# arclab-hku/ESVIO

Measured on AMD Instinct MI355X. Metric: Mevents/s through time-surface+detect+track @640x480, higher is better.
Workload: dtype f64 timestamps / u8 images / f32 LK sums in the reference build's order

## Files before the change

### esvio_amd/csrc/fe_api.cpp

```cpp
#include "fe_internal.h"

namespace {
typedef int (*nccl_allgather_fn)(const void*, void*, size_t, int , void* ,
                                 hipStream_t);
struct NcclId {
  char internal[128];
};
typedef int (*nccl_get_id_fn)(NcclId*);
typedef int (*nccl_init_rank_fn)(void** , int, NcclId, int);
typedef int (*nccl_destroy_fn)(void*);
void* rccl_lib() {
  static void* lib = []() -> void* {
    const char* names[] = {"librccl.so.1", "librccl.so"};
    for (const char* n : names)
      if (void* l = dlopen(n, RTLD_NOW | RTLD_NOLOAD | RTLD_GLOBAL)) return l;
    for (const char* n : names)
      if (void* l = dlopen(n, RTLD_NOW | RTLD_GLOBAL)) return l;
    return dlopen("/opt/rocm/lib/librccl.so.1", RTLD_NOW | RTLD_GLOBAL);
  }();
  return lib;
}
template <class F>
F rccl_sym(const char* name) {
  void* l = rccl_lib();
// ... 143 lines not shown
    c->n_cu = n_cu;
    c->waits_fit_spec = lk_blocks + 2 <= n_cu;
    c->waits_fit_chain = 2 * lk_blocks + 2 <= n_cu;
  }
  int prio_least = 0, prio_greatest = 0;
  (void)hipDeviceGetStreamPriorityRange(&prio_least, &prio_greatest);
  if (c->stream.create(hipStreamNonBlocking, prio_greatest) != hipSuccess ||
      c->stream2.create(hipStreamNonBlocking, prio_least) != hipSuccess ||
      c->stream3.create(hipStreamNonBlocking, prio_greatest) != hipSuccess ||
      c->stream4.create(hipStreamNonBlocking, prio_least) != hipSuccess)
    return bail(ESVIO_FE_EHIP);
  {
    const unsigned timed = c->trace ? 0 : hipEventDisableTiming;
    const std::pair<Event*, unsigned> evs[] = {
        {&c->ev_pts_ready, hipEventDisableTiming},  {&c->ev_spec_done, timed},
        {&c->ev_chain_done, timed},                 {&c->ev_dbg_sel_start, 0},
        {&c->ev_sel_host, timed},                   {&c->ev_lks_done[0], hipEventDisableTiming},
        {&c->ev_lks_done[1], hipEventDisableTiming}, {&c->ev_lknew_done, hipEventDisableTiming},
        {&c->ev_planes_free, hipEventDisableTiming}, {&c->ev_imgs_ready, hipEventDisableTiming},
        {&c->ev_arc_side, hipEventDisableTiming},   {&c->ev_sae_left, hipEventDisableTiming},
        {&c->ev_right_ready, hipEventDisableTiming}};
    for (const auto& ef : evs)
      if (ef.first->create(ef.second) != hipSuccess) return bail(ESVIO_FE_EHIP);
    for (int i = 0; i < kPrefetchDepth; i++)
      if (c->ev_lane_done[i].create(timed) != hipSuccess || c->ev_lane_arc[i].create() != hipSuccess)
        return bail(ESVIO_FE_EHIP);
  }
  const size_t M = cfg->max_cnt;
  const int Mc = cfg->max_cnt;
  int rc = 0;
  if ((rc = c->L2.alloc(c, (size_t)2 * c->P))) return bail(rc);
  if ((rc = c->S2.alloc(c, (size_t)2 * c->P))) return bail(rc);
  if ((rc = c->d_rejected.alloc(c, 1))) return bail(rc);
  if ((rc = c->d_res.alloc(c, res_layout(Mc).total))) return bail(rc);
  c->dres = res_view(c->d_res, Mc, 0);
  c->dres.mask = nullptr;
  {
    uint8_t* z_spec = nullptr;
    const size_t bytes = kSpecBlocks * spec_layout(Mc).bytes;
    if ((rc = c->h_spec.alloc(c, bytes))) return bail(rc);
    if (hipHostGetDevicePointer((void**)&z_spec, c->h_spec, 0) != hipSuccess) return bail(ESVIO_FE_EHIP);
    std::memset(c->h_spec, 0, bytes);
    for (int b = 0; b < kSpecBlocks; b++) {
      c->hspec[b] = spec_view(c->h_spec, Mc, b);
      c->zspec[b] = spec_view(z_spec, Mc, b);
    }
  }
  if ((rc = c->d_chain.alloc(c, 2 * std::max<size_t>(M, 1)))) return bail(rc);
  if ((rc = c->d_lane_gate.alloc(c, 16))) return bail(rc);
  c->stage_threads = stager_threads_from_env();
  if (const char* v = getenv("ESVIO_FE_FAULT")) esvio_fe_debug_inject(c, atoi(v));
  if (const char* e = getenv("ESVIO_FE_STEREO_SPLIT")) c->stereo_split_env = atoi(e) != 0;
  c->chain_enabled = getenv("ESVIO_FE_NO_CHAIN") == nullptr;
  c->cam_split_enabled = getenv("ESVIO_FE_NO_CAMSPLIT") == nullptr;
  c->dedup_enabled = getenv("ESVIO_FE_NO_DEDUP") == nullptr && (cfg->max_cnt > 500 || getenv("ESVIO_FE_DEDUP") != nullptr);
  c->fuse_ts_pyr = getenv("ESVIO_FE_NO_FUSE") == nullptr;
  if (const char* v = getenv("ESVIO_FE_CONVERT_PINNED_COPY")) c->cvt_pinned_copy = atoi(v) != 0 ? 1 : 0;
  if (const char* v = getenv("ESVIO_FE_RAW_PINNED_COPY")) c->rawdec.pinned_copy = atoi(v) != 0 ? 1 : 0;
  c->select_one_wave = getenv("ESVIO_FE_SELECT_SERIAL") != nullptr;
  if (const char* v = getenv("ESVIO_FE_SAE_EV_MIN")) c->sae_ev_min = (size_t)strtoull(v, nullptr, 10);
  c->tiled = make_tile_geom(c->W, c->H, &c->tgeom) && getenv("ESVIO_FE_SAE_SORT") == nullptr;
  for (int i = 0; i < kRightSlots; i++)
    if ((rc = c->d_first[i].alloc(c, (size_t)c->P))) return bail(rc);
  for (int i = 0; i < kRightSlots; i++) {
    const size_t words = arc_bitmap_words(c->W, c->H);
    if ((rc = c->d_cmap[i].alloc(c, words))) return bail(rc);
    if ((rc = c->d_touched[i].alloc(c, arc_flag_bytes(c->W, c->H)))) return bail(rc);
    if (hipMemsetAsync(c->d_cmap[i], 0, words * 4, cur_stream(c)) != hipSuccess ||
        hipMemsetAsync(c->d_touched[i], 0, arc_flag_bytes(c->W, c->H), cur_stream(c)) != hipSuccess)
      return bail(ESVIO_FE_EHIP);
  }
  if ((rc = c->d_pub_slots.alloc(c, std::max<size_t>(M, 1)))) return bail(rc);
  if ((rc = c->d_pub_done.alloc(c, 1))) return bail(rc);
  if (hipMemsetAsync(c->d_lane_gate, 0, 64, cur_stream(c)) != hipSuccess ||
      hipMemsetAsync(c->d_chain, 0, std::max<size_t>(M, 1) * 16, cur_stream(c)) != hipSuccess ||
      hipMemsetAsync(c->d_pub_slots, 0, std::max<size_t>(M, 1) * 8, cur_stream(c)) != hipSuccess ||
      hipMemsetAsync(c->d_pub_done, 0, 8, cur_stream(c)) != hipSuccess)
    return bail(ESVIO_FE_EHIP);
  if ((rc = c->d_ptsD.alloc(c, M))) return bail(rc);
  if ((rc = c->d_sel_idx.alloc(c, M))) return bail(rc);
  if ((rc = c->d_mask_bits.alloc(c, (size_t)c->H * ((c->W + 31) / 32)))) return bail(rc);
  for (PyrStore& ps : c->pyr)
    if ((rc = pyr_alloc(c, ps, c->W, c->H, 3))) return bail(rc);
  if (cfg->median_blur_kernel_size > 0)
    for (PyrStore& ps : c->med_tmp)
      if ((rc = pyr_alloc(c, ps, c->W, c->H, 0))) return bail(rc);
  if (cfg->equalize) {
    for (auto& rb : c->raw)
      for (PyrStore& ps : rb)
        if ((rc = pyr_alloc(c, ps, c->W, c->H, 0))) return bail(rc);
    if ((rc = c->d_lut.alloc(c, (size_t)2 * 64 * 256))) return bail(rc);
    if ((rc = c->d_eq_tmp.alloc(c, (size_t)2 * c->P))) return bail(rc);
    if ((rc = c->d_minmax.alloc(c, 4))) return bail(rc);
  }
  {
    uint8_t* z_res = nullptr;
    if ((rc = c->h_pin.alloc(c, pin_bytes(Mc, cfg->width, cfg->height)))) return bail(rc);
    if (hipHostGetDevicePointer((void**)&z_res, c->h_pin, 0) != hipSuccess) return bail(ESVIO_FE_EHIP);
    std::memset(c->h_pin, 0, c->h_pin.cap);
    for (int s = 0; s < 2; s++) {
      c->pin[s] = res_view(c->h_pin, Mc, s);
      c->zpin[s] = res_view(z_res, Mc, s);
    }
  }
  if (hipMemsetAsync(c->L2, 0, (size_t)2 * c->P * 16, cur_stream(c)) != hipSuccess ||
      hipMemsetAsync(c->S2, 0, (size_t)2 * c->P * 16, cur_stream(c)) != hipSuccess ||
// ... 23 lines not shown
    const hipStream_t st[5] = {c->stream, c->stream2, c->stream3, c->stream4, c->stream6};
    const char* nm[5] = {"main", "prefetch", "speculative", "stereo", "stereo-unpublished"};
    const int ns = c->stream6 ? 5 : 4;
    for (int a = 0; a < ns; a++)
      for (int b = 0; b < ns; b++) {
        if (a == b || st[a] == st[b]) continue;
        launch_spin(st[a], 10000);
        const auto t0 = std::chrono::steady_clock::now();
        launch_fill_f64(st[b], (double*)c->d_rejected, 1, 0.0);
        (void)hipStreamSynchronize(st[b]);
        const double us = std::chrono::duration<double, std::micro>(std::chrono::steady_clock::now() - t0).count();
        (void)hipStreamSynchronize(st[a]);
        if (us > 60.0) {
          c->n_queue_conflicts++;
          fprintf(stderr, "[esvio_fe] streams '%s' and '%s' share a hardware queue (%.0f us behind a 100 us kernel)\n", nm[b], nm[a], us);
        }
      }
    if (!c->n_queue_conflicts) fprintf(stderr, "[esvio_fe] the handle's %d streams have a hardware queue each\n", ns);
  }
  c->select_ok = select_lds_bytes(c) <= 160 * 1024;
  if (!c->select_ok && (rc = c->d_sel_bitmap.alloc(c, (size_t)c->H * ((c->W + 31) / 32) + 4))) return bail(rc);
  *out = c;
  return 0;
}

namespace {
int baf_clear(esvio_fe_ctx* c);
int hot_clear(esvio_fe_ctx* c);
int baf_ensure(esvio_fe_ctx* c, size_t n, bool host_src, bool host_dst, bool fields_form);
void decode_state_reset(esvio_fe_ctx* c);
void feed_empty(esvio_fe_ctx* c, bool streams_idle);
}

int esvio_fe_reset(esvio_fe_handle c) {
  if (!c) return ESVIO_FE_EINVAL;
  HIPCHK(c, hipSetDevice(c->dev));
  (void)launcher_drain(c);
  launcher_clear_error(c);
  HIPCHK(c, hipStreamSynchronize(c->stream3));
  HIPCHK(c, hipStreamSynchronize(c->stream4));
  if (c->stream6) HIPCHK(c, hipStreamSynchronize(c->stream6));
  HIPCHK(c, hipStreamSynchronize(c->stream2));
  HIPCHK(c, hipStreamSynchronize(c->stream));
  c->announced.clear();
  c->inflight.clear();
  stager_drain(c);
  c->cur_stage = -1;
  c->pin[0].counts[3] = 0;
  if (c->hist) HIPCHK(c, hipMemsetAsync(c->hist, 0, c->hist.cap * 4, cur_stream(c)));
  std::memset(c->h_spec, 0, kSpecBlocks * spec_layout(c->cfg.max_cnt).bytes);
  c->spec_valid = false;
  c->chain_valid = false;
  c->chain_map_ok = false;
  c->pend.active = false;
  c->pend_right.active = false;
  HIPCHK(c, hipMemsetAsync(c->L2, 0, (size_t)2 * c->P * 16, cur_stream(c)));
  HIPCHK(c, hipMemsetAsync(c->S2, 0, (size_t)2 * c->P * 16, cur_stream(c)));
  if (c->evimg.on)
    if (int rc = evimg_zero(c, true)) return rc;
  if (int rc = baf_clear(c)) return rc;
  if (int rc = hot_clear(c)) return rc;
  decode_state_reset(c);
  c->slice.st[0] = c->slice.st[1] = esvio_fe_ctx::Slice::State();
  HIPCHK(c, hipStreamSynchronize(cur_stream(c)));
  feed_empty(c, true);
  clear_tracker_state(c);
  return 0;
}

static int create_sae_stereo(esvio_fe_ctx* c, const esvio_fe_event* left, size_t nL, const esvio_fe_event* right,
                             size_t nR, int space, const McParams* mc, uint64_t* n_rejected) {
  if (nL + nR >= (1ull << 31)) return fail(c, ESVIO_FE_EINVAL, "batch too large");
  if (!c->inflight.empty()) return fail(c, ESVIO_FE_EINVAL, "a prefetched batch is pending");
  HIPCHK(c, hipSetDevice(c->dev));
  c->ext_sae_pending = false;
  const EventRec *dL, *dR;
  if (int rc = stage_events(c, left, nL, right, nR, space, &dL, &dR)) return rc;
  HIPCHK(c, hipMemsetAsync(c->d_rejected, 0, 8, cur_stream(c)));
  c->evimg.fresh_cams = 0;
  if (int rc = sae_update(c, dL, (uint32_t)nL, dR, (uint32_t)nR, mc)) return rc;
  unsigned long long rej = 0;
  HIPCHK(c, hipMemcpyAsync(&rej, c->d_rejected, 8, hipMemcpyDeviceToHost, cur_stream(c)));
  HIPCHK(c, hipStreamSynchronize(cur_stream(c)));
  if (int rc = lookback_expired(c)) return rc;
  if (n_rejected) *n_rejected = rej;
  if (c->prof_on) resolve_profile(c);
  return 0;
}

int esvio_fe_create_sae_stereo(esvio_fe_handle c, const esvio_fe_event* left, size_t nL,
                               const esvio_fe_event* right, size_t nR, int space,
                               uint64_t* n_rejected) {
  if (!c || (nL && !left) || (nR && !right)) return ESVIO_FE_EINVAL;
  return create_sae_stereo(c, left, nL, right, nR, space, nullptr, n_rejected);
}

int esvio_fe_create_sae_stereo_mc(esvio_fe_handle c, const esvio_fe_event* left, size_t nL,
                                  const esvio_fe_event* right, size_t nR, int space,
                                  const esvio_fe_motion* motion, uint64_t* n_rejected) {
  if (!c || !motion || !nL || !left || (nR && !right)) return ESVIO_FE_EINVAL;
  const McParams mc = make_mc_params(motion);
  return create_sae_stereo(c, left, nL, right, nR, space, &mc, n_rejected);
}

namespace {
int slice_scratch(esvio_fe_ctx* c) {
// ... 238 lines not shown
    for (uint32_t i = 0; i < c->P; i++) {
      L0[i] = l[2 * i];
      L1[i] = l[2 * i + 1];
      S0[i] = s[2 * i];
      S1[i] = s[2 * i + 1];
    }
  }
  return 0;
}

int esvio_fe_get_sae(esvio_fe_handle c, int cam, double* L0, double* L1, double* S0, double* S1) {
  if (!L0 || !L1 || !S0 || !S1) return ESVIO_FE_EINVAL;
  return planes_io(c, cam, L0, L1, S0, S1, nullptr, nullptr, nullptr, nullptr, false);
}
int esvio_fe_set_sae(esvio_fe_handle c, int cam, const double* L0, const double* L1,
                     const double* S0, const double* S1) {
  if (!L0 || !L1 || !S0 || !S1) return ESVIO_FE_EINVAL;
  return planes_io(c, cam, nullptr, nullptr, nullptr, nullptr, L0, L1, S0, S1, true);
}

static int prep_tmp_pyr(esvio_fe_handle c, int slot, const uint8_t* img, int w, int hgt,
                        int max_level) {
  if (int rc = pyr_alloc(c, c->tmp_pyr[slot], w, hgt, max_level)) return rc;
  return copy_level0_in(c, c->tmp_pyr[slot].d, img);
}

int esvio_fe_calc_optical_flow_pyr_lk(esvio_fe_handle c, const uint8_t* prev_img,
                                      const uint8_t* next_img, int w, int hgt,
                                      const float* prev_pts, float* next_pts, uint8_t* status,
                                      int n, int max_level, int max_count, double eps, int flags) {
  if (!c || !prev_img || !next_img || n < 0 || (n && (!prev_pts || !next_pts || !status)))
    return ESVIO_FE_EINVAL;
  if (w < 2 * kLkWin || hgt < 2 * kLkWin || max_level < 0 || max_level >= kMaxLevels)
    return ESVIO_FE_EINVAL;
  if (n > c->cfg.max_cnt) return fail(c, ESVIO_FE_EINVAL, "n > max_cnt");
  if (!n) return 0;
  HIPCHK(c, hipSetDevice(c->dev));
  if (int rc = prep_tmp_pyr(c, 0, prev_img, w, hgt, max_level)) return rc;
  if (int rc = prep_tmp_pyr(c, 1, next_img, w, hgt, max_level)) return rc;
  PyrDesc two[2] = {c->tmp_pyr[0].d, c->tmp_pyr[1].d};
  pyr_build(c, two, 2);
  float2 *d_prev = (float2*)c->dres.A, *d_next = (float2*)c->dres.s1.fwd;
  uint8_t* d_st = c->dres.s1.st_fwd;
  HIPCHK(c, hipMemcpyAsync(d_prev, prev_pts, (size_t)n * 8, hipMemcpyHostToDevice, cur_stream(c)));
  if (flags & ESVIO_FE_LK_USE_INITIAL_FLOW)
    HIPCHK(c, hipMemcpyAsync(d_next, next_pts, (size_t)n * 8, hipMemcpyHostToDevice, cur_stream(c)));
  LkArgs f = make_lk(two[0], two[1], d_prev, d_next, d_next, d_st, nullptr, n, max_level, max_count, eps, flags);
  run_lk(c, f, nullptr, nullptr, nullptr);
  HIPCHK(c, hipMemcpyAsync(next_pts, d_next, (size_t)n * 8, hipMemcpyDeviceToHost, cur_stream(c)));
  HIPCHK(c, hipMemcpyAsync(status, d_st, (size_t)n, hipMemcpyDeviceToHost, cur_stream(c)));
  HIPCHK(c, hipStreamSynchronize(cur_stream(c)));
  if (c->prof_on) resolve_profile(c);
  return 0;
}

int esvio_fe_build_pyramid(esvio_fe_handle c, const uint8_t* img, int w, int hgt, int max_level,
                           int level, uint8_t* out_img, int16_t* out_deriv, int32_t* lw,
                           int32_t* lh, int32_t* n_levels) {
  if (!c || !img || max_level < 0 || max_level >= kMaxLevels || w < 2 * kLkWin || hgt < 2 * kLkWin)
    return ESVIO_FE_EINVAL;
  HIPCHK(c, hipSetDevice(c->dev));
  if (int rc = prep_tmp_pyr(c, 0, img, w, hgt, max_level)) return rc;
  const PyrDesc& d = c->tmp_pyr[0].d;
  pyr_build(c, &d, 1);
  if (n_levels) *n_levels = d.levels + 1;
  if (level < 0 || level > d.levels) {
    HIPCHK(c, hipStreamSynchronize(cur_stream(c)));
    return level < 0 ? 0 : ESVIO_FE_EINVAL;
  }
  if (lw) *lw = d.w[level];
  if (lh) *lh = d.h[level];
  const int stride = d.stride[level];
  if (out_img)
    HIPCHK(c, hipMemcpy2DAsync(out_img, d.w[level], d.img[level] + (size_t)kPad * stride + kPad,
                               stride, d.w[level], d.h[level], hipMemcpyDeviceToHost, cur_stream(c)));
  if (out_deriv)
    HIPCHK(c, hipMemcpy2DAsync(out_deriv, (size_t)d.w[level] * 4,
                               d.deriv[level] + ((size_t)kPad * stride + kPad) * 2, (size_t)stride * 4,
                               (size_t)d.w[level] * 4, d.h[level], hipMemcpyDeviceToHost, cur_stream(c)));
  HIPCHK(c, hipStreamSynchronize(cur_stream(c)));
  if (c->prof_on) resolve_profile(c);
  return 0;
}

int esvio_fe_find_fundamental_mat(const float* p1, const float* p2, int n, double thr, double conf,
                                  uint8_t* status, int32_t* n_inliers) {
  if (n < 0 || (n && (!p1 || !p2 || !status))) return ESVIO_FE_EINVAL;
  const int k = host::find_fundamental_mat(p1, p2, n, thr, conf, status);
  if (n_inliers) *n_inliers = k;
  return 0;
}

int esvio_fe_host_hypot(const double* x, const double* y, int n, double* out) {
  if (n < 0 || (n && (!x || !y || !out))) return ESVIO_FE_EINVAL;
  host::host_hypot(x, y, n, out);
  return ESVIO_FE_OK;
}

int esvio_fe_host_stage_copy(void* dst, const void* src, size_t len) {
  if (len && (!dst || !src)) return ESVIO_FE_EINVAL;
  stager_copy_bytes((uint8_t*)dst, (const uint8_t*)src, len);
  return ESVIO_FE_OK;
}

int esvio_fe_host_stage_pack(void* dst, const void* src, size_t len, uint32_t* base_sec) {
  uint32_t b = 0;
// ... 3415 lines not shown
  return 0;
}

int esvio_fe_mem_free(int space, void* p) {
  if (space != ESVIO_FE_HOST && space != ESVIO_FE_DEVICE) return ESVIO_FE_EINVAL;
  if (!p) return 0;
  return (space == ESVIO_FE_HOST ? hipHostFree(p) : hipFree(p)) == hipSuccess ? 0 : ESVIO_FE_EHIP;
}

int esvio_fe_mem_upload(void* dst_device, const void* src_host, size_t bytes) {
  if (bytes && (!dst_device || !src_host)) return ESVIO_FE_EINVAL;
  if (!bytes) return 0;
  return hipMemcpy(dst_device, src_host, bytes, hipMemcpyHostToDevice) == hipSuccess ? 0 : ESVIO_FE_EHIP;
}

int esvio_fe_register_host_buffer(void* p, size_t bytes) {
  if (!p || !bytes) return ESVIO_FE_EINVAL;
  if (hipHostRegister(p, bytes, hipHostRegisterDefault) != hipSuccess) {
    (void)hipGetLastError();
    return ESVIO_FE_EHIP;
  }
  return 0;
}

int esvio_fe_unregister_host_buffer(void* p) {
  if (!p) return ESVIO_FE_EINVAL;
  if (hipHostUnregister(p) != hipSuccess) {
    (void)hipGetLastError();
    return ESVIO_FE_EHIP;
  }
  return 0;
}

int esvio_fe_debug_inject(esvio_fe_handle c, int mask) {
  if (!c || mask < 0 || mask > 31) return ESVIO_FE_EINVAL;
  c->lim = esvio_fe_ctx::WaitLimits();
  c->lazy_late = (mask & ESVIO_FE_FAULT_LAZY_LATE) != 0;
  if (mask & ESVIO_FE_FAULT_TICKET) c->lim.ticket = 0;
  if (mask & ESVIO_FE_FAULT_LOOKBACK) c->lim.lookback = 0;
  if (mask & ESVIO_FE_FAULT_SPECULATIVE) c->lim.poll = 0;
  if (mask & ESVIO_FE_FAULT_CHAINED) c->lim.chain = 0;
  return 0;
}

int esvio_fe_debug_counters(esvio_fe_handle c, uint64_t out4[4]) {
  if (!c || !out4) return ESVIO_FE_EINVAL;
  out4[0] = c->n_spec_expired;
  out4[1] = c->n_chain_expired;
  out4[2] = c->tr_chain_launch;
  out4[3] = c->tr_chain_used;
  return 0;
}

int esvio_fe_plain_call_counters(esvio_fe_handle c, uint64_t out4[4]) {
  if (!c || !out4) return ESVIO_FE_EINVAL;
  out4[0] = c->n_plain_calls;
  out4[1] = c->n_cam_split;
  out4[2] = c->n_stereo_chained;
  out4[3] = c->n_chain_expired;
  return 0;
}

int esvio_fe_reserve(esvio_fe_handle c, size_t max_left, size_t max_right, int host_batches) {
  if (!c) return ESVIO_FE_EINVAL;
  const size_t n = max_left + max_right;
  if (n >= (1ull << 31)) return fail(c, ESVIO_FE_EINVAL, "batch too large");
  if (!c->inflight.empty() || !c->announced.empty())
    return fail(c, ESVIO_FE_EINVAL, "esvio_fe_reserve while batches are announced");
  HIPCHK(c, hipSetDevice(c->dev));
  HIPCHK(c, hipStreamSynchronize(c->stream2));
  HIPCHK(c, hipStreamSynchronize(c->stream3));
  HIPCHK(c, hipStreamSynchronize(c->stream4));
  if (c->stream6) HIPCHK(c, hipStreamSynchronize(c->stream6));
  HIPCHK(c, hipStreamSynchronize(c->stream));
  if (c->tiled) {
    if (int rc = ensure_part_capacity(c, n, false)) return rc;
  } else if (int rc = ensure_sort_capacity(c, n)) {
    return rc;
  }
  for (int k = 0; k < kRightSlots; k++)
    if (int rc = ensure_arc_capacity(c, max_left, k)) return rc;
  if (c->baf.B)
    if (int rc = baf_ensure(c, std::max(max_left, max_right), host_batches != 0, false, false)) return rc;
  const size_t events[2] = {max_left, max_right};
  if (int rc = raw_reserve(c, events, host_batches != 0)) return rc;
  if (int rc = text_reserve(c, events, host_batches != 0)) return rc;
  if (int rc = aedat_reserve(c, events)) return rc;
  if (int rc = bag_reserve(c, events)) return rc;
  if (int rc = bag_image_reserve(c)) return rc;
  if (int rc = aedat_frame_reserve(c)) return rc;
  if (c->feed.open) {
    const size_t ev[2] = {max_left, max_right};
    for (int cam = 0; cam < 2; cam++) {
      esvio_fe_ctx::Feed::Cam& fc = c->feed.cam[cam];
      for (int b = 0; b < 2; b++)
        if ((b != fc.cur || fc.len == 0) && fc.buf[b].cap < 2 * ev[cam]) {
          if (int rc = fc.buf[b].alloc(c, 2 * ev[cam])) return rc;
          fc.read_rec[b] = false;
        }
    }
  }
  if (host_batches) {
    if (int rc = ensure_event_capacity(c, n)) return rc;
    if (stager_enabled(c)) {
      if (int rc = stager_reserve(c, n)) return rc;
    } else {
// ... 447 lines not shown
```

### esvio_amd/csrc/fe_ctx.h

```cpp
#pragma once
#include <hip/hip_runtime.h>

#include <algorithm>
#include <atomic>
#include <chrono>
#include <cmath>
#include <cstdarg>
#include <cstdio>
#include <cstdlib>
#include <cstring>
#include <dlfcn.h>
#include <map>
#include <string>
#include <utility>
#include <deque>
#include <vector>

#include "../../include/esvio_fe.h"
#include "../../include/esvio_fe_test.h"
#include "fe_aedat.h"
#include "fe_bag.h"
#include "fe_host.h"
#include "fe_kernels.h"
#include "fe_layout.h"
// ... 180 lines not shown
  DevBuf<double> slice_stage;
  bool ext_sae_pending = false;
  DevBuf<float> x_send, x_recv;
  PinBuf<float> x_pin, x_pin_recv;
  void* x_comm = nullptr;
  int x_world = 0;
  Stream x_stream;
  Event x_done;
  bool x_pending = false;
  bool x_auto = false;
  bool x_deferred = false;
  std::deque<Batch> announced;
  std::deque<Inflight> inflight;
  bool cur_prefetched = false;
  EventStager* stager = nullptr;
  std::atomic<int> stage_pending{0};
  int cur_stage = -1;
  int stage_threads = 0;
  Launcher* launcher = nullptr;
  uint64_t lane_job[kPrefetchDepth] = {};
  int launch_err = 0;
  uint64_t lks_wait_job[2] = {};
  struct WaitLimits {
    uint32_t lookback = kSpinLookback, ticket = kSpinTicket;
    unsigned long long poll = kTicksPoll, chain = kTicksChain;
  } lim;
  bool lazy_late = false;
  uint64_t n_spec_expired = 0, n_chain_expired = 0;
  DevBuf<EventRec> d_evp[kPrefetchDepth];
  Event ev_lane_done[kPrefetchDepth], ev_lane_arc[kPrefetchDepth];
  PyrStore tmp_pyr[2];
  PyrStore med_tmp[2];
  PyrStore raw[kRightSlots][2];
  int raw_cur = 0;
  DevBuf<uint8_t> d_lut;
  DevBuf<int> d_minmax;
  DevBuf<uint8_t> d_res;
  ResView dres{};
  DevBuf<float2> d_ptsD;
  ResView pin[2] = {}, zpin[2] = {};
  SpecView hspec[kSpecBlocks] = {}, zspec[kSpecBlocks] = {};
  int res_set = 0;
  int lks_last = -1;
  PinBuf<uint8_t> h_spec;
  bool spec_valid = false;
  int spec_n = 0;
  DevBuf<unsigned long long> d_chain;
  DevBuf<uint32_t> d_lane_gate;
  uint32_t gate_seq = 0;
  int n_cu = 0;
  bool waits_fit_spec = true, waits_fit_chain = true;
  uint32_t chain_seq = 0;
  bool chain_enabled = true;
  bool cam_split_enabled = true;
  uint64_t n_plain_calls = 0, n_cam_split = 0, n_stereo_chained = 0;
  bool chain_valid = false;
  uint64_t chain_for = 0;
  bool chain_map_ok = false;
  std::vector<int> chain_map;
  uint64_t frame_no = 0;
  Event ev_chain_done;
  DevBuf<unsigned long long> d_pub_slots, d_pub_done;
  uint32_t pub_seq = 0;
  bool lazy_new = false;
  struct PendingNew {
    bool active = false;
    bool prev_map_was_empty = false;
    std::vector<int> ids;
    std::vector<P2f> left;
  } pend;
  struct PendingRight {
    bool active = false;
    int set = 0;
    double dt = 0;
    std::vector<int> ids;
    std::vector<P2f> left;
  } pend_right;
  Event ev_lks_done[2], ev_lknew_done;
  host::RansacPool* pool = nullptr;
  DevBuf<uint8_t> d_flags;
  struct CandSet {
    DevBuf<uint32_t> xy, idx, cnt;
    DevBuf<uint32_t> comp_xy, comp_idx, total, grp;
    size_t cap = 0;
  } cand[kRightSlots];
  DevBuf<uint32_t> d_first[kRightSlots];
  DevBuf<uint32_t> d_cmap[kRightSlots];
  DevBuf<uint8_t> d_touched[kRightSlots];
  uint32_t first_epoch[kRightSlots] = {};
  bool dedup_enabled = true;
  bool fuse_ts_pyr = true;
  int cand_cur = 0;
  DevBuf<uint32_t> d_mask_bits;
  DevBuf<float4> d_gftt_cov, d_gftt_rowsum;
  DevBuf<float> d_gftt_eig;
  DevBuf<uint32_t> d_gftt_max;
  DevBuf<int32_t> d_sel_idx;
  DevBuf<uint8_t> d_fast_img;
  PinBuf<uint8_t> h_img;
  DevBuf<uint8_t> d_img;
  unsigned img_stage_next = 0;
  PinBuf<uint8_t> h_pin;

  int n_id = 0;
  double cur_time = 0, prev_time = 0;
  std::vector<P2f> prev_pts, cur_pts, cur_right_pts, n_pts;
// ... 359 lines not shown
```

### esvio_amd/csrc/fe_host.cpp

```cpp
#include "fe_host.h"

#include <algorithm>
#include <cfloat>
#include <climits>
#include <cmath>
#include <cstdio>
#include <cstdlib>
#include <cstring>

#include <atomic>
#include <chrono>
#include <condition_variable>
#include <sys/resource.h>
#include <memory>
#include <mutex>
#include <thread>

#if defined(__linux__)
#include <pthread.h>
#include <sched.h>
#endif

#if defined(__HIP_DEVICE_COMPILE__) || defined(ESVIO_NO_SIMD_CLONES)
#define ESVIO_SIMD_CLONES
// ... 678 lines not shown
  const double F0 = F[0], F1 = F[1], F2 = F[2], F3 = F[3], F4 = F[4], F5 = F[5], F6 = F[6], F7 = F[7],
               F8 = F[8];
  int good = 0;
  for (int i = i0; i < i1; i++) {
    double a = F0 * x1[i] + F1 * y1[i] + F2;
    double b = F3 * x1[i] + F4 * y1[i] + F5;
    double c = F6 * x1[i] + F7 * y1[i] + F8;
    const double s2 = 1. / (a * a + b * b);
    const double d2 = x2[i] * a + y2[i] * b + c;
    a = F0 * x2[i] + F3 * y2[i] + F6;
    b = F1 * x2[i] + F4 * y2[i] + F7;
    c = F2 * x2[i] + F5 * y2[i] + F8;
    const double s1 = 1. / (a * a + b * b);
    const double d1 = x1[i] * a + y1[i] * b + c;
    const double e1 = d1 * d1 * s1, e2 = d2 * d2 * s2;
    const float err = (float)(e1 < e2 ? e2 : e1);
    const int f = err <= t;
    mask[i] = (uint8_t)f;
    good += f;
  }
  return good;
}

int mark_inliers_bounded(const double* x1, const double* y1, const double* x2, const double* y2, int n,
                         const double* F, uint8_t* mask, double thresh, int need) {
  const float t = (float)(thresh * thresh);
  constexpr int kBlock = 32;
  int good = 0;
  for (int i0 = 0; i0 < n; i0 += kBlock) {
    const int i1 = std::min(n, i0 + kBlock);
    good += score_block(x1, y1, x2, y2, i0, i1, F, t, mask);
    if (good + (n - i1) <= need) return good;
  }
  return good;
}

}

namespace {
constexpr int kRansacMaxIters = 1000;
constexpr int kRansacWindow = 128;
constexpr int kIdleSpinUs = 2000;

struct alignas(64) IterResult {
  int nm;
  int good[3];
  double models[27];
};
constexpr uint32_t kCollinear = 0xffffffffu;
}

namespace {
std::atomic<uint64_t> g_rs_calls{0}, g_rs_iters{0}, g_rs_points{0}, g_rs_ns{0}, g_rs_lm_calls{0}, g_rs_lm_ns{0};
std::atomic<uint64_t> g_rs_max_ns{0}, g_rs_lm_max_ns{0}, g_rs_redone{0}, g_rs_solo{0}, g_rs_skipped{0}, g_rs_helper_sw{0};
void atomic_max(std::atomic<uint64_t>& a, uint64_t v) {
  uint64_t cur = a.load(std::memory_order_relaxed);
  while (v > cur && !a.compare_exchange_weak(cur, v, std::memory_order_relaxed)) {
  }
}
}

struct RansacJob {
  alignas(64) std::atomic<int> next{0};
  alignas(64) std::atomic<int> avail{0};
  alignas(64) std::atomic<int> bound{0};
  alignas(64) std::atomic<int> active{0};
  std::vector<double> xy;
  std::vector<float> pts;
  int count = 0;
  double thr = 0;
  bool lmeds = false;
  std::vector<int32_t> picks;
  std::unique_ptr<IterResult[]> res;
  std::unique_ptr<std::atomic<uint64_t>[]> summary;

  uint32_t evaluate(int idx, IterResult& r, std::vector<uint8_t>& scratch) const {
    float s1[14], s2[14];
    if (!gather(idx, s1, s2)) {
      r.nm = -1;
      return kCollinear;
    }
    r.nm = seven_point(s1, s2, r.models);
    return score(r, scratch);
  }

  void evaluate_lanes(int idx0, int cnt, uint32_t e, std::vector<uint8_t>& scratch) {
    float s1[kLanes][14], s2[kLanes][14];
    int lane_of[kLanes], nm[kLanes], live = 0;
    double models[kLanes][27];
    for (int i = 0; i < cnt; i++) {
      if (gather(idx0 + i, s1[live], s2[live])) {
        lane_of[i] = live++;
      } else {
        lane_of[i] = -1;
        res[idx0 + i].nm = -1;
        summary[idx0 + i].store(((uint64_t)e << 32) | kCollinear, std::memory_order_release);
      }
    }
    if (!live) return;
    seven_point_lanes(live, s1, s2, nm, models);
    for (int i = 0; i < cnt; i++) {
      if (lane_of[i] < 0) continue;
      IterResult& r = res[idx0 + i];
      r.nm = nm[lane_of[i]];
      if (r.nm > 0) std::memcpy(r.models, models[lane_of[i]], sizeof(double) * 9 * r.nm);
      summary[idx0 + i].store(((uint64_t)e << 32) | score(r, scratch), std::memory_order_release);
    }
// ... 289 lines not shown
  if (reset) {
    g_rs_skipped = 0;
    g_rs_helper_sw = 0;
    g_rs_max_ns = 0;
    g_rs_lm_max_ns = 0;
    g_rs_redone = 0;
    g_rs_solo = 0;
  }
}

void host_hypot(const double* x, const double* y, int n, double* out) {
  for (int i = 0; i < n; i++) out[i] = cv_hypot(x[i], y[i]);
}

int host_nullspace(const double* A, int n, int lanes, double* f) {
  if (!lanes) {
    for (int i = 0; i < n; i++)
      epipolar_nullspace((const double(*)[9])(A + (size_t)i * 63), f + (size_t)i * 18, f + (size_t)i * 18 + 9);
    return 0;
  }
  int redone = 0;
  for (int i0 = 0; i0 < n; i0 += kLanes) {
    const int cnt = std::min(kLanes, n - i0);
    double Al[kLanes][7][9], f1[kLanes][9], f2[kLanes][9];
    for (int l = 0; l < kLanes; l++) std::memcpy(Al[l], A + (size_t)(i0 + (l < cnt ? l : 0)) * 63, sizeof(Al[l]));
    if (!epipolar_nullspace_lanes(Al, f1, f2)) {
      for (int l = 0; l < cnt; l++) epipolar_nullspace(Al[l], f1[l], f2[l]);
      redone += cnt;
    }
    for (int l = 0; l < cnt; l++) {
      std::memcpy(f + (size_t)(i0 + l) * 18, f1[l], sizeof(f1[l]));
      std::memcpy(f + (size_t)(i0 + l) * 18 + 9, f2[l], sizeof(f2[l]));
    }
  }
  return redone;
}

RansacStats ransac_stats(bool reset) {
  RansacStats r{g_rs_calls.load(), g_rs_iters.load(), g_rs_points.load(), g_rs_ns.load(),
                g_rs_lm_calls.load(), g_rs_lm_ns.load()};
  if (reset) {
    g_rs_lm_calls = 0;
    g_rs_lm_ns = 0;
    g_rs_calls = 0;
    g_rs_iters = 0;
    g_rs_points = 0;
    g_rs_ns = 0;
    g_rs_max_ns = 0;
    g_rs_lm_max_ns = 0;
    g_rs_redone = 0;
    g_rs_solo = 0;
    g_rs_skipped = 0;
    g_rs_helper_sw = 0;
  }
  return r;
}

namespace {
int ransac_pooled(RansacPool* P, const float* m1, const float* m2, int count, double thr, double conf,
                  const double* xy, uint8_t* status, int* iterations) {
  const int kModelPoints = 7;
  const uint32_t e = P->epoch.load(std::memory_order_relaxed) + 1;
  RansacJob& J = P->job[(e >> 1) & 1];
  while (J.active.load(std::memory_order_acquire) != 0) cpu_relax();
  J.xy.assign(xy, xy + 4 * (size_t)count);
  J.pts.resize(4 * (size_t)count);
  std::memcpy(J.pts.data(), m1, 2 * (size_t)count * sizeof(float));
  std::memcpy(J.pts.data() + 2 * (size_t)count, m2, 2 * (size_t)count * sizeof(float));
  J.count = count;
  J.thr = thr;
  J.lmeds = false;
  J.next.store(0, std::memory_order_relaxed);
  J.avail.store(0, std::memory_order_relaxed);
  J.bound.store(kModelPoints - 1, std::memory_order_relaxed);
  P->epoch.store(e, std::memory_order_release);
  if (!P->th.empty()) ransac_pool_wake(P);

  OcvRng rng;
  std::vector<uint8_t> scratch(count);
  std::vector<uint64_t> rng_before;
  rng_before.reserve(256);
  IterResult local;
  double best_F[9];
  const double *x1 = J.xy.data(), *y1 = x1 + count, *x2 = y1 + count, *y2 = x2 + count;
  int drawn = 0, rp = 0, niters = kRansacMaxIters, best_good = 0;
  bool have_best = false;
  int collinear_at = -1;
  unsigned stalled = 0;
  while (collinear_at < 0) {
    while (rp < niters && rp < drawn) {
      const IterResult* r = &J.res[rp];
      const uint64_t sm = J.summary[rp].load(std::memory_order_acquire);
      uint32_t code;
      if ((uint32_t)(sm >> 32) == e) {
        code = (uint32_t)sm;
      } else if (stalled > 64) {
        code = J.evaluate(rp, local, scratch);
        r = &local;
        g_rs_redone.fetch_add(1, std::memory_order_relaxed);
      } else {
        break;
      }
      stalled = 0;
      if (code == kCollinear) {
        collinear_at = rp;
        break;
      }
      if ((int)code > std::max(best_good, kModelPoints - 1))
        for (int k = 0; k < r->nm; k++)
          if (r->good[k] > std::max(best_good, kModelPoints - 1)) {
            best_good = r->good[k];
            std::memcpy(best_F, r->models + 9 * k, sizeof(best_F));
            have_best = true;
            niters = update_num_iters(conf, (double)(count - best_good) / count, kModelPoints, niters);
          }
      rp++;
      J.bound.store(std::max(best_good, kModelPoints - 1), std::memory_order_relaxed);
    }
    if (rp >= niters || collinear_at >= 0) break;
    if (drawn < niters && drawn - rp < kRansacWindow) {
      for (int j = 0; j < kLanes && drawn < niters; j++) {
        rng_before.push_back(rng.s);
        int32_t* pk = &J.picks[(size_t)drawn * 8];
        for (int i = 0; i < 7; i++) {
          int pick, q;
          for (;;) {
            pick = pk[i] = rng.uniform(0, count);
            for (q = 0; q < i; q++)
              if (pick == pk[q]) break;
            if (q == i) break;
          }
        }
        drawn++;
      }
      J.avail.store(drawn, std::memory_order_release);
      continue;
    }
    int idx = J.next.load(std::memory_order_relaxed);
    if (idx < drawn && J.next.compare_exchange_strong(idx, idx + kLanes, std::memory_order_relaxed)) {
      J.evaluate_lanes(idx, std::min(kLanes, drawn - idx), e, scratch);
    } else {
      cpu_relax();
      stalled++;
    }
  }
  P->epoch.store(e + 1, std::memory_order_release);
  if (collinear_at >= 0) {
    rng.s = rng_before[collinear_at];
    float s1[14], s2[14];
    for (int iter = collinear_at; iter < niters; iter++) {
      if (!draw_subset(m1, m2, count, s1, s2, rng, 10000)) {
        if (iter == 0) return 0;
        break;
      }
      const int nm = seven_point(s1, s2, local.models);
      for (int k = 0; k < nm; k++) {
        const int good = mark_inliers_bounded(x1, y1, x2, y2, count, local.models + 9 * k, scratch.data(), thr,
                                              std::max(best_good, kModelPoints - 1));
        if (good > std::max(best_good, kModelPoints - 1)) {
          best_good = good;
          std::memcpy(best_F, local.models + 9 * k, sizeof(best_F));
          have_best = true;
          niters = update_num_iters(conf, (double)(count - good) / count, kModelPoints, niters);
        }
      }
    }
  }
  *iterations = niters;
  if (have_best) score_block(x1, y1, x2, y2, 0, count, best_F, (float)(thr * thr), status);
  return best_good;
}

int lmeds_pooled(RansacPool* P, const float* m1, const float* m2, int count, double conf, uint8_t* status) {
  const int kModelPoints = 7;
  const int niters = std::max(update_num_iters(conf, 0.45, kModelPoints, kRansacMaxIters), 3);
  const uint32_t e = P->epoch.load(std::memory_order_relaxed) + 1;
  RansacJob& J = P->job[(e >> 1) & 1];
  while (J.active.load(std::memory_order_acquire) != 0) cpu_relax();
  OcvRng rng;
  float s1[14], s2[14];
  int nsub = 0;
  for (; nsub < niters; nsub++)
    if (!draw_subset(m1, m2, count, s1, s2, rng, 1000, &J.picks[(size_t)nsub * 8])) break;
  if (nsub == 0) return 0;
  J.pts.resize(4 * (size_t)count);
  std::memcpy(J.pts.data(), m1, 2 * (size_t)count * sizeof(float));
  std::memcpy(J.pts.data() + 2 * (size_t)count, m2, 2 * (size_t)count * sizeof(float));
  J.count = count;
  J.lmeds = true;
  J.next.store(0, std::memory_order_relaxed);
  J.avail.store(nsub, std::memory_order_relaxed);
  P->epoch.store(e, std::memory_order_release);
  if (!P->th.empty()) ransac_pool_wake(P);
  std::vector<uint8_t> scratch;
  IterResult local;
  double best[9], min_median = DBL_MAX;
  unsigned stalled = 0;
  for (int rp = 0; rp < nsub;) {
    const IterResult* r = &J.res[rp];
    const uint64_t sm = J.summary[rp].load(std::memory_order_acquire);
    if ((uint32_t)(sm >> 32) != e) {
      int idx = J.next.load(std::memory_order_relaxed);
      if (idx < nsub && J.next.compare_exchange_strong(idx, idx + kLanes, std::memory_order_relaxed)) {
        J.evaluate_lanes(idx, std::min(kLanes, nsub - idx), e, scratch);
        continue;
      }
      if (++stalled <= 64) {
        cpu_relax();
        continue;
      }
      J.evaluate(rp, local, scratch);
      r = &local;
      g_rs_redone.fetch_add(1, std::memory_order_relaxed);
    }
    stalled = 0;
    for (int k = 0; k < r->nm; k++) {
      float med;
      std::memcpy(&med, &r->good[k], sizeof(float));
      if ((double)med < min_median) {
        min_median = med;
        std::memcpy(best, r->models + 9 * k, sizeof(best));
      }
    }
    rp++;
  }
  P->epoch.store(e + 1, std::memory_order_release);
  if (min_median < DBL_MAX) {
    double sigma = 2.5 * 1.4826 * (1 + 5. / (count - kModelPoints)) * std::sqrt(min_median);
    sigma = std::max(sigma, 0.001);
    std::vector<float> err(count);
    return mark_inliers(m1, m2, count, best, err, status, sigma);
  }
  return 0;
}
}

int find_fundamental_mat(const float* m1, const float* m2, int count, double thr, double conf,
                         uint8_t* status, RansacPool* pool) {
  std::fill(status, status + count, (uint8_t)0);
  if (count < 7) return 0;
  if (thr <= 0) thr = 3;
  if (conf < DBL_EPSILON || conf > 1 - DBL_EPSILON) conf = 0.99;
  if (count == 7) {
    double models[27];
    const int n = seven_point(m1, m2, models);
    std::fill(status, status + count, (uint8_t)1);
    return n > 0 ? count : 0;
  }
  static thread_local std::unique_ptr<RansacPool> solo;
  if (pool) {
    auto held = [&](uint32_t e) { return pool->job[(e >> 1) & 1].active.load(std::memory_order_acquire) != 0; };
    const uint32_t e = pool->epoch.load(std::memory_order_relaxed) + 1;
    int spins = 0;
    while (held(e) && ++spins < 256) cpu_relax();
    if (held(e)) {
      if (!held(e + 2)) {
        pool->epoch.store(e + 1, std::memory_order_release);
        g_rs_skipped.fetch_add(1, std::memory_order_relaxed);
      } else {
        g_rs_solo.fetch_add(1, std::memory_order_relaxed);
        pool = nullptr;
      }
    }
  }
  if (!pool) {
    if (!solo) solo.reset(ransac_pool_alloc());
    pool = solo.get();
  }
  if (count >= 15) {
    std::vector<double> xy((size_t)4 * count);
    double *x1 = xy.data(), *y1 = x1 + count, *x2 = y1 + count, *y2 = x2 + count;
    for (int i = 0; i < count; i++) {
      x1[i] = m1[2 * i];
      y1[i] = m1[2 * i + 1];
      x2[i] = m2[2 * i];
      y2[i] = m2[2 * i + 1];
    }
    const auto t0 = std::chrono::steady_clock::now();
    int iters = 0;
    const int good = ransac_pooled(pool, m1, m2, count, thr, conf, xy.data(), status, &iters);
    g_rs_calls.fetch_add(1, std::memory_order_relaxed);
    g_rs_iters.fetch_add((uint64_t)iters, std::memory_order_relaxed);
    g_rs_points.fetch_add((uint64_t)count, std::memory_order_relaxed);
    const uint64_t ns = (uint64_t)std::chrono::duration_cast<std::chrono::nanoseconds>(
                            std::chrono::steady_clock::now() - t0).count();
    g_rs_ns.fetch_add(ns, std::memory_order_relaxed);
    atomic_max(g_rs_max_ns, ns);
    return good;
  }
  const auto t0 = std::chrono::steady_clock::now();
  const int good = lmeds_pooled(pool, m1, m2, count, conf, status);
  g_rs_lm_calls.fetch_add(1, std::memory_order_relaxed);
  const uint64_t ns = (uint64_t)std::chrono::duration_cast<std::chrono::nanoseconds>(
                          std::chrono::steady_clock::now() - t0).count();
  g_rs_lm_ns.fetch_add(ns, std::memory_order_relaxed);
  atomic_max(g_rs_lm_max_ns, ns);
  return good;
}

}
}
```

### esvio_amd/csrc/fe_host.h

```cpp
#pragma once
#include <atomic>
#include <stdint.h>

#include <vector>

#include "../../include/esvio_fe.h"
#include "../../include/esvio_fe_test.h"

namespace esvio {
inline void cpu_relax() {
#if !defined(__HIP_DEVICE_COMPILE__) && (defined(__x86_64__) || defined(__i386__))
  __builtin_ia32_pause();
#endif
}
namespace host {

int cv_round(double v);
int cv_floor(float v);

void lift_projective(const esvio_fe_camera& cam, double u, double v, double out[3]);
void lift_projective_batch(const esvio_fe_camera& cam, const float* uv, int n, double* xu, double* yu);

std::vector<int> disc_halfwidths(int r);

struct BitMask {
  int W = 0, H = 0, wpr = 0;
  std::vector<uint32_t> bits;
  void reset(int w, int h);
  bool test(int x, int y) const { return (bits[(size_t)y * wpr + (x >> 5)] >> (x & 31)) & 1u; }
  void stamp_disc(int cx, int cy, int r, const std::vector<int>& hw);
  void from_bytes(const uint8_t* mask);
};

struct RansacPool;
RansacPool* ransac_pool_create(int helpers);
void ransac_pool_destroy(RansacPool* p);
void ransac_pool_wake(RansacPool* p);
void host_hypot(const double* x, const double* y, int n, double* out);
int host_nullspace(const double* A, int n, int lanes, double* f);
struct RansacStats {
  uint64_t calls, iterations, points, ns, lmeds_calls, lmeds_ns;
};
RansacStats ransac_stats(bool reset);
void ransac_tail(uint64_t out6[6], bool reset);
void ransac_pool_hold(RansacPool* p, int mask, bool on);
void ransac_pool_set_idle_work(RansacPool* p, const std::atomic<int>* pending, bool (*fn)(void*), void* arg);
int find_fundamental_mat(const float* p1, const float* p2, int n, double thr, double conf,
                         uint8_t* status, RansacPool* pool = nullptr);

}
}
```

### esvio_amd/csrc/fe_internal.h

```cpp
#pragma once
#include "fe_ctx.h"

namespace esvio {
namespace fe {

template <class T>
void reduce_vector(std::vector<T>& v, const std::vector<uint8_t>& status) {
  int j = 0;
  for (int i = 0; i < int(v.size()); i++)
    if (status[i]) v[j++] = v[i];
  v.resize(j);
}

inline uint8_t* px00(const PyrDesc& d) { return d.img[0] + (size_t)kPad * d.stride[0] + kPad; }

inline int lookback_expired(esvio_fe_ctx* c) {
  return c->pin[0].counts[3] ? fail(c, ESVIO_FE_EINTERNAL, "radix sort look-back spin expired") : 0;
}

int ensure_event_capacity(esvio_fe_ctx* c, size_t n);
int ensure_sort_capacity(esvio_fe_ctx* c, size_t n);
int ensure_part_capacity(esvio_fe_ctx* c, size_t n, bool mc);
int ensure_cand_capacity(esvio_fe_ctx* c, int set, size_t n);
int ensure_arc_capacity(esvio_fe_ctx* c, size_t n, int set);
int pyr_alloc(esvio_fe_ctx* c, PyrStore& ps, int w, int h, int max_level);
uint64_t pyr_pixels(const PyrDesc& d);
void pyr_build(esvio_fe_ctx* c, const PyrDesc* p, int nimg);
McParams make_mc_params(const esvio_fe_motion* m);
int sae_update(esvio_fe_ctx* c, const EventRec* evL, uint32_t nL, const EventRec* evR, uint32_t nR,
               const McParams* mc = nullptr, double2* L2 = nullptr, double2* S2 = nullptr, int arc_set = -1,
               bool* arc_marked = nullptr);
int evimg_update(esvio_fe_ctx* c, const EventRec* evL, uint32_t nL, const EventRec* evR, uint32_t nR, const McParams* mc);
int evimg_zero(esvio_fe_ctx* c, bool every_set = false);
int radix_sort_pairs(esvio_fe_ctx* c, uint32_t n, int passes, int bits, bool booked = true);
struct SortBufs {
  uint32_t *keys[2], *vals[2];
  uint32_t* scratch;
  const uint32_t* n_dev;
};
int radix_sort_pairs(esvio_fe_ctx* c, const SortBufs& b, uint32_t n, int passes, int bits, bool booked);
int cand_set_alloc(esvio_fe_ctx* c, esvio_fe_ctx::CandSet& s, size_t cap, size_t total_words = 1);
int stage_events(esvio_fe_ctx* c, const esvio_fe_event* left, size_t nL, const esvio_fe_event* right,
                 size_t nR, int space, const EventRec** dL, const EventRec** dR, int lane = -1);
void render_ts(esvio_fe_ctx* c, double t_sync, uint8_t* dst0, uint8_t* dst1, int ncam, const double2* S2);
void run_clahe(esvio_fe_ctx* c, const uint8_t* src0, const uint8_t* src1, int src_stride, uint8_t* dst0, uint8_t* dst1,
               int dst_stride, int nimg, int stages, uint64_t booked_px);
void render_lk_images(esvio_fe_ctx* c, double t_sync, int cams, int slotL, int slotR, int rawbuf);
bool render_cam_ok(const esvio_fe_ctx* c);
void build_lk_images(esvio_fe_ctx* c, double t_sync, int cams , int slotL, int slotR,
                     int rawbuf, bool right_imported = false);
inline int other_right_slot(const esvio_fe_ctx* c) { return c->slot_curR == kLeftSlots ? kLeftSlots + 1 : kLeftSlots; }
void rotate_slots(esvio_fe_ctx* c, bool right_advanced);
const PyrDesc& raw_ts_desc(const esvio_fe_ctx* c, int cam);
LkArgs make_lk(const PyrDesc& P, const PyrDesc& N, const float2* prev, const float2* init, float2* next,
               uint8_t* status, const int* n_ptr, int n_max, int max_level, int max_count, double eps,
               int flags);
void run_lk(esvio_fe_ctx* c, const LkArgs& f, const LkArgs* b, float2* back_pts, uint8_t* back_status);
enum LkPairKind { kLkTemporal, kLkStereo };
struct LkPair {
  LkArgs f, b;
  LkOut out;
};
LkPair lk_pair(const PyrDesc& P, const PyrDesc& N, const P2f* src, const int* n_ptr, int n_max, LkPairKind kind,
               const LkOut& out);
void run_lk_pair(esvio_fe_ctx* c, const LkPair& p);
int copy_level0_out(esvio_fe_ctx* c, const PyrDesc& d, uint8_t* out);
int copy_level0_in(esvio_fe_ctx* c, const PyrDesc& d, const uint8_t* in, int space = ESVIO_FE_HOST);
bool in_border_event(const esvio_fe_ctx* c, const P2f& pt);
double pt_distance(const P2f& a, const P2f& b);
void event_set_mask(esvio_fe_ctx* c);
std::vector<P2f> undistorted_pts(const std::vector<P2f>& pts, const esvio_fe_camera& cam);
std::vector<P2f> pts_velocity_fn(std::vector<int>& ids, std::vector<P2f>& pts, IdMap& cur_id_pts,
                                 IdMap& prev_id_pts, double dt, size_t n_left);
void reject_with_f_event(esvio_fe_ctx* c);
void clear_tracker_state(esvio_fe_ctx* c);
SelectArgs make_select_args(esvio_fe_ctx* c, int set, int max_corners, float2* out_pts, int out_base,
                            int32_t* out_idx);
size_t select_lds_bytes(const esvio_fe_ctx* c);
KernelId launch_select_args(esvio_fe_ctx* c, SelectArgs s);
void compact_set(esvio_fe_ctx* c, const esvio_fe_ctx::CandSet& cs, uint32_t nblk, bool booked);
void run_select(esvio_fe_ctx* c, int set, int max_corners, float2* out_pts, int out_base, int32_t* out_idx,
                const uint32_t* mask_bits = nullptr, int* host_counts = nullptr, bool publish = false,
                const float2* stamp_pts = nullptr, int n_stamp = 0);
void run_arc(esvio_fe_ctx* c, const EventRec* ev, uint32_t n, const PyrDesc* ts, bool use_mask,
             bool want_flags, bool want_cand, int set, bool marked = false);
int run_detect(esvio_fe_ctx* c, const EventRec* ev, uint32_t n, const PyrDesc& ts, int set, bool marked);
inline size_t detect_cand_need(const esvio_fe_ctx* c, size_t n) { return c->detector == ESVIO_FE_DETECT_FAST ? (size_t)c->P : n; }
hipError_t sync_main(esvio_fe_ctx* c);
hipError_t sync_event(hipEvent_t ev);

int stager_threads_from_env();
inline bool stager_enabled(const esvio_fe_ctx* c) { return c->stage_threads > 0; }
int stager_begin(esvio_fe_ctx* c, const esvio_fe_event* left, size_t nL, const esvio_fe_event* right, size_t nR,
                 int dma_groups, int* slot_out, bool by_camera = false);
int stager_attach_left(esvio_fe_ctx* c, int slot, hipStream_t s, const EventRec** dL);
int stager_mark_read_aux(esvio_fe_ctx* c, int slot, hipStream_t s);
bool stager_ready(esvio_fe_ctx* c, int slot);
int stager_attach(esvio_fe_ctx* c, int slot, size_t nL, hipStream_t s, const EventRec** dL, const EventRec** dR);
int stager_mark_read(esvio_fe_ctx* c, int slot, hipStream_t s, bool main_stream);
int stager_release(esvio_fe_ctx* c, int slot);
void stager_abandon(esvio_fe_ctx* c, int slot);
void stager_share_pool(esvio_fe_ctx* c);
int stager_reserve(esvio_fe_ctx* c, size_t n_events);
void stager_ptrs(esvio_fe_ctx* c, int slot, size_t nL, const EventRec** dL, const EventRec** dR);
void stager_drain(esvio_fe_ctx* c);
void stager_destroy(esvio_fe_ctx* c);
void stager_copy_bytes(uint8_t* dst, const uint8_t* src, size_t len);
bool stager_pack_bytes(uint8_t* dst, const uint8_t* src, size_t len, uint32_t* base_sec);
void stager_counters(esvio_fe_ctx* c, uint64_t out4[4]);

int prefetch_next(esvio_fe_ctx* c, bool wait_planes, bool must_take_first = false);
int launcher_set(esvio_fe_ctx* c, bool on);
int stereo_split_prepare(esvio_fe_ctx* c);
int launcher_drain(esvio_fe_ctx* c);
int launcher_wait_lane(esvio_fe_ctx* c, int lane);
void launcher_clear_error(esvio_fe_ctx* c);
int cancel_chain(esvio_fe_ctx* c);
int finalize_lazy(esvio_fe_ctx* c);
int track_event_impl(esvio_fe_ctx* c, double cur_time, const esvio_fe_event* left, size_t nL,
                     const esvio_fe_event* right, size_t nR, int space, bool PUB_THIS_FRAME,
                     const esvio_fe_motion* motion = nullptr);

int exchange_pack(esvio_fe_ctx* c);
int exchange_flush(esvio_fe_ctx* c);

void euclid_halfwidths(double md, int8_t* hw , int* radius);
int gftt_run(esvio_fe_ctx* c, const PyrDesc& d, int max_corners, double quality, double min_distance,
// ... 16 lines not shown
```

### esvio_amd/csrc/fe_kernels.h

```cpp
#pragma once
#include <hip/hip_runtime.h>
#include <stdint.h>
#include <stdlib.h>

#include <vector>

namespace esvio {


struct __attribute__((aligned(16))) EventRec {
  uint16_t x, y;
  uint32_t sec, nsec;
  uint8_t pol;
  uint8_t pad[3];
};
static_assert(sizeof(EventRec) == 16, "event record must be 16 B");

constexpr int kPad = 24;
constexpr int kMaxLevels = 4;
constexpr int kLkWin = 21;
constexpr int kArcBlock = 256;
constexpr int kMaxDiscR = 63;

struct PyrDesc {
// ... 205 lines not shown
                      unsigned long long* n_rejected);
void launch_tile_scatter(hipStream_t s, const EventRec* evL, uint32_t nL, const EventRec* evR, uint32_t nR,
                         const TileGeom& g, const TileScratch& sc, EventRec* part, const uint32_t* warp_xy = nullptr);
void launch_tile_apply(hipStream_t s, const EventRec* part, uint32_t n, const TileGeom& g, const TileScratch& sc,
                       double2* L2, double2* S2, double filter_threshold, uint8_t* arc_touched, int* err,
                       uint32_t spin_limit = kSpinTicket);

constexpr double kSliceNone = -1.0;
void launch_fill_f64(hipStream_t s, double* p, size_t n, double v);
void launch_spin(hipStream_t s, unsigned long long ticks);
void launch_set_u32(hipStream_t s, uint32_t* p, uint32_t v);
void launch_overlay_f64(hipStream_t s, double* dst, const double* src, size_t n, double none);

KernelId launch_time_surface(hipStream_t s, const double2* S2, int W, int H, double t_sync,
                         double decay_sec, int ignore_polarity, uint8_t* dst0, uint8_t* dst1,
                         int dst_stride, int ncam);

constexpr int kMaxMedianK = 7;
void launch_median(hipStream_t s, const uint8_t* src0, const uint8_t* src1, int src_stride,
                   uint8_t* dst0, uint8_t* dst1, int dst_stride, int W, int H, int k, int nimg);

void launch_norm_pyr(hipStream_t s, const uint8_t* src0, const uint8_t* src1, int src_stride, const int* minmax,
                     const PyrDesc* p);
void launch_clahe(hipStream_t s, const uint8_t* raw0, const uint8_t* raw1, int raw_stride,
                  uint8_t* dst0, uint8_t* dst1, int dst_stride, int W, int H, uint8_t* lut,
                  int* minmax, int nimg, int stage);

void launch_pyr_down(hipStream_t s, const PyrDesc* p, int nimg, int src_level);
void launch_pyr3(hipStream_t s, const PyrDesc* p, int nimg);
void launch_pyr_pad(hipStream_t s, const PyrDesc* p, int nimg);
void launch_pad_scharr(hipStream_t s, const PyrDesc* p, int nimg);
void launch_scharr(hipStream_t s, const PyrDesc* p, int nimg);

struct LkArgs {
  PyrDesc P;
  PyrDesc N;
  const float2* prev_pts;
  const float2* init_pts;
  float2* next_pts;
  uint8_t* status;
  const int* n_ptr;
  int n_max;
  const unsigned long long* poll_slots = nullptr;
  const unsigned long long* poll_done = nullptr;
  uint32_t poll_seq = 0;
  int poll_from = 0;
  int* poll_err = nullptr;
  unsigned long long* chain_out = nullptr;
  const unsigned long long* chain_in = nullptr;
  uint32_t chain_seq = 0;
  unsigned long long poll_ticks = kTicksPoll, chain_ticks = kTicksChain;
  const uint32_t* gate_ptr = nullptr;
  uint32_t gate_val = 0;
  int max_level;
  int max_count;
  double eps2;
  int flags;
  int accum = 1;
};
void launch_lk(hipStream_t s, const LkArgs& f, const LkArgs* b, float2* back_pts,
               uint8_t* back_status);

struct ArcArgs {
  const EventRec* ev;
  uint32_t n;
  const double2* L2;
  const double2* S2;
  int W, H;
  double filter_threshold;
  int border;
  const uint8_t* ts;
  int ts_stride;
  double ts_lk_threshold;
  const uint32_t* mask_bits;
  int wpr;
  uint8_t* flags;
  uint32_t* cand_xy;
  uint32_t* cand_idx;
  uint32_t* cand_cnt;
  uint32_t* first_map;
  uint32_t first_key;
  uint8_t* touched;
  uint32_t* cmap;
};
inline size_t arc_bitmap_words(int W, int H) { return ((size_t)2 * W * H + 31) / 32 + 64; }
inline size_t arc_flag_bytes(int W, int H) { return (size_t)2 * W * H + 1024; }
void launch_stage_pull(hipStream_t s, const void* pinned_src, void* dst, size_t bytes);
void launch_stage_pull_packed(hipStream_t s, const void* pinned_src, void* dst, size_t bytes, const void* desc, uint32_t epc);
void launch_arc_mark(hipStream_t s, const ArcArgs& a);
void launch_arc_map(hipStream_t s, const ArcArgs& a);
void launch_arc(hipStream_t s, const ArcArgs& a);

void launch_dedup(hipStream_t s, uint32_t* cand_xy, uint32_t* cand_idx, uint32_t* cand_cnt,
                  uint32_t nblk, const uint32_t* first_map, uint32_t first_key, int W);

void launch_compact(hipStream_t s, const uint32_t* cand_xy, const uint32_t* cand_idx,
                    const uint32_t* cand_cnt, uint32_t nblk, uint32_t* comp_xy, uint32_t* comp_idx,
                    uint32_t* total, uint32_t* grp_scratch = nullptr);

struct GfttArgs {
  const uint8_t* img;
  int stride;
  int W, H;
  float4* cov;
  float4* rowsum;
  float* eig;
// ... 446 lines not shown
```

### esvio_amd/csrc/fe_kernels.hip

```cpp
#include "fe_kernels.h"
#include "fe_mc.h"
#include "fe_text.h"

#include <algorithm>
#include <cstdio>
#include <cstdlib>
#include <cstring>
#include <tuple>
#include <type_traits>

namespace esvio {

namespace {
template <typename... P, typename... A>
void launch_k(void (*kernel)(P...), dim3 grid, dim3 block, unsigned shmem, hipStream_t s, A... args) {
  static_assert(sizeof...(P) == sizeof...(A), "argument count");
  hipLaunchKernelGGL(kernel, grid, block, shmem, s, args...);
}
}

__device__ __forceinline__ int lane_id() { return threadIdx.x & 63; }

__device__ __forceinline__ double ev_time(uint32_t sec, uint32_t nsec) {
  return __dadd_rn((double)sec, __dmul_rn(1e-9, (double)nsec));
// ... 2270 lines not shown
          np.y -= d.y * 0.5f;
          level_done = true;
          break;
        }
        if (j >= c.max_count) {
          level_done = true;
          break;
        }
        if (wave_any(inx < -WIN || inx >= cols || iny < -WIN || iny >= rows)) {
          if (L == 0) st = 0;
          level_done = true;
          break;
        }
        if (wave_any(ox > rngx || oy > rngy)) {
          restage = true;
          break;
        }
      }
      (void)restage;
    }
    if (st && L == 0) {
      const float fx = np.x - halfWin, fy = np.y - halfWin;
      const int ix = (int)floorf(fx), iy = (int)floorf(fy);
      if (ix < -WIN || ix >= cols || iy < -WIN || iy >= rows) st = 0;
    }
  }
  np_out = np;
  st_out = st;
}

struct LkKernelArgs {
  LkCall fwd;
  LkCall back;
  int have_back;
  const float2* prev_pts;
  const float2* init_pts;
  float2* next_pts;
  uint8_t* status;
  float2* back_pts;
  uint8_t* back_status;
  const int* n_ptr;
  int n_max;
  const unsigned long long* poll_slots;
  const unsigned long long* poll_done;
  uint32_t poll_seq;
  int poll_from;
  int* poll_err;
  unsigned long long* chain_out;
  const unsigned long long* chain_in;
  uint32_t chain_seq;
  unsigned long long poll_ticks, chain_ticks;
  const uint32_t* gate_ptr;
  uint32_t gate_val;
};

__device__ __forceinline__ void chain_publish(const LkKernelArgs& a, int pt, int lane, float2 p, int alive) {
  if (!a.chain_out || lane != 0) return;
  const unsigned long long hi = (unsigned long long)((a.chain_seq << 2) | (uint32_t)(alive ? 1 : 0)) << 32;
  __hip_atomic_store(&a.chain_out[2 * pt], hi | __float_as_uint(p.x), __ATOMIC_RELAXED, __HIP_MEMORY_SCOPE_AGENT);
  __hip_atomic_store(&a.chain_out[2 * pt + 1], hi | __float_as_uint(p.y), __ATOMIC_RELAXED,
                     __HIP_MEMORY_SCOPE_AGENT);
}

template <int ACCUM>
__device__ __forceinline__ void lk_kernel_body(const LkKernelArgs& a, uint32_t (*regJ_s)[kLkRegStore], uint32_t acc_t,
                                               float* acc_ta, const LkLaneF32* lnf) {
  const int wave = threadIdx.x >> 6, lane = lane_id();
  const int pt = blockIdx.x * kLkWaves + wave;
  const int n = a.n_ptr ? *a.n_ptr : a.n_max;
  if (pt >= a.n_max) return;
  if (pt >= n) {
    chain_publish(a, pt, lane, make_float2(0.f, 0.f), 0);
    return;
  }
  float2 prev0;
  if (a.chain_in) {
    const unsigned long long t0 = wall_clock64();
    unsigned long long vx, vy;
    if (!a.chain_ticks) {
      if (lane == 0) *a.poll_err = 1;
      return;
    }
    for (;;) {
      vx = __hip_atomic_load(&a.chain_in[2 * pt], __ATOMIC_RELAXED, __HIP_MEMORY_SCOPE_AGENT);
      vy = __hip_atomic_load(&a.chain_in[2 * pt + 1], __ATOMIC_RELAXED, __HIP_MEMORY_SCOPE_AGENT);
      if ((uint32_t)(vx >> 34) == a.chain_seq && (uint32_t)(vy >> 34) == a.chain_seq) break;
      if (wall_clock64() - t0 > a.chain_ticks) {
        if (lane == 0) *a.poll_err = 1;
        return;
      }
      __builtin_amdgcn_s_sleep(8);
    }
    if (!((uint32_t)(vx >> 32) & 1u)) {
      if (lane == 0) {
        a.status[pt] = 0;
        if (a.have_back) a.back_status[pt] = 0;
      }
      return;
    }
    prev0 = make_float2(__uint_as_float((uint32_t)vx), __uint_as_float((uint32_t)vy));
    if (a.gate_ptr) {
      for (;;) {
        const uint32_t gv = __hip_atomic_load(a.gate_ptr, __ATOMIC_RELAXED, __HIP_MEMORY_SCOPE_AGENT);
        if ((int)(gv - a.gate_val) >= 0) break;
        if (wall_clock64() - t0 > a.chain_ticks) {
          if (lane == 0) *a.poll_err = 1;
          return;
        }
        __builtin_amdgcn_s_sleep(8);
      }
      __builtin_amdgcn_fence(__ATOMIC_ACQUIRE, "agent");
    }
  } else if (a.poll_slots && pt >= a.poll_from) {
    const unsigned long long t0 = wall_clock64();
    unsigned long long v;
    for (;;) {
      v = __hip_atomic_load(&a.poll_slots[pt], __ATOMIC_RELAXED, __HIP_MEMORY_SCOPE_AGENT);
      if ((uint32_t)(v >> 32) == a.poll_seq) break;
      const unsigned long long d = __hip_atomic_load(a.poll_done, __ATOMIC_RELAXED, __HIP_MEMORY_SCOPE_AGENT);
      if ((uint32_t)(d >> 32) == a.poll_seq && pt >= (int)(uint32_t)d) {
        chain_publish(a, pt, lane, make_float2(0.f, 0.f), 0);
        return;
      }
      if (wall_clock64() - t0 > a.poll_ticks) {
        if (lane == 0) *a.poll_err = 1;
        chain_publish(a, pt, lane, make_float2(0.f, 0.f), 0);
        return;
      }
      __builtin_amdgcn_s_sleep(16);
    }
    prev0 = make_float2((float)(uint32_t)(v & 0xffffu), (float)(uint32_t)((v >> 16) & 0xffffu));
  } else {
    prev0 = a.prev_pts[pt];
  }
  const float2 init = (a.fwd.flags & 4) ? a.init_pts[pt] : make_float2(0.f, 0.f);
  float2 np;
  int st;
  lk_point<ACCUM>(a.fwd, prev0, init, regJ_s[wave], acc_t, acc_ta, lnf, lane, np, st);
  chain_publish(a, pt, lane, np, st);
  if (lane == 0) {
    a.next_pts[pt] = np;
    a.status[pt] = (uint8_t)st;
  }
  if (a.have_back) {
    float2 bp;
    int bs;
    lk_point<ACCUM>(a.back, np, prev0, regJ_s[wave], acc_t, acc_ta, lnf, lane, bp, bs);
    if (lane == 0) {
      a.back_pts[pt] = bp;
      a.back_status[pt] = (uint8_t)bs;
    }
  }
}

__global__ __launch_bounds__(64 * kLkWaves) void k_lk(LkKernelArgs a) {
  __shared__ __attribute__((aligned(16))) uint32_t regJ_s[kLkWaves][kLkRegStore];
  lk_kernel_body<1>(a, regJ_s, 0u, nullptr, nullptr);
}
__global__ __launch_bounds__(64 * kLkWaves) void k_lk_f32(LkKernelArgs a) {
  __shared__ __attribute__((aligned(16))) uint32_t regJ_s[kLkWaves][kLkRegStore];
  __shared__ __attribute__((aligned(16))) int term_all[kLkWaves][kF32TermWords];
  __shared__ __attribute__((aligned(16))) float term_a[kLkWaves][kLkTermWordsA];
  const int wave = threadIdx.x >> 6, lane = threadIdx.x & 63;
  for (int i = lane; i < kF32TermWords; i += 64) term_all[wave][i] = 0;
  {
    const int l = lane < 63 ? lane : 62, t = l / kLkWin, rw = l - t * kLkWin;
    float* z = term_a[wave] + 5 * t * kLkChainWordsA + rw * 5 + 4;
#pragma unroll
    for (int L = 0; L < kMaxLevels; L++)
#pragma unroll
      for (int k = 0; k < 4; k++) z[L * kLkTermLevelA + k * kLkChainWordsA] = 0.f;
  }
  __builtin_amdgcn_fence(__ATOMIC_SEQ_CST, "wavefront", "local");
  const LkLaneF32 lnf =
      lk_lane_f32(lane, (uint32_t)(uintptr_t)(__attribute__((address_space(3))) float*)term_a[wave]);
  const uint32_t tb = (uint32_t)(uintptr_t)(__attribute__((address_space(3))) int*)term_all[wave];
  lk_kernel_body<2>(a, regJ_s, tb, term_a[wave], &lnf);
}

void launch_lk(hipStream_t s, const LkArgs& f, const LkArgs* b, float2* back_pts,
               uint8_t* back_status) {
  if (f.n_max <= 0) return;
  LkKernelArgs a;
  a.fwd.P = f.P;
  a.fwd.N = f.N;
  a.fwd.max_level = f.max_level;
  a.fwd.max_count = f.max_count;
  a.fwd.eps2 = f.eps2;
  a.fwd.flags = f.flags;
  a.have_back = b ? 1 : 0;
  a.back = a.fwd;
  if (b) {
    a.back.P = b->P;
    a.back.N = b->N;
    a.back.max_level = b->max_level;
    a.back.max_count = b->max_count;
    a.back.eps2 = b->eps2;
    a.back.flags = b->flags;
  }
  a.prev_pts = f.prev_pts;
  a.init_pts = f.init_pts;
  a.next_pts = f.next_pts;
  a.status = f.status;
  a.back_pts = back_pts;
  a.back_status = back_status;
  a.n_ptr = f.n_ptr;
  a.n_max = f.n_max;
  a.poll_slots = f.poll_slots;
  a.poll_done = f.poll_done;
  a.poll_seq = f.poll_seq;
  a.poll_from = f.poll_from;
  a.poll_err = f.poll_err;
  a.chain_out = f.chain_out;
  a.chain_in = f.chain_in;
  a.chain_seq = f.chain_seq;
  a.poll_ticks = f.poll_ticks;
  a.chain_ticks = f.chain_ticks;
  a.gate_ptr = f.gate_ptr;
  a.gate_val = f.gate_val;
  if (f.accum == 2)
    launch_k(k_lk_f32, dim3((a.n_max + kLkWaves - 1) / kLkWaves), dim3(64 * kLkWaves), 0, s, a);
  else
    launch_k(k_lk, dim3((a.n_max + kLkWaves - 1) / kLkWaves), dim3(64 * kLkWaves), 0, s, a);
}

__constant__ int8_t c_small[16][2] = {{0, 3},  {1, 3},   {2, 2},   {3, 1},  {3, 0},  {3, -1},
                                      {2, -2}, {1, -3},  {0, -3},  {-1, -3}, {-2, -2}, {-3, -1},
                                      {-3, 0}, {-3, 1},  {-2, 2},  {-1, 3}};
__constant__ int8_t c_large[20][2] = {{0, 4},   {1, 4},   {2, 3},   {3, 2},  {4, 1},  {4, 0},  {4, -1},
                                      {3, -2},  {2, -3},  {1, -4},  {0, -4}, {-1, -4}, {-2, -3}, {-3, -2},
                                      {-4, -1}, {-4, 0},  {-4, 1},  {-3, 2}, {-2, 3},  {-1, 4}};

template <int N>
struct RingRanks {
  unsigned long long lo, hi;
  __device__ __forceinline__ int get(int i) const {
    if (N <= 16) return (int)((lo >> (4 * i)) & 15ull);
    return i < 10 ? (int)((lo >> (5 * i)) & 31ull) : (int)((hi >> (5 * (i - 10))) & 31ull);
  }
};

template <int N, int KMIN, int KMAX>
__device__ __forceinline__ bool arc_ring_ranks(const double (&v)[N]) {
  int r[N];
#pragma unroll
  for (int i = 0; i < N; i++) r[i] = 0;
#pragma unroll
  for (int i = 1; i < N; i++)
#pragma unroll
    for (int j = 0; j < i; j++) {
      r[i] += v[j] < v[i] ? 1 : 0;
      r[j] += v[i] < v[j] ? 1 : 0;
    }
  RingRanks<N> rk;
  rk.lo = 0;
  rk.hi = 0;
#pragma unroll
  for (int i = 0; i < N; i++) {
    if (N <= 16) rk.lo |= (unsigned long long)r[i] << (4 * i);
    else if (i < 10) rk.lo |= (unsigned long long)r[i] << (5 * i);
    else rk.hi |= (unsigned long long)r[i] << (5 * (i - 10));
  }
  int segment_new_min_t = r[0];
  int arc_right_idx = 0;
#pragma unroll
  for (int i = 1; i < N; i++)
    if (r[i] > segment_new_min_t) {
      segment_new_min_t = r[i];
      arc_right_idx = i;
    }
  int arc_left_idx = arc_right_idx == 0 ? N - 1 : arc_right_idx - 1;
  arc_right_idx = arc_right_idx == N - 1 ? 0 : arc_right_idx + 1;
// ... 3655 lines not shown
```

### esvio_amd/csrc/fe_layout.h

```cpp
#pragma once
#include <cstddef>
#include <cstdint>

namespace esvio {
namespace fe {

struct P2f {
  float x, y;
};

struct LkOut {
  P2f *fwd, *back;
  uint8_t *st_fwd, *st_back;
};

inline size_t layout_points(int max_cnt) { return max_cnt > 1 ? (size_t)max_cnt : 1; }
inline size_t round_up(size_t v, size_t to) { return (v + to - 1) / to * to; }

struct ResLayout {
  size_t B1[2], C1[2], SA1[2], SB1[2], A[2], CNT, NEW, B2, C2, SA2, SB2, total;
  size_t mask;
};
inline ResLayout res_layout(int max_cnt) {
  const size_t M = layout_points(max_cnt), stM = round_up(M, 64);
  ResLayout L;
  size_t o = 0;
  for (int s = 0; s < 2; s++) {
    L.B1[s] = o;  o += M * 8;
    L.C1[s] = o;  o += M * 8;
    L.SA1[s] = o; o += stM;
    L.SB1[s] = o; o += stM;
    L.A[s] = o;   o += M * 8;
  }
  L.CNT = o; o += 64;
  L.NEW = o; o += M * 8;
  L.B2 = o;  o += M * 8;
  L.C2 = o;  o += M * 8;
  L.SA2 = o; o += stM;
  L.SB2 = o; o += stM;
  L.total = o;
  L.mask = round_up(o, 256);
  return L;
}
inline size_t pin_bytes(int max_cnt, int width, int height) {
  return res_layout(max_cnt).mask + (size_t)height * ((width + 31) / 32) * 4 + 256;
}

struct SpecLayout {
  size_t B, C, SA, SB, expired, bytes;
};
inline SpecLayout spec_layout(int max_cnt) {
  const size_t M = layout_points(max_cnt), stM = round_up(M, 64);
  SpecLayout L;
  L.B = 0;
  L.C = M * 8;
  L.SA = M * 16;
  L.SB = L.SA + stM;
  L.expired = L.SB + stM;
  L.bytes = round_up(L.expired + 64, 256);
  return L;
}
constexpr int kSpecBlocks = 2;

struct ResView {
  LkOut s1;
  P2f* A;
  LkOut s2;
  P2f* news;
  int* counts;
  uint32_t* mask;
};
inline ResView res_view(uint8_t* b, int max_cnt, int set) {
  const ResLayout L = res_layout(max_cnt);
  ResView v;
  v.s1 = LkOut{(P2f*)(b + L.B1[set]), (P2f*)(b + L.C1[set]), b + L.SA1[set], b + L.SB1[set]};
  v.A = (P2f*)(b + L.A[set]);
  v.s2 = LkOut{(P2f*)(b + L.B2), (P2f*)(b + L.C2), b + L.SA2, b + L.SB2};
  v.news = (P2f*)(b + L.NEW);
  v.counts = (int*)(b + L.CNT);
  v.mask = (uint32_t*)(b + L.mask);
  return v;
}

struct SpecView {
  LkOut out;
  int* expired;
};
inline SpecView spec_view(uint8_t* b, int max_cnt, int block) {
  const SpecLayout L = spec_layout(max_cnt);
  b += (size_t)block * L.bytes;
  return SpecView{LkOut{(P2f*)(b + L.B), (P2f*)(b + L.C), b + L.SA, b + L.SB}, (int*)(b + L.expired)};
}

}
}
```

### esvio_amd/csrc/fe_stages.cpp

```cpp
#include "fe_internal.h"

#include <optional>

namespace esvio {
namespace fe {


int ensure_event_capacity(esvio_fe_ctx* c, size_t n) { return c->d_ev.grow(c, n); }

static int grow_sort_buffers(esvio_fe_ctx* c, size_t cap) {
  c->sort_cap = 0;
  for (int i = 0; i < 2; i++) {
    c->keys[i].release();
    c->vals[i].release();
  }
  for (int i = 0; i < 2; i++) {
    if (int rc = c->keys[i].alloc(c, cap)) return rc;
    if (int rc = c->vals[i].alloc(c, cap)) return rc;
  }
  if (int rc = c->sae_marks.alloc(c, cap)) return rc;
  c->sort_cap = cap;
  return 0;
}

// ... 431 lines not shown
  return LkPair{make_lk(P, N, (const float2*)src, nullptr, (float2*)out.fwd, out.st_fwd, n_ptr, n_max, 3, 30, 0.01, 0),
                make_lk(N, P, nullptr, nullptr, nullptr, nullptr, n_ptr, n_max, t ? 1 : 3, 30, 0.01,
                        t ? ESVIO_FE_LK_USE_INITIAL_FLOW : 0),
                out};
}

void run_lk_pair(esvio_fe_ctx* c, const LkPair& p) {
  run_lk(c, p.f, c->cfg.flow_back ? &p.b : nullptr, (float2*)p.out.back, p.out.st_back);
}

static int image_stage_slot(esvio_fe_ctx* c, size_t bytes, size_t* off) {
  constexpr int kSlots = 4;
  if (!c->d_img || c->d_img.cap < kSlots * bytes) {
    HIPCHK(c, hipStreamSynchronize(cur_stream(c)));
    c->d_img.release();
    if (int rc = c->h_img.alloc(c, kSlots * bytes)) return rc;
    if (int rc = c->d_img.alloc(c, kSlots * bytes)) return rc;
  }
  *off = (size_t)(c->img_stage_next++ % kSlots) * (c->d_img.cap / kSlots);
  return 0;
}

int copy_level0_in(esvio_fe_ctx* c, const PyrDesc& d, const uint8_t* in, int space) {
  const int stride = d.stride[0];
  const size_t bytes = (size_t)d.w[0] * d.h[0];
  if (space == ESVIO_FE_DEVICE) {
    HIPCHK(c, hipMemcpy2DAsync(d.img[0] + (size_t)kPad * stride + kPad, stride, in, d.w[0], d.w[0], d.h[0], hipMemcpyDeviceToDevice,
                               cur_stream(c)));
    return 0;
  }
  size_t off = 0;
  if (int rc = image_stage_slot(c, bytes, &off)) return rc;
  std::memcpy(c->h_img + off, in, bytes);
  HIPCHK(c, hipMemcpyAsync(c->d_img + off, c->h_img + off, bytes, hipMemcpyHostToDevice, cur_stream(c)));
  HIPCHK(c, hipMemcpy2DAsync(d.img[0] + (size_t)kPad * stride + kPad, stride, c->d_img + off, d.w[0], d.w[0],
                             d.h[0], hipMemcpyDeviceToDevice, cur_stream(c)));
  return 0;
}

int copy_level0_out(esvio_fe_ctx* c, const PyrDesc& d, uint8_t* out) {
  const int stride = d.stride[0];
  const size_t bytes = (size_t)d.w[0] * d.h[0];
  size_t off = 0;
  if (int rc = image_stage_slot(c, bytes, &off)) return rc;
  HIPCHK(c, hipMemcpy2DAsync(c->d_img + off, d.w[0], d.img[0] + (size_t)kPad * stride + kPad, stride, d.w[0],
                             d.h[0], hipMemcpyDeviceToDevice, cur_stream(c)));
  HIPCHK(c, hipMemcpyAsync(c->h_img + off, c->d_img + off, bytes, hipMemcpyDeviceToHost, cur_stream(c)));
  HIPCHK(c, hipStreamSynchronize(cur_stream(c)));
  std::memcpy(out, c->h_img + off, bytes);
  return 0;
}


bool in_border_event(const esvio_fe_ctx* c, const P2f& pt) {
  const int BORDER_SIZE = 1;
  const int img_x = host::cv_round(pt.x), img_y = host::cv_round(pt.y);
  return BORDER_SIZE <= img_x && img_x < c->W - BORDER_SIZE && BORDER_SIZE <= img_y &&
         img_y < c->H - BORDER_SIZE;
}

double pt_distance(const P2f& a, const P2f& b) {
  const double dx = a.x - b.x, dy = a.y - b.y;
  return std::sqrt(dx * dx + dy * dy);
}

void event_set_mask(esvio_fe_ctx* c) {
  c->mask_event.reset(c->W, c->H);
  struct Item {
    int first;
    std::pair<P2f, int> second;
    int src;
  };
  std::vector<Item> cnt_pts_id;
  cnt_pts_id.reserve(c->cur_pts.size());
  for (unsigned int i = 0; i < c->cur_pts.size(); i++)
    cnt_pts_id.push_back(Item{c->track_cnt[i], std::make_pair(c->cur_pts[i], c->ids[i]), c->src_idx[i]});
  std::sort(cnt_pts_id.begin(), cnt_pts_id.end(),
            [](const Item& a, const Item& b) { return a.first > b.first; });
  c->cur_pts.clear();
  c->ids.clear();
  c->track_cnt.clear();
  c->src_idx.clear();
  for (auto& it : cnt_pts_id) {
    const int px = host::cv_round(it.second.first.x), py = host::cv_round(it.second.first.y);
    if (px < 0 || px >= c->W || py < 0 || py >= c->H) continue;
    if (!c->mask_event.test(px, py)) {
      c->cur_pts.push_back(it.second.first);
      c->ids.push_back(it.second.second);
      c->track_cnt.push_back(it.first);
      c->src_idx.push_back(it.src);
      c->mask_event.stamp_disc(px, py, c->cfg.min_dist, c->hw);
    }
  }
}

std::vector<P2f> undistorted_pts(const std::vector<P2f>& pts, const esvio_fe_camera& cam) {
  const size_t n = pts.size();
  std::vector<P2f> un(n);
  if (!n) return un;
  std::vector<double> lx(n), ly(n);
  host::lift_projective_batch(cam, &pts[0].x, (int)n, lx.data(), ly.data());
  for (size_t i = 0; i < n; i++) un[i] = P2f{(float)lx[i], (float)ly[i]};
  return un;
}

std::vector<P2f> pts_velocity_fn(std::vector<int>& ids, std::vector<P2f>& pts, IdMap& cur_id_pts,
                                 IdMap& prev_id_pts, double dt, size_t n_left) {
  std::vector<P2f> vel;
  cur_id_pts.build(ids, pts);
  if (!prev_id_pts.empty()) {
    vel.reserve(pts.size());
    for (unsigned int i = 0; i < pts.size(); i++) {
      const P2f* prev = ids[i] != -1 ? prev_id_pts.find(ids[i]) : nullptr;
      if (prev) {
        const double v_x = (pts[i].x - prev->x) / dt;
        const double v_y = (pts[i].y - prev->y) / dt;
        vel.push_back(P2f{(float)v_x, (float)v_y});
      } else {
        vel.push_back(P2f{0, 0});
      }
    }
  } else {
    vel.assign(n_left, P2f{0, 0});
  }
  return vel;
}

void reject_with_f_event(esvio_fe_ctx* c) {
  if (c->trace) c->tr_fm_class[c->cur_pts.size() < 8 ? 0 : c->cur_pts.size() < 15 ? 1 : 2]++;
  if (c->cur_pts.size() >= 8) {
    const esvio_fe_camera& cam = c->cfg.cam[0];
    const double FOCAL = c->cfg.focal_length;
    const size_t n = c->prev_pts.size();
    std::vector<float> un_cur(n * 2), un_prev(n * 2);
    std::vector<double> lx(n), ly(n);
    const double cx = c->W / 2.0, cy = c->H / 2.0;
    const auto tl = std::chrono::steady_clock::now();
    const bool pre = c->pre_lift_valid && c->pre_lx.size() == n;
    if (!pre) host::lift_projective_batch(cam, &c->prev_pts[0].x, (int)n, lx.data(), ly.data());
    const double* plx = pre ? c->pre_lx.data() : lx.data();
    const double* ply = pre ? c->pre_ly.data() : ly.data();
    c->pre_lift_valid = false;
    for (size_t i = 0; i < n; i++) {
      un_prev[2 * i] = (float)(FOCAL * plx[i] / 1.0 + cx);
      un_prev[2 * i + 1] = (float)(FOCAL * ply[i] / 1.0 + cy);
    }
    host::lift_projective_batch(cam, &c->cur_pts[0].x, (int)n, lx.data(), ly.data());
    for (size_t i = 0; i < n; i++) {
      un_cur[2 * i] = (float)(FOCAL * lx[i] / 1.0 + cx);
      un_cur[2 * i + 1] = (float)(FOCAL * ly[i] / 1.0 + cy);
    }
    std::vector<uint8_t> status(c->cur_pts.size());
    const auto t0 = std::chrono::steady_clock::now();
    host::find_fundamental_mat(un_prev.data(), un_cur.data(), (int)c->cur_pts.size(),
                               c->cfg.f_threshold, 0.99, status.data(), c->pool);
    if (c->trace) {
      const double ms = std::chrono::duration<double, std::milli>(std::chrono::steady_clock::now() - t0).count();
      c->tr_fm_ms += ms;
      c->tr_fm_max_ms = std::max(c->tr_fm_max_ms, ms);
      c->tr_lift_ms += std::chrono::duration<double, std::milli>(t0 - tl).count();
    }
    reduce_vector(c->prev_pts, status);
    reduce_vector(c->cur_pts, status);
    reduce_vector(c->ids, status);
    reduce_vector(c->track_cnt, status);
    reduce_vector(c->src_idx, status);
  }
}

void clear_tracker_state(esvio_fe_ctx* c) {
  c->prev_pts.clear();
  c->cur_pts.clear();
  c->cur_right_pts.clear();
  c->n_pts.clear();
  c->cur_un_pts.clear();
  c->cur_un_right_pts.clear();
  c->pts_velocity.clear();
  c->right_pts_velocity.clear();
  c->ids.clear();
  c->ids_right.clear();
  c->track_cnt.clear();
  c->track_cnt_right.clear();
  c->cur_un_pts_map.clear();
  c->prev_un_pts_map.clear();
  c->cur_un_right_pts_map.clear();
  c->prev_un_right_pts_map.clear();
  c->have_img = false;
  c->slot_prevL = c->slot_curL = 0;
  c->slot_curR = kLeftSlots;
  c->ext_right_pending = false;
  c->ext_sae_pending = false;
  c->cur_time = c->prev_time = 0;
}

SelectArgs make_select_args(esvio_fe_ctx* c, int set, int max_corners, float2* out_pts, int out_base,
                            int32_t* out_idx) {
  SelectArgs s{};
  s.comp_xy = c->cand[set].comp_xy;
  s.comp_idx = c->cand[set].comp_idx;
  s.total = c->cand[set].total;
  s.W = c->W;
  s.H = c->H;
  s.wpr = (c->W + 31) / 32;
  s.max_corners = max_corners;
  s.radius = c->cfg.min_dist;
  for (int i = 0; i <= kMaxDiscR; i++) s.hw[i] = i < (int)c->hw.size() ? (int8_t)c->hw[i] : -1;
  s.disc_c = disc_threshold(s.hw, s.radius);
  s.out_pts = out_pts;
  s.out_idx = out_idx;
  s.out_base = out_base;
  s.n_out = c->dres.counts;
  s.n_total = c->dres.counts + 1;
  s.host_counts = nullptr;
  s.init_bits = nullptr;
  s.gbitmap = nullptr;
  s.pub_slots = nullptr;
  s.pub_done = nullptr;
  s.pub_seq = 0;
  s.one_wave = c->select_one_wave ? 1 : 0;
  return s;
// ... 113 lines not shown
```

### esvio_amd/csrc/fe_track.cpp

```cpp
#include "fe_internal.h"

#include <sched.h>
#include <sys/resource.h>

#include <atomic>
#include <condition_variable>
#include <mutex>
#include <thread>

namespace esvio {
namespace fe {

struct PrefetchJob {
  Inflight b;
  bool wait_planes = false;
  int lks_wait = -1;
};

static int prefetch_issue(esvio_fe_ctx* c, const PrefetchJob& j) {
  const Inflight& b = j.b;
  StreamScope on_prefetch_stream(c->stream2);
  PrefetchBatchScope its_event_images(&b);
  if (j.wait_planes) HIPCHK(c, hipStreamWaitEvent(c->stream2, c->ev_planes_free, 0));
  if (j.lks_wait >= 0) HIPCHK(c, hipStreamWaitEvent(c->stream2, c->ev_lks_done[j.lks_wait], 0));
// ... 237 lines not shown
      }
    }
    if (rc) break;
    c->inflight.push_back(b);
    c->announced.pop_front();
    if (only_first) break;
  }
  return rc;
}

static uint32_t next_chain_seq(esvio_fe_ctx* c) {
  c->chain_seq = (c->chain_seq + 1) & 0x3fffffffu;
  if (!c->chain_seq) c->chain_seq = 1;
  return c->chain_seq;
}

int enqueue_spec_temporal(esvio_fe_ctx* c, const Inflight& nxt ,
                          int n_kept, bool with_new) {
  if (int rc = launcher_wait_lane(c, nxt.lane)) return rc;
  HIPCHK(c, hipStreamWaitEvent(c->stream3, c->ev_lane_done[nxt.lane], 0));
  const PyrDesc& P = c->pyr[c->slot_curL].d;
  const PyrDesc& N = c->pyr[nxt.slotL].d;
  const int n_max = with_new ? (int)layout_points(c->cfg.max_cnt) : n_kept;
  LkPair sp = lk_pair(P, N, c->zpin[0].news, nullptr, n_max, kLkTemporal, c->zspec[0].out);
  if (with_new) {
    sp.f.poll_slots = c->d_pub_slots;
    sp.f.poll_done = c->d_pub_done;
    sp.f.poll_seq = c->pub_seq;
    sp.f.poll_from = n_kept;
    sp.f.poll_err = c->zspec[0].expired;
    sp.f.poll_ticks = c->lim.poll;
  }
  const Inflight* nxt2 = nullptr;
  if (c->chain_enabled && c->waits_fit_chain && !nxt.pub && c->inflight.size() >= 2 && c->inflight[0].lane == nxt.lane &&
      !c->chain_valid)
    nxt2 = &c->inflight[1];
  if (nxt2) {
    sp.f.chain_out = c->d_chain;
    sp.f.chain_seq = next_chain_seq(c);
  }
  {
    StreamScope on_spec_stream(c->stream3);
    run_lk_pair(c, sp);
  }
  HIPCHK(c, hipEventRecord(c->ev_spec_done, c->stream3));
  c->spec_valid = true;
  if (nxt2) {
    const bool gated = c->launcher && nxt2->gate != 0;
    if (!gated)
      if (int rc = launcher_wait_lane(c, nxt2->lane)) return rc;
    HIPCHK(c, hipStreamWaitEvent(c->stream4, c->ev_lane_done[nxt.lane], 0));
    if (!gated) HIPCHK(c, hipStreamWaitEvent(c->stream4, c->ev_lane_done[nxt2->lane], 0));
    const PyrDesc& N2 = c->pyr[nxt2->slotL].d;
    LkPair ch = lk_pair(N, N2, nullptr, nullptr, n_max, kLkTemporal, c->zspec[1].out);
    ch.f.chain_in = c->d_chain;
    ch.f.chain_seq = c->chain_seq;
    ch.f.chain_ticks = c->lim.chain;
    ch.f.poll_err = c->zspec[1].expired;
    if (gated) {
      ch.f.gate_ptr = c->d_lane_gate + nxt2->lane;
      ch.f.gate_val = nxt2->gate;
    }
    {
      StreamScope on_chain_stream(c->stream4);
      run_lk_pair(c, ch);
    }
    HIPCHK(c, hipEventRecord(c->ev_chain_done, c->stream4));
    c->chain_valid = true;
    c->tr_chain_launch++;
    c->chain_for = c->frame_no + 2;
    c->chain_map_ok = false;
  }
  return 0;
}

int cancel_chain(esvio_fe_ctx* c) {
  if (!c->chain_valid) return 0;
  c->chain_valid = false;
  c->chain_map_ok = false;
  c->tr_chain_cancel++;
  HIPCHK(c, hipStreamSynchronize(c->stream4));
  return 0;
}

void right_tail(esvio_fe_ctx* c, const LkOut& kept, const P2f* left, const int* ids, const int* src,
                int n, int n_kept, double dt, size_t n_left) {
  const esvio_fe_config& cfg = c->cfg;
  c->ids_right.clear();
  c->cur_right_pts.clear();
  c->cur_un_right_pts.clear();
  c->right_pts_velocity.clear();
  c->cur_un_right_pts_map.clear();
  c->track_cnt_right.clear();
  if (n_left) {
    std::vector<uint8_t> status(n), statusRightLeft(n);
    std::vector<P2f> reverseLeftPts(n);
    c->cur_right_pts.resize(n);
    for (int i = 0; i < n; i++) {
      const LkOut& r = i < n_kept ? kept : c->pin[0].s2;
      const int j = i < n_kept ? (src ? src[i] : i) : i - n_kept;
      c->cur_right_pts[i] = r.fwd[j];
      status[i] = r.st_fwd[j];
      reverseLeftPts[i] = r.back[j];
      statusRightLeft[i] = r.st_back[j];
    }
    if (cfg.flow_back && !c->cur_right_pts.empty()) {
      for (int i = 0; i < n; i++) {
        if (status[i] && statusRightLeft[i] && in_border_event(c, c->cur_right_pts[i]) &&
            pt_distance(left[i], reverseLeftPts[i]) <= 0.5)
          status[i] = 1;
        else
          status[i] = 0;
      }
    }
    c->ids_right.assign(ids, ids + n);
    reduce_vector(c->cur_right_pts, status);
    reduce_vector(c->ids_right, status);
    c->track_cnt_right.assign(c->cur_right_pts.size(), 1);
    c->cur_un_right_pts = undistorted_pts(c->cur_right_pts, cfg.cam[1]);
    c->right_pts_velocity =
        pts_velocity_fn(c->ids_right, c->cur_un_right_pts, c->cur_un_right_pts_map,
                        c->prev_un_right_pts_map, dt, n_left);
  }
  c->prev_un_right_pts_map.swap(c->cur_un_right_pts_map);
}

static int finalize_right(esvio_fe_ctx* c) {
  if (!c->pend_right.active) return 0;
  esvio_fe_ctx::PendingRight& pr = c->pend_right;
  pr.active = false;
  const int n = (int)pr.left.size();
  if (n) HIPCHK(c, sync_event(c->ev_lks_done[pr.set]));
  if (int rc = lookback_expired(c)) return rc;
  right_tail(c, c->pin[pr.set].s1, pr.left.data(), pr.ids.data(), nullptr, n, n, pr.dt, (size_t)n);
  return 0;
}
// ... 15 lines not shown
      add_ids.push_back(c->pend.ids[j]);
    }
  }
  if (add.empty()) return 0;
  const std::vector<P2f> un = undistorted_pts(add, cfg.cam[1]);
  for (size_t j = 0; j < add.size(); j++) {
    c->ids_right.push_back(add_ids[j]);
    c->cur_right_pts.push_back(add[j]);
    c->cur_un_right_pts.push_back(un[j]);
    c->track_cnt_right.push_back(1);
    if (!c->pend.prev_map_was_empty) c->right_pts_velocity.push_back(P2f{0, 0});
    c->prev_un_right_pts_map.v.emplace_back(add_ids[j], un[j]);
  }
  return 0;
}

int finalize_lazy(esvio_fe_ctx* c) {
  if (int rc = finalize_pending(c)) return rc;
  return finalize_right(c);
}

static bool event_over(hipEvent_t ev) {
  const bool over = hipEventQuery(ev) != hipErrorNotReady;
  (void)hipGetLastError();
  return over;
}

namespace {
using clk = std::chrono::steady_clock;

struct TrackCall {
  esvio_fe_ctx* c;
  const double time;
  const esvio_fe_event *left, *right;
  const size_t nL, nR;
  const int space;
  const bool PUB_THIS_FRAME;
  const esvio_fe_motion* motion;
  const int M;
  ResView pin{}, zpin{};
  const EventRec *dL = nullptr, *dR = nullptr;
  bool first = false;
  bool arc_done = false, arc_prefetched = false, arc_marked_main = false;
  int arc_lane = 0;
  bool main_reads_events = false;
  bool main_reads_planes = false;
  bool have_next = false, had_announced = false;
  Inflight next_b;
  bool early_done = false, defer_late = false;
  bool use_spec = false, use_chain = false, chain_covers_next = false;
  bool will_spec = false, detect = false;
  bool plain = false, arc_side = false, stereo_chained = false;
  bool split_right = false;
  int set_st = 0;
  std::vector<int> surv_src;
  int n_surv = 0, n_kept = 0;
  PhaseClock clock;

  TrackCall(esvio_fe_ctx* ctx, double t, const esvio_fe_event* l, size_t nl, const esvio_fe_event* r, size_t nr,
            int sp, bool pub, const esvio_fe_motion* mo)
      : c(ctx), time(t), left(l), right(r), nL(nl), nR(nr), space(sp), PUB_THIS_FRAME(pub), motion(mo),
        M(ctx->cfg.max_cnt) {}

  void lap(Phase p) { c->lat.cur_phase[p] += clock.lap(); }

  bool same_motion(const Batch& a) const {
    if ((motion != nullptr) != a.has_motion) return false;
    if (!motion) return true;
    const esvio_fe_motion &x = *motion, &y = a.motion;
    bool eq = x.t1 == y.t1 && x.fx == y.fx && x.fy == y.fy && x.cx == y.cx && x.cy == y.cy;
    for (int i = 0; i < 3; i++)
      eq = eq && x.v[i] == y.v[i] && x.v_pre[i] == y.v_pre[i] && x.accel[i] == y.accel[i] && x.omega[i] == y.omega[i];
    return eq;
  }

  int check() {
    if (c->launch_err)
      return fail(c, c->launch_err, "a prefetch job of the launch thread failed earlier: esvio_fe_reset the handle");
    if (c->inflight.empty() && !c->announced.empty()) {
      const Batch& a = c->announced.front();
      if (left == a.left && nL == a.nL && right == a.right && nR == a.nR && space == a.space) {
        if (time != a.time || !same_motion(a))
          return fail(c, ESVIO_FE_EINVAL, "batch differs from the one given to esvio_fe_set_next_batch");
        HIPCHK(c, hipEventRecord(c->ev_planes_free, c->stream));
        if (int rc = prefetch_next(c, true, true)) return rc;
      }
    }
    if (!c->inflight.empty()) {
      const Inflight& b = c->inflight.front();
      if (left != b.left || nL != b.nL || right != b.right || nR != b.nR || space != b.space ||
          time != b.time || !same_motion(b))
        return fail(c, ESVIO_FE_EINVAL, "batch differs from the one given to esvio_fe_set_next_batch");
      if (PUB_THIS_FRAME && !b.arc_done && c->inflight.size() > 1)
        return fail(c, ESVIO_FE_EINVAL,
                    "PUB hint was 0 for a published frame and a later batch is already applied to "
                    "the SAE: with more than one batch announced the hint must be exact");
    }
    return 0;
  }

  int take_batch() {
    first = !c->have_img;
    c->cur_stage = -1;
    if (!c->inflight.empty()) {
      const Inflight b = c->inflight.front();
      c->inflight.pop_front();
// ... 113 lines not shown
      const PyrDesc ts = raw_ts_desc(c, 0);
      if (plain) {
        StreamScope on_side_stream(c->stream2);
        HIPCHK(c, hipStreamWaitEvent(c->stream2, c->ev_imgs_ready, 0));
        if (int rc = run_detect(c, dL, (uint32_t)nL, ts, c->cand_cur, arc_marked_main)) return rc;
        HIPCHK(c, hipEventRecord(c->ev_arc_side, c->stream2));
        arc_side = true;
      } else {
        if (int rc = run_detect(c, dL, (uint32_t)nL, ts, c->cand_cur, arc_marked_main)) return rc;
      }
      arc_done = true;
      main_reads_planes = true;
      main_reads_events = true;
    }
    if (!had_announced) return 0;
    if (main_reads_planes) HIPCHK(c, hipEventRecord(c->ev_planes_free, c->stream));
    return prefetch_next(c, main_reads_planes);
  }

  int plan_temporal() {
    if (c->spec_valid) {
      c->spec_valid = false;
      use_spec = c->cur_prefetched && (int)c->prev_pts.size() == c->spec_n;
      if (!use_spec) HIPCHK(c, hipStreamSynchronize(c->stream3));
    }
    if (c->chain_valid && c->chain_for == c->frame_no) {
      use_chain = !use_spec && c->cur_prefetched && c->chain_map_ok &&
                  c->chain_map.size() == c->prev_pts.size();
      if (!use_chain)
        if (int rc = cancel_chain(c)) return rc;
      c->chain_valid = false;
    } else if (c->chain_valid && (c->chain_for != c->frame_no + 1 || PUB_THIS_FRAME || !use_spec)) {
      if (int rc = cancel_chain(c)) return rc;
    }
    chain_covers_next = c->chain_valid;
    const bool early_results = use_spec || use_chain;
    const bool before_sync = early_results && !PUB_THIS_FRAME;
    defer_late = !(PUB_THIS_FRAME && !arc_done) && have_next && !before_sync;
    return 0;
  }

  void pre_lift() {
    const esvio_fe_config& cfg = c->cfg;
    const size_t n = c->prev_pts.size();
    if (!PUB_THIS_FRAME || !cfg.f_ransac || n < 8 || c->pre_lift_valid) return;
    c->pre_lx.resize(n);
    c->pre_ly.resize(n);
    host::lift_projective_batch(cfg.cam[0], &c->prev_pts[0].x, (int)n, c->pre_lx.data(), c->pre_ly.data());
    c->pre_lift_valid = true;
  }

  bool take_expired(int block) { return std::exchange(*c->hspec[block].expired, 0) != 0; }

  int await_early(hipEvent_t done, int block, bool* ok) {
    if (!defer_late)
      if (int rc = early_work()) return rc;
    pre_lift();
    lap(PH_ENQ_TEMPORAL);
    if (int rc = exchange_flush(c)) return rc;
    HIPCHK(c, sync_event(done));
    lap(PH_WAIT_TEMPORAL);
    *ok = !take_expired(block);
    return 0;
  }

  int temporal() {
    if (int rc = plan_temporal()) return rc;
    const esvio_fe_config& cfg = c->cfg;
    c->pre_lift_valid = false;
    const PyrDesc& prevL = c->pyr[c->slot_prevL].d;
    const PyrDesc& curL = c->pyr[c->slot_curL].d;
    if (c->prev_pts.size() > 0) {
      const int n = (int)c->prev_pts.size();
      LkOut t{};
      bool spec_ok = false;
      if (use_spec) {
        if (int rc = await_early(c->ev_spec_done, 0, &spec_ok)) return rc;
        t = c->hspec[0].out;
        if (!spec_ok) {
          c->n_spec_expired++;
          HIPCHK(c, hipStreamSynchronize(c->stream3));
        }
      }
      std::vector<P2f> g_ptsB, g_ptsC;
      std::vector<uint8_t> g_stA, g_stB;
      if (use_chain) {
        if (int rc = await_early(c->ev_chain_done, 1, &spec_ok)) return rc;
        c->tr_chain_used += spec_ok;
        if (!spec_ok) c->n_chain_expired++;
        if (c->trace && spec_ok) trace_chain_intervals();
        if (spec_ok) {
          const LkOut& r = c->hspec[1].out;
          g_ptsB.resize(n);
          g_ptsC.resize(n);
          g_stA.resize(n);
          g_stB.resize(n);
          for (int j = 0; j < n; j++) {
            const int k = c->chain_map[j];
            g_ptsB[j] = r.fwd[k];
            g_ptsC[j] = r.back[k];
            g_stA[j] = r.st_fwd[k];
            g_stB[j] = r.st_back[k];
          }
          t = LkOut{g_ptsB.data(), g_ptsC.data(), g_stA.data(), g_stB.data()};
        }
      }
      if (!spec_ok) {
        std::memcpy(pin.A, c->prev_pts.data(), (size_t)n * 8);
        LkPair lk = lk_pair(prevL, curL, zpin.A, nullptr, n, kLkTemporal, zpin.s1);
        stereo_chained = plain && c->chain_enabled && c->waits_fit_chain;
        if (stereo_chained) {
          c->n_stereo_chained++;
          lk.f.chain_out = c->d_chain;
          lk.f.chain_seq = next_chain_seq(c);
        }
        run_lk_pair(c, lk);
        if (stereo_chained) {
          const PyrDesc& curR = c->pyr[c->slot_curR].d;
          set_st = c->res_set ^ 1;
          LkPair st = lk_pair(curL, curR, nullptr, nullptr, n, kLkStereo, c->zpin[set_st].s1);
          st.f.chain_in = c->d_chain;
          st.f.chain_seq = c->chain_seq;
          st.f.chain_ticks = c->lim.chain;
          st.f.poll_err = c->zspec[1].expired;
          StreamScope on_stereo_stream(stereo_stream(c));
          HIPCHK(c, hipStreamWaitEvent(stereo_stream(c), c->ev_imgs_ready, 0));
          run_lk_pair(c, st);
          if (int rc = record_lks_done(c, c->res_set)) return rc;
        }
        if (int rc = early_work()) return rc;
        if (int rc = exchange_flush(c)) return rc;
        pre_lift();
        lap(PH_ENQ_TEMPORAL);
        HIPCHK(c, sync_main(c));
        lap(PH_WAIT_TEMPORAL);
        t = pin.s1;
      }
      std::vector<uint8_t> status(t.st_fwd, t.st_fwd + n);
      c->cur_pts.resize(n);
      std::memcpy(c->cur_pts.data(), t.fwd, (size_t)n * 8);
      if (cfg.flow_back) {
        const P2f* reverse_pts = t.back;
        for (int i = 0; i < n; i++) {
          if (status[i] && t.st_back[i] && pt_distance(c->prev_pts[i], reverse_pts[i]) <= 0.5)
            status[i] = 1;
          else
            status[i] = 0;
        }
      }
      for (int i = 0; i < n; i++)
        if (status[i] && !in_border_event(c, c->cur_pts[i])) status[i] = 0;
      if (chain_covers_next) {
        if (use_spec && spec_ok) {
          c->chain_map.clear();
          for (int i = 0; i < n; i++)
            if (status[i]) c->chain_map.push_back(i);
          c->chain_map_ok = true;
        } else if (int rc = cancel_chain(c)) {
          return rc;
        }
      }
      if (stereo_chained) {
        surv_src.clear();
        for (int i = 0; i < n; i++)
          if (status[i]) surv_src.push_back(i);
// ... 23 lines not shown
      c->tr_gpu_sel += a;
      c->tr_gpu_spec += b;
      c->tr_gpu_chain += d;
      float e2 = 0;
      if (c->tr_lane >= 0 && hipEventElapsedTime(&e2, c->ev_sel_host, c->ev_lane_done[c->tr_lane]) == hipSuccess)
        c->tr_gpu_pyr += e2;
      else
        (void)hipGetLastError();
      c->tr_host_chain += std::chrono::duration<double, std::milli>(clk::now() - c->tr_sel_launch).count();
      c->tr_gpu_n++;
    } else {
      (void)hipGetLastError();
    }
  }

  int upload_kept() {
    if (!will_spec || !n_kept) return 0;
    if (c->pend.active && M > 1024) HIPCHK(c, sync_event(c->ev_lknew_done));
    std::memcpy(pin.news, c->cur_pts.data(), (size_t)n_kept * 8);
    return 0;
  }

  int survivors_stereo() {
    const PyrDesc& curL = c->pyr[c->slot_curL].d;
    const PyrDesc& curR = c->pyr[c->slot_curR].d;
    n_surv = (int)c->cur_pts.size();
    c->src_idx.resize(n_surv);
    for (int i = 0; i < n_surv; i++) c->src_idx[i] = stereo_chained ? surv_src[i] : i;
    lap(PH_FILTER);
    n_kept = n_surv;
    will_spec = (have_next || had_announced) && c->waits_fit_spec;
    if (!PUB_THIS_FRAME) {
      if (int rc = upload_kept()) return rc;
      if (will_spec && n_kept && !c->chain_valid)
        if (const Inflight* nb = next_batch())
          if (int rc = enqueue_spec_temporal(c, *nb, n_kept, false)) return rc;
    }
    if (n_surv && !stereo_chained) {
      std::memcpy(pin.A, c->cur_pts.data(), (size_t)n_surv * 8);
      {
        StreamScope on_stereo_stream(stereo_stream(c));
        run_lk_pair(c, lk_pair(curL, curR, zpin.A, nullptr, n_surv, kLkStereo, zpin.s1));
        if (int rc = record_lks_done(c, c->res_set)) return rc;
      }
    }
    return 0;
  }

  int publish() {
    const esvio_fe_config& cfg = c->cfg;
    const PyrDesc& curL = c->pyr[c->slot_curL].d;
    const PyrDesc& curR = c->pyr[c->slot_curR].d;
    if (PUB_THIS_FRAME) {
      if (cfg.f_ransac) reject_with_f_event(c);
      lap(PH_RANSAC);
      PhaseClock parts;
      auto sub = [&](Phase p) { c->lat.cur_phase[p] += parts.lap(); };
      event_set_mask(c);
      sub(PH_PUB_SETMASK);
      if (arc_side) HIPCHK(c, hipStreamWaitEvent(c->stream, c->ev_arc_side, 0));
      n_kept = (int)c->cur_pts.size();
      const int n_max_cnt = M - n_kept;
      if (int rc = upload_kept()) return rc;
      if (n_max_cnt <= 0 && will_spec && n_kept)
        if (const Inflight* nb = next_batch())
          if (int rc = enqueue_spec_temporal(c, *nb, n_kept, false)) return rc;
      if (n_max_cnt > 0) {
        detect = true;
        if (!will_spec && n_kept) std::memcpy(pin.news, c->cur_pts.data(), (size_t)n_kept * 8);
        if (arc_prefetched) HIPCHK(c, hipStreamWaitEvent(c->stream, c->ev_lane_arc[arc_lane], 0));
        c->pub_seq++;
        if (c->trace) {
          HIPCHK(c, hipEventRecord(c->ev_dbg_sel_start, cur_stream(c)));
          c->tr_sel_launch = clk::now();
        }
        run_select(c, c->cand_cur, n_max_cnt, (float2*)zpin.news, n_kept, nullptr, nullptr, zpin.counts, will_spec,
                   (const float2*)zpin.news, n_kept);
        sub(PH_PUB_SELECT);
        if (will_spec)
          if (const Inflight* nb = next_batch())
            if (int rc = enqueue_spec_temporal(c, *nb, n_kept, true)) return rc;
        sub(PH_PUB_SPEC);
        HIPCHK(c, hipEventRecord(c->ev_sel_host, cur_stream(c)));
        if (int rc = finalize_pending(c)) return rc;
        if (!c->pend_right.active || c->pend_right.left.empty() ||
            (!c->lazy_late && event_over(c->ev_lks_done[c->pend_right.set])))
          if (int rc = finalize_right(c)) return rc;
        sub(PH_PUB_PREV_RIGHT);
        if (split_right) HIPCHK(c, hipStreamWaitEvent(c->stream, c->ev_right_ready, 0));
        run_lk_pair(c, lk_pair(curL, curR, zpin.news + n_kept, c->dres.counts, n_max_cnt, kLkStereo, zpin.s2));
        if (c->lazy_new) HIPCHK(c, hipEventRecord(c->ev_lknew_done, cur_stream(c)));
        sub(PH_PUB_STEREO_NEW);
      }
      if (defer_late)
        if (int rc = early_work()) return rc;
      sub(PH_PUB_PREFETCH);
    } else if (defer_late) {
      if (int rc = early_work()) return rc;
    }
    lap(PH_MASK_DETECT);
    if (detect) HIPCHK(c, sync_event(c->ev_sel_host));
    return 0;
  }

  int tails() {
    const esvio_fe_config& cfg = c->cfg;
    int n_new = 0;
    if (PUB_THIS_FRAME) {
      c->n_pts.clear();
      if (detect) {
        n_new = pin.counts[0];
// ... 200 lines not shown
```

### esvio_amd/frontend.py

```python
import ctypes as C
import os

import numpy as np

from . import build as _build

_HERE = os.path.dirname(os.path.abspath(__file__))
HOST, DEVICE = 0, 1
EVENT_IMAGES_AHEAD = 2
LK_USE_INITIAL_FLOW = 4


class FrontendError(RuntimeError):
    pass


class Camera(C.Structure):
    _fields_ = [(n, C.c_double) for n in ("fx", "fy", "cx", "cy", "k1", "k2", "p1", "p2")]


class Config(C.Structure):
    _fields_ = [
        ("width", C.c_int32), ("height", C.c_int32),
        ("decay_ms", C.c_double),
# ... 260 lines not shown
        if origin is not None:
            self.origin.sec, self.origin.nsec, self.has_origin = int(origin[0]), int(origin[1]), 1


class SliceInfo(C.Structure):
    _fields_ = [("closed", C.c_uint64), ("first_window", C.c_uint64), ("count", C.c_uint64), ("open_events", C.c_uint64),
                ("first_sec", C.c_uint32), ("first_nsec", C.c_uint32), ("last_sec", C.c_uint32), ("last_nsec", C.c_uint32)]


SLICE_MAX_WINDOWS = 4096


class FeedInfo(C.Structure):
    _fields_ = [("appended", C.c_uint64), ("rejected", C.c_uint64), ("bad", C.c_uint64), ("closed", C.c_uint64),
                ("queued", C.c_uint64)]


class FeedWindow(C.Structure):
    _fields_ = [("ready", C.c_int32), ("reserved", C.c_int32), ("index", C.c_uint64), ("end_sec", C.c_uint32),
                ("end_nsec", C.c_uint32), ("count", C.c_uint64 * 2)]


class Tracks(C.Structure):
    _fields_ = [
        ("n_left", C.c_int32), ("n_right", C.c_int32),
        ("ids", C.c_void_p), ("track_cnt", C.c_void_p),
        ("cur_pts", C.c_void_p), ("cur_un_pts", C.c_void_p), ("pts_velocity", C.c_void_p),
        ("ids_right", C.c_void_p), ("cur_right_pts", C.c_void_p),
        ("cur_un_right_pts", C.c_void_p), ("right_pts_velocity", C.c_void_p),
    ]


ABI_SYMBOLS = [
    "esvio_fe_calc_optical_flow_pyr_lk", "esvio_fe_comm_init", "esvio_fe_comm_unique_id",
    "esvio_fe_convert_events", "esvio_fe_create", "esvio_fe_decode_raw", "esvio_fe_decode_reset",
    "esvio_fe_decode_triggers", "esvio_fe_raw_header", "esvio_fe_slice_events_at",
    "esvio_fe_aedat_header", "esvio_fe_decode_aedat", "esvio_fe_aedat_side", "esvio_fe_track_aedat", "esvio_fe_feed_push_aedat",
    "esvio_fe_decode_aedat_frames", "esvio_fe_convert_frame16",
    "esvio_fe_bag_header", "esvio_fe_bag_set_topics", "esvio_fe_decode_bag", "esvio_fe_bag_side", "esvio_fe_feed_push_bag",
    "esvio_fe_bag_set_image_topics", "esvio_fe_decode_bag_images", "esvio_fe_convert_image", "esvio_fe_track_image_space",
    "esvio_fe_create_sae", "esvio_fe_create_sae_stereo", "esvio_fe_create_sae_stereo_mc", "esvio_fe_destroy",
    "esvio_fe_exchange_begin", "esvio_fe_exchange_end", "esvio_fe_exchange_tracks", "esvio_fe_export_image",
    "esvio_fe_feed_close", "esvio_fe_feed_open", "esvio_fe_feed_peek", "esvio_fe_feed_push_events", "esvio_fe_feed_push_fields",
    "esvio_fe_feed_push_raw", "esvio_fe_feed_track",
    "esvio_fe_fast_corners", "esvio_fe_filter_batch", "esvio_fe_filter_events", "esvio_fe_filter_reset", "esvio_fe_features_to_track", "esvio_fe_features_to_track_fast", "esvio_fe_find_fundamental_mat", "esvio_fe_finish", "esvio_fe_get_sae",
    "esvio_fe_get_pixel_mask", "esvio_fe_get_time_surface", "esvio_fe_good_features_to_track", "esvio_fe_hot_learn",
    "esvio_fe_hot_reset", "esvio_fe_hot_select", "esvio_fe_import_image", "esvio_fe_is_corner",
    "esvio_fe_last_error", "esvio_fe_mem_alloc", "esvio_fe_mem_free", "esvio_fe_mem_upload",
    "esvio_fe_pack_track_records", "esvio_fe_register_host_buffer", "esvio_fe_reserve", "esvio_fe_reset",
    "esvio_fe_sae_plane_doubles", "esvio_fe_sae_slice_apply", "esvio_fe_sae_slice_commit",
    "esvio_fe_sae_slice_last", "esvio_fe_sae_to_time_surface", "esvio_fe_set_address_filter", "esvio_fe_set_auto_exchange",
    "esvio_fe_set_detector", "esvio_fe_set_pixel_mask",
    "esvio_fe_set_event_images", "esvio_fe_clear_event_images", "esvio_fe_get_event_image", "esvio_fe_get_event_canvas",
    "esvio_fe_set_host_threads", "esvio_fe_set_launch_thread", "esvio_fe_set_lazy_new_stereo",
    "esvio_fe_set_next_batch", "esvio_fe_set_next_batch_mc", "esvio_fe_slice_events", "esvio_fe_slice_flush",
    "esvio_fe_slice_reset", "esvio_fe_track_batch", "esvio_fe_track_event", "esvio_fe_track_event_fields",
    "esvio_fe_track_event_filtered", "esvio_fe_track_event_mc", "esvio_fe_track_raw",
    "esvio_fe_track_image", "esvio_fe_unregister_host_buffer", "esvio_fe_version",
    "esvio_fe_kf_set_pattern", "esvio_fe_kf_blur", "esvio_fe_kf_fast", "esvio_fe_kf_brief", "esvio_fe_kf_match",
    "esvio_fe_kf_describe",
    "esvio_fe_bow_vocabulary_header", "esvio_fe_bow_set_vocabulary", "esvio_fe_bow_transform", "esvio_fe_bow_add",
    "esvio_fe_bow_query", "esvio_fe_bow_detect_loop", "esvio_fe_bow_clear", "esvio_fe_bow_entries", "esvio_fe_bow_reserve",
    "esvio_fe_bow_create_vocabulary", "esvio_fe_bow_get_created",
    "esvio_fe_decode_text", "esvio_fe_track_text", "esvio_fe_feed_push_text", "esvio_fe_text_imu", "esvio_fe_text_images",
]
TEST_SYMBOLS = [
    "esvio_fe_build_pyramid", "esvio_fe_debug_counters", "esvio_fe_debug_inject", "esvio_fe_device_memory",
    "esvio_fe_export_level",
    "esvio_fe_find_fundamental_mat_held", "esvio_fe_find_fundamental_mat_idle", "esvio_fe_find_fundamental_mat_mt",
    "esvio_fe_get_kernel_stats", "esvio_fe_host_hypot", "esvio_fe_host_nullspace", "esvio_fe_host_stage_copy",
    "esvio_fe_host_stage_pack", "esvio_fe_staging_counters",
    "esvio_fe_kernel_count", "esvio_fe_kernel_name", "esvio_fe_latency_phase_name", "esvio_fe_latency_recent",
    "esvio_fe_latency_stats", "esvio_fe_lift_projective", "esvio_fe_plain_call_counters", "esvio_fe_ransac_stats",
    "esvio_fe_ransac_tail", "esvio_fe_raw_tile_bytes", "esvio_fe_reset_kernel_stats", "esvio_fe_select_candidates",
    "esvio_fe_set_profiling", "esvio_fe_set_sae",
    "esvio_fe_slice_tile_events", "esvio_fe_stage_kernel_count", "esvio_fe_stream",
    "esvio_fe_aedat_tile_events", "esvio_fe_ingest_kernel_count", "esvio_fe_aedat_walk_tap", "esvio_fe_aedat_walk_state_bytes",
    "esvio_fe_bag_tile_events", "esvio_fe_bag_walk_tap", "esvio_fe_bag_walk_state_bytes",
    "esvio_fe_bag_image_walk_tap", "esvio_fe_image_tile_pixels", "esvio_fe_event_image_kernel_stats",
    "esvio_fe_aedat_frame_walk_tap", "esvio_fe_aedat_frame_kernel_stats", "esvio_fe_frame16_tile_pixels",
    "esvio_fe_kf_kernel_count", "esvio_fe_kf_kernel_name", "esvio_fe_kf_kernel_stats", "esvio_fe_kf_blur_tile",
    "esvio_fe_bow_kernel_count", "esvio_fe_bow_kernel_name", "esvio_fe_bow_kernel_stats", "esvio_fe_bow_limits", "esvio_fe_bow_scores",
    "esvio_fe_bow_create_kernel_count", "esvio_fe_bow_create_kernel_name", "esvio_fe_bow_create_kernel_stats", "esvio_fe_bow_create_pick",
    "esvio_fe_text_limits", "esvio_fe_text_kernel_count", "esvio_fe_text_kernel_name", "esvio_fe_text_kernel_stats",
    "esvio_fe_scan_lanes",
]

LATENCY_PHASES = 16
SELECT_EUCLID, SELECT_TABLE = 1, 2


class LatencyCall(C.Structure):
    _fields_ = [("call", C.c_uint64), ("published", C.c_int32), ("reserved", C.c_int32), ("begin_ms", C.c_double),
                ("ms", C.c_double), ("phase_ms", C.c_double * LATENCY_PHASES)]


class KfOut(C.Structure):
    _fields_ = [("window_desc", C.c_void_p), ("kp_xy", C.c_void_p), ("kp_score", C.c_void_p), ("kp_norm", C.c_void_p),
                ("kp_desc", C.c_void_p), ("kp_capacity", C.c_int32), ("n_kp", C.c_int32), ("n_detected", C.c_int32),
                ("desc_space", C.c_int32)]


KF_BEST_INIT, KF_MATCH_DIST = 128, 80


class BowVocabularyInfo(C.Structure):
    _fields_ = [("k", C.c_int32), ("L", C.c_int32), ("scoring", C.c_int32), ("weighting", C.c_int32), ("nodes", C.c_int32),
                ("words", C.c_int32), ("leaves", C.c_int32), ("max_children", C.c_int32), ("depth", C.c_int32),
                ("message", C.c_char * 188)]


class BowResult(C.Structure):
    _fields_ = [("id", C.c_int32), ("score", C.c_double)]


class BowCreateParams(C.Structure):
    _fields_ = [("k", C.c_int32), ("L", C.c_int32), ("weighting", C.c_int32), ("scoring", C.c_int32), ("max_passes", C.c_int32),
                ("reserved", C.c_int32), ("seed", C.c_uint64)]


class BowCreateInfo(C.Structure):
    _fields_ = [("nodes", C.c_int32), ("words", C.c_int32), ("depth", C.c_int32), ("max_children", C.c_int32),
# ... 68 lines not shown


_lib = None


def lib_path():
    return os.environ.get("ESVIO_FE_LIB") or os.path.join(_HERE, "libesvio_fe.so")


def load_library(build_if_missing=True):
    global _lib
    if _lib is not None:
        return _lib
    path = lib_path()
    if build_if_missing and not os.environ.get("ESVIO_FE_LIB") and _build.needs_build():
        _build.build()
    if not os.path.exists(path):
        raise FrontendError("libesvio_fe.so is missing: run `python -m esvio_amd.build`")
    L = C.CDLL(path)
    vp, i, d, sz = C.c_void_p, C.c_int, C.c_double, C.c_size_t
    L.esvio_fe_create.argtypes = [C.POINTER(Config), C.POINTER(vp)]
    L.esvio_fe_destroy.argtypes = [vp]
    L.esvio_fe_reset.argtypes = [vp]
    L.esvio_fe_last_error.restype = C.c_char_p
    L.esvio_fe_last_error.argtypes = [vp]
    L.esvio_fe_version.restype = C.c_char_p
    L.esvio_fe_create_sae.argtypes = [vp, i, vp, sz, i, C.POINTER(C.c_uint64)]
    L.esvio_fe_create_sae_stereo.argtypes = [vp, vp, sz, vp, sz, i, C.POINTER(C.c_uint64)]
    L.esvio_fe_sae_to_time_surface.argtypes = [vp, i, d, vp]
    L.esvio_fe_is_corner.argtypes = [vp, vp, sz, i, vp]
    L.esvio_fe_features_to_track.argtypes = [vp, vp, sz, i, i, vp, vp, vp, C.POINTER(C.c_int32)]
    L.esvio_fe_get_sae.argtypes = [vp, i, vp, vp, vp, vp]
    L.esvio_fe_set_sae.argtypes = [vp, i, vp, vp, vp, vp]
    L.esvio_fe_calc_optical_flow_pyr_lk.argtypes = [vp, vp, vp, i, i, vp, vp, vp, i, i, i, d, i]
    L.esvio_fe_build_pyramid.argtypes = [vp, vp, i, i, i, i, vp, vp, C.POINTER(C.c_int32),
                                         C.POINTER(C.c_int32), C.POINTER(C.c_int32)]
    L.esvio_fe_find_fundamental_mat.argtypes = [vp, vp, i, d, d, vp, C.POINTER(C.c_int32)]
    L.esvio_fe_lift_projective.argtypes = [C.POINTER(Camera), d, d, vp]
    L.esvio_fe_track_event.argtypes = [vp, d, vp, sz, vp, sz, i, i, C.POINTER(Tracks)]
    L.esvio_fe_track_event_mc.argtypes = [vp, d, vp, sz, vp, sz, i, i, C.POINTER(Motion),
                                          C.POINTER(Tracks)]
    L.esvio_fe_create_sae_stereo_mc.argtypes = [vp, vp, sz, vp, sz, i, C.POINTER(Motion),
                                                C.POINTER(C.c_uint64)]
    L.esvio_fe_set_next_batch.argtypes = [vp, d, vp, sz, vp, sz, i, i]
    L.esvio_fe_set_next_batch_mc.argtypes = [vp, d, vp, sz, vp, sz, i, i, C.POINTER(Motion)]
    L.esvio_fe_mem_alloc.argtypes = [i, sz, vp]
    L.esvio_fe_mem_free.argtypes = [i, vp]
    L.esvio_fe_mem_upload.argtypes = [vp, vp, sz]
    L.esvio_fe_register_host_buffer.argtypes = [vp, sz]
    L.esvio_fe_unregister_host_buffer.argtypes = [vp]
    L.esvio_fe_debug_inject.argtypes = [vp, i]
    L.esvio_fe_debug_counters.argtypes = [vp, vp]
    L.esvio_fe_plain_call_counters.argtypes = [vp, vp]
    L.esvio_fe_good_features_to_track.argtypes = [vp, vp, i, d, d, vp, vp, vp, vp]
    L.esvio_fe_track_image.argtypes = [vp, d, vp, vp, i, vp]
    L.esvio_fe_pack_track_records.argtypes = [vp, vp, vp]
    L.esvio_fe_set_lazy_new_stereo.argtypes = [vp, i]
    L.esvio_fe_set_host_threads.argtypes = [vp, i]
    L.esvio_fe_ransac_stats.argtypes = [vp, i]
    L.esvio_fe_host_hypot.argtypes = [vp, vp, i, vp]
    L.esvio_fe_host_stage_copy.argtypes = [vp, vp, C.c_size_t]
    L.esvio_fe_host_nullspace.argtypes = [vp, i, i, vp, C.POINTER(C.c_int32)]
    L.esvio_fe_find_fundamental_mat_mt.argtypes = [vp, vp, i, d, d, i, vp, C.POINTER(C.c_int32)]
    L.esvio_fe_finish.argtypes = [vp, vp]
    L.esvio_fe_get_time_surface.argtypes = [vp, i, vp]
    L.esvio_fe_export_image.argtypes = [vp, i, vp, i]
    L.esvio_fe_import_image.argtypes = [vp, i, vp, i]
    L.esvio_fe_export_level.argtypes = [vp, i, i, vp, vp, C.POINTER(C.c_int32), C.POINTER(C.c_int32), C.POINTER(C.c_int32)]
    L.esvio_fe_fast_corners.argtypes = [vp, i, vp, i, i, i, i, vp, vp, C.c_int32, C.POINTER(C.c_int32),
                                        C.POINTER(C.c_int32)]
    L.esvio_fe_set_detector.argtypes = [vp, i, i]
    L.esvio_fe_set_event_images.argtypes = [vp, i]
    L.esvio_fe_clear_event_images.argtypes = [vp]
    L.esvio_fe_get_event_image.argtypes = [vp, i, vp, i]
    L.esvio_fe_get_event_canvas.argtypes = [vp, vp, i]
    L.esvio_fe_event_image_kernel_stats.argtypes = [vp, i, C.POINTER(d), C.POINTER(C.c_uint64), C.POINTER(C.c_uint64)]
    L.esvio_fe_features_to_track_fast.argtypes = [vp, vp, i, i, i, vp, vp, vp, C.POINTER(C.c_int32), C.POINTER(C.c_int32)]
    L.esvio_fe_select_candidates.argtypes = [vp, vp, vp, i, d, i, vp, vp, i, i, i, i, vp, vp, vp, C.POINTER(C.c_int32)]
    L.esvio_fe_convert_events.argtypes = [vp, C.POINTER(EventFieldsDesc), sz, i, vp, i, C.POINTER(C.c_uint64)]
    L.esvio_fe_track_event_fields.argtypes = [vp, d, C.POINTER(EventFieldsDesc), sz, C.POINTER(EventFieldsDesc), sz, i, i,
                                              C.POINTER(Tracks)]
    L.esvio_fe_filter_events.argtypes = [vp, i, vp, sz, i, C.c_int64, i, vp, i, C.POINTER(C.c_uint64), vp, vp,
                                         C.POINTER(C.c_uint64)]
    L.esvio_fe_filter_reset.argtypes = [vp]
    L.esvio_fe_filter_batch.argtypes = [vp, i, vp, C.POINTER(EventFieldsDesc), sz, i, C.POINTER(FilterParams), vp, i,
                                        C.POINTER(C.c_uint64), vp, vp, C.POINTER(C.c_uint64), C.POINTER(C.c_uint64)]
    L.esvio_fe_set_address_filter.argtypes = [vp, i, C.POINTER(AddressFilter)]
    L.esvio_fe_set_pixel_mask.argtypes = [vp, i, vp, sz]
    L.esvio_fe_get_pixel_mask.argtypes = [vp, i, vp, sz, C.POINTER(sz)]
    L.esvio_fe_hot_learn.argtypes = [vp, i, vp, C.POINTER(EventFieldsDesc), sz, i, C.POINTER(C.c_uint64)]
    L.esvio_fe_hot_select.argtypes = [vp, i, C.POINTER(HotParams), vp, vp, sz, C.POINTER(HotInfo)]
    L.esvio_fe_hot_reset.argtypes = [vp]
    L.esvio_fe_track_batch.argtypes = [vp, C.POINTER(Batch), C.POINTER(Tracks), C.POINTER(BatchInfo)]
    L.esvio_fe_track_event_filtered.argtypes = [vp, vp, sz, vp, sz, i, C.c_int64, i, i, C.POINTER(Tracks),
                                                C.POINTER(C.c_uint64 * 2), C.POINTER(d)]
    L.esvio_fe_decode_raw.argtypes = [vp, i, i, vp, sz, i, C.c_int64, vp, sz, i, C.POINTER(RawInfo)]
    L.esvio_fe_decode_reset.argtypes = [vp]
    L.esvio_fe_track_raw.argtypes = [vp, i, vp, sz, vp, sz, i, C.c_int64, i, C.POINTER(FilterParams), C.POINTER(Motion),
                                     C.POINTER(Tracks), C.POINTER(BatchInfo), C.POINTER(RawInfo * 2)]
    L.esvio_fe_slice_events.argtypes = [vp, i, vp, sz, i, C.POINTER(SliceParams), vp, sz, C.POINTER(SliceInfo)]
    L.esvio_fe_decode_triggers.argtypes = [vp, i, i, vp, sz, i, C.c_int64, vp, sz, C.POINTER(TriggerInfo)]
    L.esvio_fe_raw_header.argtypes = [vp, sz, C.POINTER(RawHeaderInfo)]
    L.esvio_fe_slice_events_at.argtypes = [vp, i, vp, sz, i, vp, sz, vp, sz, C.POINTER(SliceInfo)]
    L.esvio_fe_slice_flush.argtypes = [vp, i, C.POINTER(SliceInfo)]
    L.esvio_fe_slice_reset.argtypes = [vp]
    L.esvio_fe_feed_open.argtypes = [vp, C.POINTER(SliceParams), C.POINTER(FilterParams)]
# ... 992 lines not shown
        pr, nr, sr, k2 = _events_arg(event_right)
        assert sl == sr
        self._next_keep = (getattr(self, "_next_keep", []) + [(k1, k2)])[-8:]
        if measurements is None:
            self._hd.check(self._hd.L.esvio_fe_set_next_batch(self._hd.h, float(next_cur_time), pl, nl,
                                                              pr, nr, sl, int(bool(PUB_NEXT_FRAME))))
        else:
            self._hd.check(self._hd.L.esvio_fe_set_next_batch_mc(self._hd.h, float(next_cur_time), pl, nl, pr, nr, sl,
                                                                 int(bool(PUB_NEXT_FRAME)), C.byref(measurements)))

    def reset(self):
        self._hd.check(self._hd.L.esvio_fe_reset(self._hd.h))

    def reserve(self, max_left, max_right, host_batches=False):
        self._hd.check(self._hd.L.esvio_fe_reserve(self._hd.h, int(max_left), int(max_right), int(bool(host_batches))))

    def latency_stats(self, reset=False):
        o = Latency()
        L = self._hd.L
        self._hd.check(L.esvio_fe_latency_stats(self._hd.h, C.byref(o), int(bool(reset))))
        phases = {L.esvio_fe_latency_phase_name(k).decode(): round(o.max_phase_ms[k], 4)
                  for k in range(LATENCY_PHASES) if o.max_phase_ms[k] > 0.0005}
        return dict(calls=int(o.calls), mean_ms=o.mean_ms, p50_ms=o.p50_ms, p99_ms=o.p99_ms, max_ms=o.max_ms,
                    max_call=int(o.max_call), max_published=bool(o.max_published),
                    max_cpu=(int(o.max_cpu_begin), int(o.max_cpu_end)), max_invol_switches=int(o.max_invol_switches),
                    max_allocs=int(o.max_allocs), max_phase_ms=phases, allocs=int(o.allocs),
                    invol_switches=int(o.invol_switches))

    def latency_recent(self, n):
        L = self._hd.L
        names = [L.esvio_fe_latency_phase_name(k).decode() for k in range(LATENCY_PHASES)]
        out = []
        for back in range(n - 1, -1, -1):
            o = LatencyCall()
            if L.esvio_fe_latency_recent(self._hd.h, back, C.byref(o)) != 0:
                continue
            out.append((int(o.call), bool(o.published), o.begin_ms, o.ms,
                        {names[k]: o.phase_ms[k] for k in range(LATENCY_PHASES) if o.phase_ms[k] > 0.0005}))
        return out

    def debug_inject(self, mask):
        self._hd.check(self._hd.L.esvio_fe_debug_inject(self._hd.h, int(mask)))

    def staging_counters(self):
        out = (C.c_uint64 * 4)()
        self._hd.check(self._hd.L.esvio_fe_staging_counters(self._hd.h, out))
        return dict(batches=out[0], bytes=out[1], chunks_packed=out[2], chunks_raw=out[3])

    def debug_counters(self):
        out = (C.c_uint64 * 4)()
        self._hd.check(self._hd.L.esvio_fe_debug_counters(self._hd.h, out))
        return dict(spec_redone=out[0], chain_redone=out[1], chain_launched=out[2], chain_used=out[3])

    def plain_call_counters(self):
        out = (C.c_uint64 * 4)()
        self._hd.check(self._hd.L.esvio_fe_plain_call_counters(self._hd.h, out))
        return dict(plain_calls=out[0], split_by_camera=out[1], stereo_chained=out[2], chained_redone=out[3])

    def comm_init(self, unique_id, rank, world):
        buf = (C.c_uint8 * 128).from_buffer_copy(bytes(unique_id))
        self._hd.check(self._hd.L.esvio_fe_comm_init(self._hd.h, buf, int(rank), int(world)))
        self._x_world = int(world)

    def set_auto_exchange(self, on=True):
        self._hd.check(self._hd.L.esvio_fe_set_auto_exchange(self._hd.h, int(bool(on))))

    def exchange_begin(self):
        self._hd.check(self._hd.L.esvio_fe_exchange_begin(self._hd.h))

    def exchange_end(self, want=True):
        out = np.empty((self._x_world, 2 * self.cfg.max_cnt, 8), np.float32) if want else None
        self._hd.check(self._hd.L.esvio_fe_exchange_end(self._hd.h, _p(out)))
        return out

    def device_memory(self):
        f, t = C.c_size_t(0), C.c_size_t(0)
        self._hd.check(self._hd.L.esvio_fe_device_memory(self._hd.h, C.byref(f), C.byref(t)))
        return f.value, t.value

    def sae_plane_doubles(self):
        return int(self._hd.L.esvio_fe_sae_plane_doubles(self._hd.h))

    @staticmethod
    def _planes_arg(a):
        if isinstance(a, tuple):
            return C.c_void_p(a[0]), DEVICE
        return _p(a), HOST

    def sae_slice_last(self, event_left, event_right, out):
        pl, nl, sl, k1 = _events_arg(event_left)
        pr, nr, sr, k2 = _events_arg(event_right)
        assert sl == sr
        po, so = self._planes_arg(out)
        self._hd.check(self._hd.L.esvio_fe_sae_slice_last(self._hd.h, pl, nl, pr, nr, sl, po, so))

    def sae_slice_apply(self, event_left, event_right, last_before, n_before, s_out):
        pl, nl, sl, k1 = _events_arg(event_left)
        pr, nr, sr, k2 = _events_arg(event_right)
        assert sl == sr
        pi, si = self._planes_arg(last_before) if n_before else (None, HOST)
        po, so = self._planes_arg(s_out)
        self._hd.check(self._hd.L.esvio_fe_sae_slice_apply(self._hd.h, pl, nl, pr, nr, sl, pi, int(n_before),
                                                          si, po, so))

    def sae_slice_commit(self, last_all, s_all, n_slices):
        pa, sa = self._planes_arg(last_all)
# ... 498 lines not shown
        raise FrontendError("host_nullspace rc=%d" % rc)
    return f, redone.value


def host_hypot(x, y):
    x = np.ascontiguousarray(x, np.float64)
    y = np.ascontiguousarray(y, np.float64)
    out = np.empty_like(x)
    rc = load_library().esvio_fe_host_hypot(_p(x), _p(y), x.size, _p(out))
    if rc != 0:
        raise FrontendError("host_hypot rc=%d" % rc)
    return out


def ransac_stats(reset=False):
    out = (C.c_uint64 * 6)()
    L = load_library()
    rc = L.esvio_fe_ransac_stats(out, 1 if reset else 0)
    if rc != 0:
        raise FrontendError("ransac_stats rc=%d" % rc)
    return {"calls": int(out[0]), "iterations": int(out[1]), "points": int(out[2]), "us": out[3] / 1e3,
            "lmeds_calls": int(out[4]), "lmeds_us": out[5] / 1e3}


def ransac_tail(reset=False):
    out = (C.c_uint64 * 6)()
    rc = load_library().esvio_fe_ransac_tail(out, 1 if reset else 0)
    if rc != 0:
        raise FrontendError("ransac_tail rc=%d" % rc)
    return {"max_us": out[0] / 1e3, "lmeds_max_us": out[1] / 1e3, "redone_iterations": int(out[2]),
            "solo_jobs": int(out[3]), "skipped_buffers": int(out[4]), "helper_invol_switches": int(out[5])}


def find_fundamental_mat(p1, p2, thr=1.0, conf=0.99, threads=1, hold_mask=None):
    L = load_library()
    p1 = np.ascontiguousarray(p1, np.float32).reshape(-1, 2)
    p2 = np.ascontiguousarray(p2, np.float32).reshape(-1, 2)
    n = p1.shape[0]
    status = np.zeros(n, np.uint8)
    k = C.c_int32(0)
    if hold_mask is not None:
        rc = L.esvio_fe_find_fundamental_mat_held(_p(p1), _p(p2), n, thr, conf, threads, int(hold_mask), _p(status),
                                                  C.byref(k))
    elif threads > 1:
        rc = L.esvio_fe_find_fundamental_mat_mt(_p(p1), _p(p2), n, thr, conf, threads, _p(status),
                                                C.byref(k))
    else:
        rc = L.esvio_fe_find_fundamental_mat(_p(p1), _p(p2), n, thr, conf, _p(status), C.byref(k))
    if rc:
        raise FrontendError("find_fundamental_mat rc=%d" % rc)
    return k.value, status


def find_fundamental_mat_idle(p1, p2, thr=1.0, conf=0.99, threads=4, repeats=4, idle_units=64):
    L = load_library()
    p1 = np.ascontiguousarray(p1, np.float32).reshape(-1, 2)
    p2 = np.ascontiguousarray(p2, np.float32).reshape(-1, 2)
    n = p1.shape[0]
    status = np.zeros(n, np.uint8)
    k = C.c_int32(0)
    out = (C.c_uint64 * 3)()
    rc = L.esvio_fe_find_fundamental_mat_idle(_p(p1), _p(p2), n, thr, conf, threads, repeats, idle_units, _p(status),
                                              C.byref(k), out)
    if rc:
        raise FrontendError("find_fundamental_mat_idle rc=%d" % rc)
    return k.value, status, dict(idle_calls=int(out[0]), idle_done=int(out[1]), idle_left=int(out[2]))


def raw_header(data):
    buf = bytes(data)
    info = RawHeaderInfo()
    rc = load_library().esvio_fe_raw_header(buf if buf else None, len(buf), C.byref(info))
    if rc:
        raise FrontendError("esvio_fe_raw_header rc=%d" % rc)
    return info


def text_imu(data, t_offset_ns=0, cap=None):
    buf = bytes(data)
    cap = len(buf) // 14 + 1 if cap is None else int(cap)
    out, n = np.zeros(max(cap, 1), IMU_DTYPE), C.c_size_t(0)
    rc = load_library().esvio_fe_text_imu(buf if buf else None, len(buf), int(t_offset_ns), _p(out), cap, C.byref(n))
    if rc:
        e = FrontendError("esvio_fe_text_imu rc=%d" % rc)
        e.n = int(n.value)
        raise e
    return out[:n.value]


def text_images(data, t_offset_ns=0, cap=None):
    buf = bytes(data)
    cap = len(buf) // 4 + 1 if cap is None else int(cap)
    st, off, ln, n = np.zeros(max(cap, 1), np.int64), np.zeros(max(cap, 1), np.uint64), np.zeros(max(cap, 1), np.uint32), C.c_size_t(0)
    rc = load_library().esvio_fe_text_images(buf if buf else None, len(buf), int(t_offset_ns), _p(st), _p(off), _p(ln), cap, C.byref(n))
    if rc:
        e = FrontendError("esvio_fe_text_images rc=%d" % rc)
        e.n = int(n.value)
        raise e
    k = int(n.value)
    return st[:k], [buf[int(o):int(o) + int(m)] for o, m in zip(off[:k], ln[:k])]


def text_limits():
    out = TextLimits()
    load_library().esvio_fe_text_limits(C.byref(out))
    return out
# ... 119 lines not shown
```

### include/esvio_fe.h

```cpp
#ifndef ESVIO_FE_H
#define ESVIO_FE_H

#include <stddef.h>
#include <stdint.h>

#ifdef __cplusplus
extern "C" {
#endif

#define ESVIO_FE_OK 0
#define ESVIO_FE_EINVAL (-1)
#define ESVIO_FE_ENODEVICE (-2)
#define ESVIO_FE_EHIP (-3)
#define ESVIO_FE_ENOTIMPL (-4)
#define ESVIO_FE_EINTERNAL (-5)

typedef struct esvio_fe_event {
  uint16_t x, y;
  uint32_t sec, nsec;
  uint8_t polarity;
  uint8_t _pad[3];
} esvio_fe_event;

typedef struct esvio_fe_camera {
// ... 59 lines not shown
int esvio_fe_get_sae(esvio_fe_handle h, int cam, double* L0, double* L1, double* S0, double* S1);

#define ESVIO_FE_LK_USE_INITIAL_FLOW 4
int esvio_fe_calc_optical_flow_pyr_lk(esvio_fe_handle h, const uint8_t* prev_img,
                                      const uint8_t* next_img, int w, int hgt,
                                      const float* prev_pts, float* next_pts, uint8_t* status,
                                      int n, int max_level, int max_count, double eps, int flags);
int esvio_fe_find_fundamental_mat(const float* p1, const float* p2, int n, double thr,
                                  double conf, uint8_t* status, int32_t* n_inliers);

int esvio_fe_track_event(esvio_fe_handle h, double cur_time, const esvio_fe_event* left,
                         size_t nL, const esvio_fe_event* right, size_t nR, int space,
                         int pub_this_frame, esvio_fe_tracks* out);
typedef struct esvio_fe_motion {
  double t1;
  double v[3];
  float v_pre[3];
  float accel[3];
  float omega[3];
  double fx, fy, cx, cy;
} esvio_fe_motion;

int esvio_fe_track_event_mc(esvio_fe_handle h, double cur_time, const esvio_fe_event* left,
                            size_t nL, const esvio_fe_event* right, size_t nR, int space,
                            int pub_this_frame, const esvio_fe_motion* motion,
                            esvio_fe_tracks* out);
int esvio_fe_create_sae_stereo_mc(esvio_fe_handle h, const esvio_fe_event* left, size_t nL,
                                  const esvio_fe_event* right, size_t nR, int space,
                                  const esvio_fe_motion* motion, uint64_t* n_rejected);

int esvio_fe_set_next_batch(esvio_fe_handle h, double next_cur_time, const esvio_fe_event* left,
                            size_t nL, const esvio_fe_event* right, size_t nR, int space,
                            int pub_hint);
int esvio_fe_set_next_batch_mc(esvio_fe_handle h, double next_cur_time, const esvio_fe_event* left,
                               size_t nL, const esvio_fe_event* right, size_t nR, int space,
                               int pub_hint, const esvio_fe_motion* motion);

int esvio_fe_good_features_to_track(esvio_fe_handle h, const uint8_t* img, int max_corners,
                                    double quality, double min_distance, const uint8_t* mask,
                                    float* out_xy, int32_t* n_out, float* eig_out);
int esvio_fe_track_image(esvio_fe_handle h, double cur_time, const uint8_t* img_left,
                         const uint8_t* img_right, int pub_this_frame, esvio_fe_tracks* out);

int esvio_fe_pack_track_records(esvio_fe_handle h, float* out, int32_t* n_rows);

int esvio_fe_exchange_tracks(esvio_fe_handle h, void* nccl_comm, int world, float* gathered);
int esvio_fe_comm_unique_id(uint8_t id[128]);
int esvio_fe_comm_init(esvio_fe_handle h, const uint8_t id[128], int rank, int world);
int esvio_fe_exchange_begin(esvio_fe_handle h);
int esvio_fe_exchange_end(esvio_fe_handle h, float* gathered);
int esvio_fe_set_auto_exchange(esvio_fe_handle h, int on);

int esvio_fe_set_lazy_new_stereo(esvio_fe_handle h, int on);
int esvio_fe_set_host_threads(esvio_fe_handle h, int threads);
int esvio_fe_set_launch_thread(esvio_fe_handle h, int on);
int esvio_fe_finish(esvio_fe_handle h, esvio_fe_tracks* out);

int esvio_fe_get_time_surface(esvio_fe_handle h, int cam, uint8_t* out);

int esvio_fe_fast_corners(esvio_fe_handle h, int cam, const uint8_t* img, int space, int arc, int barrier,
                          int nonmax, int16_t* out_xy, int32_t* out_score, int32_t capacity,
                          int32_t* n_out, int32_t* n_detected);

#define ESVIO_FE_DETECT_ARC  0
#define ESVIO_FE_DETECT_FAST 1
int esvio_fe_set_detector(esvio_fe_handle h, int detector, int fast_barrier);
int esvio_fe_features_to_track_fast(esvio_fe_handle h, const uint8_t* img, int space, int barrier,
                                    int max_corners, const uint8_t* mask, float* out_xy,
                                    int32_t* out_score, int32_t* n_out, int32_t* n_candidates);

typedef struct esvio_fe_event_fields {
  const void *x, *y, *t, *p;
  int32_t x_stride, y_stride, t_stride, p_stride;
  int32_t t_bits;
  int32_t t_unit_ns;
  int32_t p_bits;
  int64_t t_offset;
} esvio_fe_event_fields;
int esvio_fe_convert_events(esvio_fe_handle h, const esvio_fe_event_fields* src, size_t n, int src_space,
                            esvio_fe_event* dst, int dst_space, uint64_t* n_bad);
int esvio_fe_track_event_fields(esvio_fe_handle h, double cur_time, const esvio_fe_event_fields* left, size_t nL,
                                const esvio_fe_event_fields* right, size_t nR, int src_space,
                                int pub_this_frame, esvio_fe_tracks* out);

int esvio_fe_filter_events(esvio_fe_handle h, int cam, const esvio_fe_event* ev, size_t n, int space,
                           int64_t window_ns, int min_support, esvio_fe_event* dst, int dst_space,
                           uint64_t* n_kept, uint8_t* flags, esvio_fe_event* last_kept, uint64_t* n_rejected);
typedef struct esvio_fe_filter_params {
  int64_t window_ns;
  int32_t min_support;
  int32_t reserved;
  int64_t refractory_ns;
} esvio_fe_filter_params;
int esvio_fe_filter_batch(esvio_fe_handle h, int cam, const esvio_fe_event* ev, const esvio_fe_event_fields* fields,
                          size_t n, int space, const esvio_fe_filter_params* prm, esvio_fe_event* dst, int dst_space,
                          uint64_t* n_kept, uint8_t* flags, esvio_fe_event* last_kept, uint64_t* n_rejected,
                          uint64_t* n_bad);
int esvio_fe_filter_reset(esvio_fe_handle h);
int esvio_fe_track_event_filtered(esvio_fe_handle h, const esvio_fe_event* left, size_t nL,
                                  const esvio_fe_event* right, size_t nR, int space, int64_t window_ns,
                                  int min_support, int pub_this_frame, esvio_fe_tracks* out,
                                  uint64_t kept[2], double* cur_time_out);

typedef struct esvio_fe_address_filter {
  uint16_t roi_x0, roi_y0, roi_x1, roi_y1;
  int32_t polarity;
// ... 391 lines not shown
```

Before: 2885.

## Speculatively run publish-time F-RANSAC and masking while LK points still arrive

```diff
diff --git a/esvio_amd/csrc/fe_api.cpp b/esvio_amd/csrc/fe_api.cpp
--- a/esvio_amd/csrc/fe_api.cpp
+++ b/esvio_amd/csrc/fe_api.cpp
@@ -219,6 +219,7 @@
   if (const char* v = getenv("ESVIO_FE_FAULT")) esvio_fe_debug_inject(c, atoi(v));
   if (const char* e = getenv("ESVIO_FE_STEREO_SPLIT")) c->stereo_split_env = atoi(e) != 0;
   c->chain_enabled = getenv("ESVIO_FE_NO_CHAIN") == nullptr;
+  c->tail_spec_enabled = getenv("ESVIO_FE_NO_TAIL_SPEC") == nullptr;
   c->cam_split_enabled = getenv("ESVIO_FE_NO_CAMSPLIT") == nullptr;
   c->dedup_enabled = getenv("ESVIO_FE_NO_DEDUP") == nullptr && (cfg->max_cnt > 500 || getenv("ESVIO_FE_DEDUP") != nullptr);
   c->fuse_ts_pyr = getenv("ESVIO_FE_NO_FUSE") == nullptr;
@@ -348,6 +349,7 @@
   c->spec_valid = false;
   c->chain_valid = false;
   c->chain_map_ok = false;
+  c->chain_block_busy = false;
   c->pend.active = false;
   c->pend_right.active = false;
   HIPCHK(c, hipMemsetAsync(c->L2, 0, (size_t)2 * c->P * 16, cur_stream(c)));
@@ -692,6 +694,56 @@
   HIPCHK(c, hipStreamSynchronize(cur_stream(c)));
   if (c->prof_on) resolve_profile(c);
   return 0;
+}
+
+int esvio_fe_lk_stamp_tap(esvio_fe_handle c, const uint8_t* prev_img, const uint8_t* next_img, int w, int hgt,
+                          const float* prev_pts, int n, float* pts_stamped, uint8_t* st_stamped, float* pts_event,
+                          uint8_t* st_event, int32_t* running_at_last_stamp) {
+  if (!c || !prev_img || !next_img || n <= 0 || !prev_pts || !pts_stamped || !st_stamped || !pts_event || !st_event)
+    return ESVIO_FE_EINVAL;
+  if (w < 2 * kLkWin || hgt < 2 * kLkWin) return ESVIO_FE_EINVAL;
+  if (n > c->cfg.max_cnt) return fail(c, ESVIO_FE_EINVAL, "n > max_cnt");
+  if (c->chain_valid || c->spec_valid || !c->inflight.empty() || !c->announced.empty())
+    return fail(c, ESVIO_FE_EINVAL, "the handle has launches or batches in flight");
+  HIPCHK(c, hipSetDevice(c->dev));
+  HIPCHK(c, hipStreamSynchronize(c->stream4));
+  if (int rc = prep_tmp_pyr(c, 0, prev_img, w, hgt, 3)) return rc;
+  if (int rc = prep_tmp_pyr(c, 1, next_img, w, hgt, 3)) return rc;
+  PyrDesc two[2] = {c->tmp_pyr[0].d, c->tmp_pyr[1].d};
+  pyr_build(c, two, 2);
+  std::memcpy(c->pin[0].A, prev_pts, (size_t)n * 8);
+  LkPair lk = lk_pair(two[0], two[1], c->zpin[0].A, nullptr, n, kLkTemporal, c->zspec[1].out);
+  c->chain_seq = (c->chain_seq + 1) & 0x3fffffffu;
+  if (!c->chain_seq) c->chain_seq = 1;
+  const uint32_t seq = c->chain_seq;
+  lk.f.done = c->zspec[1].done;
+  lk.f.done_seq = seq;
+  run_lk_pair(c, lk);
+  HIPCHK(c, hipEventRecord(c->ev_chain_done, cur_stream(c)));
+  const SpecView& v = c->hspec[1];
+  auto read = [&](float* pts, uint8_t* st) {
+    std::memcpy(pts, v.out.fwd, (size_t)n * 8);
+    std::memcpy(pts + 2 * (size_t)n, v.out.back, (size_t)n * 8);
+    std::memcpy(st, v.out.st_fwd, (size_t)n);
+    std::memcpy(st + n, v.out.st_back, (size_t)n);
+  };
+  const auto t0 = std::chrono::steady_clock::now();
+  bool all = false;
+  while (!all && std::chrono::steady_clock::now() - t0 < std::chrono::seconds(2)) {
+    all = true;
+    for (int i = 0; i < n; i++) all = all && __atomic_load_n(&v.done[i], __ATOMIC_ACQUIRE) == seq;
+  }
+  if (all) {
+    if (running_at_last_stamp) {
+      *running_at_last_stamp = hipEventQuery(c->ev_chain_done) == hipErrorNotReady;
+      (void)hipGetLastError();
+    }
+    read(pts_stamped, st_stamped);
+  }
+  HIPCHK(c, hipStreamSynchronize(cur_stream(c)));
+  read(pts_event, st_event);
+  if (c->prof_on) resolve_profile(c);
+  return all ? 0 : fail(c, ESVIO_FE_EINTERNAL, "a point's completion stamp never arrived");
 }
 
 int esvio_fe_build_pyramid(esvio_fe_handle c, const uint8_t* img, int w, int hgt, int max_level,
@@ -4213,6 +4265,95 @@
   return 0;
 }
 
+int esvio_fe_tail_spec_counters(esvio_fe_handle c, uint64_t out4[4]) {
+  if (!c || !out4) return ESVIO_FE_EINVAL;
+  std::memcpy(out4, c->tail_spec, sizeof(c->tail_spec));
+  return 0;
+}
+
+int esvio_fe_find_fundamental_mat_cancel(const float* p1, const float* p2, int n, double thr, double conf, int cancel_after,
+                                         uint8_t* status, int32_t* count, uint64_t out2[2]) {
+  if (!p1 || !p2 || n < 0 || !status || !count || !out2) return ESVIO_FE_EINVAL;
+  struct Hook {
+    uint64_t asked;
+    int after;
+  } hook{0, cancel_after};
+  const host::RansacCancel cancel{[](void* p) {
+                                    Hook& h = *(Hook*)p;
+                                    const uint64_t k = h.asked++;
+                                    return h.after >= 0 && k >= (uint64_t)h.after;
+                                  },
+                                  &hook};
+  *count = host::find_fundamental_mat(p1, p2, n, thr, conf, status, nullptr, &cancel);
+  out2[0] = hook.asked;
+  out2[1] = host::ransac_cancelled();
+  return 0;
+}
+
+int esvio_fe_tail_spec_tap(const esvio_fe_camera* cam, int width, int height, int focal_length, double f_threshold,
+                           int min_dist, int f_ransac, int flow_back, int n, const float* prev_pts, const float* fwd_pts,
+                           const float* back_pts, const uint8_t* st_fwd, const uint8_t* st_back, const int32_t* ids,
+                           const int32_t* track_cnt, const int32_t* arrive_tick, int start_bound, int32_t* n_kept,
+                           int32_t* kept_ids, float* kept_pts, int32_t* kept_track_cnt, uint32_t* mask_bits,
+                           int32_t* n_f_status, uint8_t* f_status, uint64_t counters[4]) {
+  if (!cam || width <= 0 || height <= 0 || min_dist < 0 || n < 0 || !prev_pts || !fwd_pts || !back_pts || !st_fwd ||
+      !st_back || !ids || !track_cnt || !arrive_tick || start_bound < 0 || !n_kept || !kept_ids || !kept_pts ||
+      !kept_track_cnt || !mask_bits || !n_f_status || !f_status || !counters)
+    return ESVIO_FE_EINVAL;
+  const std::vector<int> hw = host::disc_halfwidths(min_dist);
+  const PubParams P{cam, (double)focal_length, f_threshold, width, height, min_dist, &hw, nullptr, f_ransac};
+  const P2f *pp = (const P2f*)prev_pts, *pf = (const P2f*)fwd_pts, *pb = (const P2f*)back_pts;
+  const std::vector<P2f> prev(pp, pp + n);
+  const std::vector<int> vid(ids, ids + n), vcnt(track_cnt, track_cnt + n);
+  struct Script : TailSpecSource {
+    const int32_t* tick;
+    const P2f *f, *b;
+    const uint8_t *sf, *sb;
+    int64_t k = 0;
+    int poll(TailSpec& ts) override {
+      for (int j = 0; j < ts.n; j++)
+        if (!ts.arrived[j] && tick[j] <= k) ts.arrive(j, f[j], b[j], sf[j], sb[j]);
+      k++;
+      return 0;
+    }
+    int64_t next = 0;
+    void idle() override {
+      next = INT64_MAX;
+      for (int j = 0; j < last->n; j++)
+        if (!last->arrived[j]) next = std::min<int64_t>(next, tick[j]);
+      if (next != INT64_MAX && next > k) k = next;
+    }
+    const TailSpec* last = nullptr;
+  } src;
+  src.tick = arrive_tick;
+  src.f = pf;
+  src.b = pb;
+  src.sf = st_fwd;
+  src.sb = st_back;
+  TailSpec ts;
+  src.last = &ts;
+  std::memset(counters, 0, 4 * sizeof(uint64_t));
+  ts.begin(P, flow_back != 0, prev, vid, vcnt, nullptr, nullptr);
+  const int r = ts.run(src, start_bound, counters);
+  if (r < 0) return ESVIO_FE_EINTERNAL;
+  if (r == 0) {
+    ts.state_of_alive(ts.result);
+    ts.compute(ts.result, ts.mask, nullptr);
+  }
+  const PubState& s = ts.result;
+  *n_kept = (int32_t)s.cur.size();
+  for (size_t i = 0; i < s.cur.size(); i++) {
+    kept_ids[i] = s.ids[i];
+    kept_track_cnt[i] = s.track_cnt[i];
+    kept_pts[2 * i] = s.cur[i].x;
+    kept_pts[2 * i + 1] = s.cur[i].y;
+  }
+  std::memcpy(mask_bits, ts.mask.bits.data(), ts.mask.bits.size() * 4);
+  *n_f_status = (int32_t)ts.f_status.size();
+  if (!ts.f_status.empty()) std::memcpy(f_status, ts.f_status.data(), ts.f_status.size());
+  return 0;
+}
+
 int esvio_fe_plain_call_counters(esvio_fe_handle c, uint64_t out4[4]) {
   if (!c || !out4) return ESVIO_FE_EINVAL;
   out4[0] = c->n_plain_calls;
diff --git a/esvio_amd/csrc/fe_ctx.h b/esvio_amd/csrc/fe_ctx.h
--- a/esvio_amd/csrc/fe_ctx.h
+++ b/esvio_amd/csrc/fe_ctx.h
@@ -256,6 +256,10 @@
   bool waits_fit_spec = true, waits_fit_chain = true;
   uint32_t chain_seq = 0;
   bool chain_enabled = true;
+  bool tail_spec_enabled = true;
+  uint64_t tail_spec[4] = {};
+  bool chain_block_busy = false;
+  uint32_t chain_done_seq = 0;
   bool cam_split_enabled = true;
   uint64_t n_plain_calls = 0, n_cam_split = 0, n_stereo_chained = 0;
   bool chain_valid = false;
diff --git a/esvio_amd/csrc/fe_host.cpp b/esvio_amd/csrc/fe_host.cpp
--- a/esvio_amd/csrc/fe_host.cpp
+++ b/esvio_amd/csrc/fe_host.cpp
@@ -754,7 +754,7 @@
 
 namespace {
 std::atomic<uint64_t> g_rs_calls{0}, g_rs_iters{0}, g_rs_points{0}, g_rs_ns{0}, g_rs_lm_calls{0}, g_rs_lm_ns{0};
-std::atomic<uint64_t> g_rs_max_ns{0}, g_rs_lm_max_ns{0}, g_rs_redone{0}, g_rs_solo{0}, g_rs_skipped{0}, g_rs_helper_sw{0};
+std::atomic<uint64_t> g_rs_max_ns{0}, g_rs_lm_max_ns{0}, g_rs_redone{0}, g_rs_solo{0}, g_rs_skipped{0}, g_rs_helper_sw{0}, g_rs_cancelled{0};
 void atomic_max(std::atomic<uint64_t>& a, uint64_t v) {
   uint64_t cur = a.load(std::memory_order_relaxed);
   while (v > cur && !a.compare_exchange_weak(cur, v, std::memory_order_relaxed)) {
@@ -1150,13 +1150,16 @@
     g_rs_solo = 0;
     g_rs_skipped = 0;
     g_rs_helper_sw = 0;
+    g_rs_cancelled = 0;
   }
   return r;
 }
+
+uint64_t ransac_cancelled() { return g_rs_cancelled.load(); }
 
 namespace {
 int ransac_pooled(RansacPool* P, const float* m1, const float* m2, int count, double thr, double conf,
-                  const double* xy, uint8_t* status, int* iterations) {
+                  const double* xy, uint8_t* status, int* iterations, const RansacCancel* cancel) {
   const int kModelPoints = 7;
   const uint32_t e = P->epoch.load(std::memory_order_relaxed) + 1;
   RansacJob& J = P->job[(e >> 1) & 1];
@@ -1186,6 +1189,10 @@
   int collinear_at = -1;
   unsigned stalled = 0;
   while (collinear_at < 0) {
+    if (cancel && cancel->fn(cancel->arg)) {
+      P->epoch.store(e + 1, std::memory_order_release);
+      return kRansacCancelled;
+    }
     while (rp < niters && rp < drawn) {
       const IterResult* r = &J.res[rp];
       const uint64_t sm = J.summary[rp].load(std::memory_order_acquire);
@@ -1269,7 +1276,8 @@
   return best_good;
 }
 
-int lmeds_pooled(RansacPool* P, const float* m1, const float* m2, int count, double conf, uint8_t* status) {
+int lmeds_pooled(RansacPool* P, const float* m1, const float* m2, int count, double conf, uint8_t* status,
+                 const RansacCancel* cancel) {
   const int kModelPoints = 7;
   const int niters = std::max(update_num_iters(conf, 0.45, kModelPoints, kRansacMaxIters), 3);
   const uint32_t e = P->epoch.load(std::memory_order_relaxed) + 1;
@@ -1295,6 +1303,10 @@
   double best[9], min_median = DBL_MAX;
   unsigned stalled = 0;
   for (int rp = 0; rp < nsub;) {
+    if (cancel && cancel->fn(cancel->arg)) {
+      P->epoch.store(e + 1, std::memory_order_release);
+      return kRansacCancelled;
+    }
     const IterResult* r = &J.res[rp];
     const uint64_t sm = J.summary[rp].load(std::memory_order_acquire);
     if ((uint32_t)(sm >> 32) != e) {
@@ -1334,7 +1346,7 @@
 }
 
 int find_fundamental_mat(const float* m1, const float* m2, int count, double thr, double conf,
-                         uint8_t* status, RansacPool* pool) {
+                         uint8_t* status, RansacPool* pool, const RansacCancel* cancel) {
   std::fill(status, status + count, (uint8_t)0);
   if (count < 7) return 0;
   if (thr <= 0) thr = 3;
@@ -1376,7 +1388,11 @@
     }
     const auto t0 = std::chrono::steady_clock::now();
     int iters = 0;
-    const int good = ransac_pooled(pool, m1, m2, count, thr, conf, xy.data(), status, &iters);
+    const int good = ransac_pooled(pool, m1, m2, count, thr, conf, xy.data(), status, &iters, cancel);
+    if (good == kRansacCancelled) {
+      g_rs_cancelled.fetch_add(1, std::memory_order_relaxed);
+      return good;
+    }
     g_rs_calls.fetch_add(1, std::memory_order_relaxed);
     g_rs_iters.fetch_add((uint64_t)iters, std::memory_order_relaxed);
     g_rs_points.fetch_add((uint64_t)count, std::memory_order_relaxed);
@@ -1387,7 +1403,11 @@
     return good;
   }
   const auto t0 = std::chrono::steady_clock::now();
-  const int good = lmeds_pooled(pool, m1, m2, count, conf, status);
+  const int good = lmeds_pooled(pool, m1, m2, count, conf, status, cancel);
+  if (good == kRansacCancelled) {
+    g_rs_cancelled.fetch_add(1, std::memory_order_relaxed);
+    return good;
+  }
   g_rs_lm_calls.fetch_add(1, std::memory_order_relaxed);
   const uint64_t ns = (uint64_t)std::chrono::duration_cast<std::chrono::nanoseconds>(
                           std::chrono::steady_clock::now() - t0).count();
diff --git a/esvio_amd/csrc/fe_host.h b/esvio_amd/csrc/fe_host.h
--- a/esvio_amd/csrc/fe_host.h
+++ b/esvio_amd/csrc/fe_host.h
@@ -45,8 +45,14 @@
 void ransac_tail(uint64_t out6[6], bool reset);
 void ransac_pool_hold(RansacPool* p, int mask, bool on);
 void ransac_pool_set_idle_work(RansacPool* p, const std::atomic<int>* pending, bool (*fn)(void*), void* arg);
+struct RansacCancel {
+  bool (*fn)(void*);
+  void* arg;
+};
+constexpr int kRansacCancelled = -1;
+uint64_t ransac_cancelled();
 int find_fundamental_mat(const float* p1, const float* p2, int n, double thr, double conf,
-                         uint8_t* status, RansacPool* pool = nullptr);
+                         uint8_t* status, RansacPool* pool = nullptr, const RansacCancel* cancel = nullptr);
 
 }
 }
diff --git a/esvio_amd/csrc/fe_internal.h b/esvio_amd/csrc/fe_internal.h
--- a/esvio_amd/csrc/fe_internal.h
+++ b/esvio_amd/csrc/fe_internal.h
@@ -73,6 +73,57 @@
 std::vector<P2f> pts_velocity_fn(std::vector<int>& ids, std::vector<P2f>& pts, IdMap& cur_id_pts,
                                  IdMap& prev_id_pts, double dt, size_t n_left);
 void reject_with_f_event(esvio_fe_ctx* c);
+bool in_border_wh(int W, int H, const P2f& pt);
+
+struct PubParams {
+  const esvio_fe_camera* cam;
+  double focal, f_threshold;
+  int W, H, min_dist;
+  const std::vector<int>* hw;
+  host::RansacPool* pool;
+  int f_ransac = 1;
+};
+struct PubState {
+  std::vector<P2f> prev, cur;
+  std::vector<int> ids, track_cnt, src_idx;
+  std::vector<double> pre_lx, pre_ly;
+};
+PubParams pub_params(const esvio_fe_ctx* c);
+int pub_reject_with_f(const PubParams& p, PubState& s, const host::RansacCancel* cancel, std::vector<uint8_t>* status_out,
+                      double* lift_ms, double* fm_ms);
+void pub_set_mask(const PubParams& p, PubState& s, host::BitMask& mask);
+void pub_commit(esvio_fe_ctx* c, PubState& s, host::BitMask& mask);
+void pub_trace_fm(esvio_fe_ctx* c, int cls, double lift_ms, double fm_ms);
+
+struct TailSpec;
+struct TailSpecSource {
+  virtual ~TailSpecSource() {}
+  virtual int poll(TailSpec& ts) = 0;
+  virtual void idle() = 0;
+};
+struct TailSpec {
+  PubParams P{};
+  bool flow_back = true;
+  const std::vector<P2f>* prev = nullptr;
+  const std::vector<int>*ids = nullptr, *track_cnt = nullptr;
+  const double *plx = nullptr, *ply = nullptr;
+  int n = 0, pending = 0, n_alive = 0;
+  std::vector<P2f> fwd, back;
+  std::vector<uint8_t> st_fwd, st_back, arrived, alive;
+  PubState input, result;
+  host::BitMask mask;
+  std::vector<uint8_t> f_status;
+  int fm_class = 0;
+  double fm_lift_ms = 0, fm_ms = 0;
+
+  void begin(const PubParams& params, bool flow_back, const std::vector<P2f>& prev_pts, const std::vector<int>& ids,
+             const std::vector<int>& track_cnt, const double* plx, const double* ply);
+  void arrive(int j, P2f f, P2f b, uint8_t sf, uint8_t sb);
+  void state_of_alive(PubState& s) const;
+  int compute(PubState& s, host::BitMask& m, const host::RansacCancel* cancel);
+  int run(TailSpecSource& src, int start_bound, uint64_t counters[4]);
+};
+constexpr int kTailSpecStart = 24;
 void clear_tracker_state(esvio_fe_ctx* c);
 SelectArgs make_select_args(esvio_fe_ctx* c, int set, int max_corners, float2* out_pts, int out_base,
                             int32_t* out_idx);
diff --git a/esvio_amd/csrc/fe_kernels.h b/esvio_amd/csrc/fe_kernels.h
--- a/esvio_amd/csrc/fe_kernels.h
+++ b/esvio_amd/csrc/fe_kernels.h
@@ -281,6 +281,8 @@
   unsigned long long poll_ticks = kTicksPoll, chain_ticks = kTicksChain;
   const uint32_t* gate_ptr = nullptr;
   uint32_t gate_val = 0;
+  uint32_t* done = nullptr;
+  uint32_t done_seq = 0;
   int max_level;
   int max_count;
   double eps2;
diff --git a/esvio_amd/csrc/fe_kernels.hip b/esvio_amd/csrc/fe_kernels.hip
--- a/esvio_amd/csrc/fe_kernels.hip
+++ b/esvio_amd/csrc/fe_kernels.hip
@@ -2346,6 +2346,8 @@
   unsigned long long poll_ticks, chain_ticks;
   const uint32_t* gate_ptr;
   uint32_t gate_val;
+  uint32_t* done;
+  uint32_t done_seq;
 };
 
 __device__ __forceinline__ void chain_publish(const LkKernelArgs& a, int pt, int lane, float2 p, int alive) {
@@ -2354,6 +2356,11 @@
   __hip_atomic_store(&a.chain_out[2 * pt], hi | __float_as_uint(p.x), __ATOMIC_RELAXED, __HIP_MEMORY_SCOPE_AGENT);
   __hip_atomic_store(&a.chain_out[2 * pt + 1], hi | __float_as_uint(p.y), __ATOMIC_RELAXED,
                      __HIP_MEMORY_SCOPE_AGENT);
+}
+
+__device__ __forceinline__ void stamp_done(const LkKernelArgs& a, int pt, int lane) {
+  if (a.done && lane == 0)
+    __hip_atomic_store(&a.done[pt], a.done_seq, __ATOMIC_RELEASE, __HIP_MEMORY_SCOPE_SYSTEM);
 }
 
 template <int ACCUM>
@@ -2365,6 +2372,7 @@
   if (pt >= a.n_max) return;
   if (pt >= n) {
     chain_publish(a, pt, lane, make_float2(0.f, 0.f), 0);
+    stamp_done(a, pt, lane);
     return;
   }
   float2 prev0;
@@ -2390,6 +2398,7 @@
         a.status[pt] = 0;
         if (a.have_back) a.back_status[pt] = 0;
       }
+      stamp_done(a, pt, lane);
       return;
     }
     prev0 = make_float2(__uint_as_float((uint32_t)vx), __uint_as_float((uint32_t)vy));
@@ -2414,6 +2423,7 @@
       const unsigned long long d = __hip_atomic_load(a.poll_done, __ATOMIC_RELAXED, __HIP_MEMORY_SCOPE_AGENT);
       if ((uint32_t)(d >> 32) == a.poll_seq && pt >= (int)(uint32_t)d) {
         chain_publish(a, pt, lane, make_float2(0.f, 0.f), 0);
+        stamp_done(a, pt, lane);
         return;
       }
       if (wall_clock64() - t0 > a.poll_ticks) {
@@ -2445,6 +2455,7 @@
       a.back_status[pt] = (uint8_t)bs;
     }
   }
+  stamp_done(a, pt, lane);
 }
 
 __global__ __launch_bounds__(64 * kLkWaves) void k_lk(LkKernelArgs a) {
@@ -2512,6 +2523,8 @@
   a.chain_ticks = f.chain_ticks;
   a.gate_ptr = f.gate_ptr;
   a.gate_val = f.gate_val;
+  a.done = f.done;
+  a.done_seq = f.done_seq;
   if (f.accum == 2)
     launch_k(k_lk_f32, dim3((a.n_max + kLkWaves - 1) / kLkWaves), dim3(64 * kLkWaves), 0, s, a);
   else
diff --git a/esvio_amd/csrc/fe_layout.h b/esvio_amd/csrc/fe_layout.h
--- a/esvio_amd/csrc/fe_layout.h
+++ b/esvio_amd/csrc/fe_layout.h
@@ -47,7 +47,7 @@
 }
 
 struct SpecLayout {
-  size_t B, C, SA, SB, expired, bytes;
+  size_t B, C, SA, SB, expired, done, bytes;
 };
 inline SpecLayout spec_layout(int max_cnt) {
   const size_t M = layout_points(max_cnt), stM = round_up(M, 64);
@@ -57,7 +57,8 @@
   L.SA = M * 16;
   L.SB = L.SA + stM;
   L.expired = L.SB + stM;
-  L.bytes = round_up(L.expired + 64, 256);
+  L.done = L.expired + 64;
+  L.bytes = round_up(L.done + M * 4, 256);
   return L;
 }
 constexpr int kSpecBlocks = 2;
@@ -85,11 +86,13 @@
 struct SpecView {
   LkOut out;
   int* expired;
+  uint32_t* done;
 };
 inline SpecView spec_view(uint8_t* b, int max_cnt, int block) {
   const SpecLayout L = spec_layout(max_cnt);
   b += (size_t)block * L.bytes;
-  return SpecView{LkOut{(P2f*)(b + L.B), (P2f*)(b + L.C), b + L.SA, b + L.SB}, (int*)(b + L.expired)};
+  return SpecView{LkOut{(P2f*)(b + L.B), (P2f*)(b + L.C), b + L.SA, b + L.SB}, (int*)(b + L.expired),
+                  (uint32_t*)(b + L.done)};
 }
 
 }
diff --git a/esvio_amd/csrc/fe_stages.cpp b/esvio_amd/csrc/fe_stages.cpp
--- a/esvio_amd/csrc/fe_stages.cpp
+++ b/esvio_amd/csrc/fe_stages.cpp
@@ -507,46 +507,76 @@
 }
 
 
-bool in_border_event(const esvio_fe_ctx* c, const P2f& pt) {
-  const int BORDER_SIZE = 1;
-  const int img_x = host::cv_round(pt.x), img_y = host::cv_round(pt.y);
-  return BORDER_SIZE <= img_x && img_x < c->W - BORDER_SIZE && BORDER_SIZE <= img_y &&
-         img_y < c->H - BORDER_SIZE;
-}
+bool in_border_event(const esvio_fe_ctx* c, const P2f& pt) { return in_border_wh(c->W, c->H, pt); }
 
 double pt_distance(const P2f& a, const P2f& b) {
   const double dx = a.x - b.x, dy = a.y - b.y;
   return std::sqrt(dx * dx + dy * dy);
 }
 
-void event_set_mask(esvio_fe_ctx* c) {
-  c->mask_event.reset(c->W, c->H);
+bool in_border_wh(int W, int H, const P2f& pt) {
+  const int BORDER_SIZE = 1;
+  const int img_x = host::cv_round(pt.x), img_y = host::cv_round(pt.y);
+  return BORDER_SIZE <= img_x && img_x < W - BORDER_SIZE && BORDER_SIZE <= img_y && img_y < H - BORDER_SIZE;
+}
+
+PubParams pub_params(const esvio_fe_ctx* c) {
+  return PubParams{&c->cfg.cam[0], (double)c->cfg.focal_length, (double)c->cfg.f_threshold, c->W, c->H, c->cfg.min_dist, &c->hw, c->pool,
+                   c->cfg.f_ransac};
+}
+
+void pub_set_mask(const PubParams& p, PubState& s, host::BitMask& mask) {
+  mask.reset(p.W, p.H);
   struct Item {
     int first;
     std::pair<P2f, int> second;
     int src;
   };
   std::vector<Item> cnt_pts_id;
-  cnt_pts_id.reserve(c->cur_pts.size());
-  for (unsigned int i = 0; i < c->cur_pts.size(); i++)
-    cnt_pts_id.push_back(Item{c->track_cnt[i], std::make_pair(c->cur_pts[i], c->ids[i]), c->src_idx[i]});
+  cnt_pts_id.reserve(s.cur.size());
+  for (unsigned int i = 0; i < s.cur.size(); i++)
+    cnt_pts_id.push_back(Item{s.track_cnt[i], std::make_pair(s.cur[i], s.ids[i]), s.src_idx[i]});
   std::sort(cnt_pts_id.begin(), cnt_pts_id.end(),
             [](const Item& a, const Item& b) { return a.first > b.first; });
-  c->cur_pts.clear();
-  c->ids.clear();
-  c->track_cnt.clear();
-  c->src_idx.clear();
+  s.cur.clear();
+  s.ids.clear();
+  s.track_cnt.clear();
+  s.src_idx.clear();
   for (auto& it : cnt_pts_id) {
     const int px = host::cv_round(it.second.first.x), py = host::cv_round(it.second.first.y);
-    if (px < 0 || px >= c->W || py < 0 || py >= c->H) continue;
-    if (!c->mask_event.test(px, py)) {
-      c->cur_pts.push_back(it.second.first);
-      c->ids.push_back(it.second.second);
-      c->track_cnt.push_back(it.first);
-      c->src_idx.push_back(it.src);
-      c->mask_event.stamp_disc(px, py, c->cfg.min_dist, c->hw);
+    if (px < 0 || px >= p.W || py < 0 || py >= p.H) continue;
+    if (!mask.test(px, py)) {
+      s.cur.push_back(it.second.first);
+      s.ids.push_back(it.second.second);
+      s.track_cnt.push_back(it.first);
+      s.src_idx.push_back(it.src);
+      mask.stamp_disc(px, py, p.min_dist, *p.hw);
     }
   }
+}
+
+static void pub_swap(esvio_fe_ctx* c, PubState& s) {
+  s.prev.swap(c->prev_pts);
+  s.cur.swap(c->cur_pts);
+  s.ids.swap(c->ids);
+  s.track_cnt.swap(c->track_cnt);
+  s.src_idx.swap(c->src_idx);
+}
+
+void pub_commit(esvio_fe_ctx* c, PubState& s, host::BitMask& mask) {
+  pub_swap(c, s);
+  c->mask_event.bits.swap(mask.bits);
+  c->mask_event.W = mask.W;
+  c->mask_event.H = mask.H;
+  c->mask_event.wpr = mask.wpr;
+  c->pre_lift_valid = false;
+}
+
+void event_set_mask(esvio_fe_ctx* c) {
+  PubState s;
+  pub_swap(c, s);
+  pub_set_mask(pub_params(c), s, c->mask_event);
+  pub_swap(c, s);
 }
 
 std::vector<P2f> undistorted_pts(const std::vector<P2f>& pts, const esvio_fe_camera& cam) {
@@ -581,46 +611,174 @@
   return vel;
 }
 
+int pub_reject_with_f(const PubParams& p, PubState& s, const host::RansacCancel* cancel, std::vector<uint8_t>* status_out,
+                      double* lift_ms, double* fm_ms) {
+  const size_t n = s.cur.size();
+  if (status_out) status_out->clear();
+  if (n < 8) return 0;
+  const esvio_fe_camera& cam = *p.cam;
+  const double FOCAL = p.focal;
+  std::vector<float> un_cur(n * 2), un_prev(n * 2);
+  std::vector<double> lx(n), ly(n);
+  const double cx = p.W / 2.0, cy = p.H / 2.0;
+  const auto tl = std::chrono::steady_clock::now();
+  const bool pre = s.pre_lx.size() == n && s.pre_ly.size() == n;
+  if (!pre) host::lift_projective_batch(cam, &s.prev[0].x, (int)n, lx.data(), ly.data());
+  const double* plx = pre ? s.pre_lx.data() : lx.data();
+  const double* ply = pre ? s.pre_ly.data() : ly.data();
+  for (size_t i = 0; i < n; i++) {
+    un_prev[2 * i] = (float)(FOCAL * plx[i] / 1.0 + cx);
+    un_prev[2 * i + 1] = (float)(FOCAL * ply[i] / 1.0 + cy);
+  }
+  host::lift_projective_batch(cam, &s.cur[0].x, (int)n, lx.data(), ly.data());
+  for (size_t i = 0; i < n; i++) {
+    un_cur[2 * i] = (float)(FOCAL * lx[i] / 1.0 + cx);
+    un_cur[2 * i + 1] = (float)(FOCAL * ly[i] / 1.0 + cy);
+  }
+  std::vector<uint8_t> status(n);
+  const auto t0 = std::chrono::steady_clock::now();
+  const int good = host::find_fundamental_mat(un_prev.data(), un_cur.data(), (int)n, p.f_threshold, 0.99, status.data(),
+                                              p.pool, cancel);
+  if (good == host::kRansacCancelled) return good;
+  if (fm_ms) *fm_ms = std::chrono::duration<double, std::milli>(std::chrono::steady_clock::now() - t0).count();
+  if (lift_ms) *lift_ms = std::chrono::duration<double, std::milli>(t0 - tl).count();
+  reduce_vector(s.prev, status);
+  reduce_vector(s.cur, status);
+  reduce_vector(s.ids, status);
+  reduce_vector(s.track_cnt, status);
+  reduce_vector(s.src_idx, status);
+  s.pre_lx.clear();
+  s.pre_ly.clear();
+  if (status_out) status_out->swap(status);
+  return n < 15 ? 1 : 2;
+}
+
+void pub_trace_fm(esvio_fe_ctx* c, int cls, double lift_ms, double fm_ms) {
+  if (!c->trace) return;
+  c->tr_fm_class[cls]++;
+  if (!cls) return;
+  c->tr_fm_ms += fm_ms;
+  c->tr_fm_max_ms = std::max(c->tr_fm_max_ms, fm_ms);
+  c->tr_lift_ms += lift_ms;
+}
+
 void reject_with_f_event(esvio_fe_ctx* c) {
-  if (c->trace) c->tr_fm_class[c->cur_pts.size() < 8 ? 0 : c->cur_pts.size() < 15 ? 1 : 2]++;
-  if (c->cur_pts.size() >= 8) {
-    const esvio_fe_camera& cam = c->cfg.cam[0];
-    const double FOCAL = c->cfg.focal_length;
-    const size_t n = c->prev_pts.size();
-    std::vector<float> un_cur(n * 2), un_prev(n * 2);
-    std::vector<double> lx(n), ly(n);
-    const double cx = c->W / 2.0, cy = c->H / 2.0;
-    const auto tl = std::chrono::steady_clock::now();
-    const bool pre = c->pre_lift_valid && c->pre_lx.size() == n;
-    if (!pre) host::lift_projective_batch(cam, &c->prev_pts[0].x, (int)n, lx.data(), ly.data());
-    const double* plx = pre ? c->pre_lx.data() : lx.data();
-    const double* ply = pre ? c->pre_ly.data() : ly.data();
-    c->pre_lift_valid = false;
-    for (size_t i = 0; i < n; i++) {
-      un_prev[2 * i] = (float)(FOCAL * plx[i] / 1.0 + cx);
-      un_prev[2 * i + 1] = (float)(FOCAL * ply[i] / 1.0 + cy);
+  PubState s;
+  pub_swap(c, s);
+  if (c->pre_lift_valid && c->pre_lx.size() == s.prev.size()) {
+    s.pre_lx.swap(c->pre_lx);
+    s.pre_ly.swap(c->pre_ly);
+  }
+  c->pre_lift_valid = false;
+  double lift_ms = 0, fm_ms = 0;
+  const int cls = pub_reject_with_f(pub_params(c), s, nullptr, nullptr, &lift_ms, &fm_ms);
+  pub_trace_fm(c, cls, lift_ms, fm_ms);
+  pub_swap(c, s);
+}
+
+void TailSpec::begin(const PubParams& params, bool flow_back_, const std::vector<P2f>& prev_pts, const std::vector<int>& ids_,
+                     const std::vector<int>& track_cnt_, const double* plx_, const double* ply_) {
+  P = params;
+  flow_back = flow_back_;
+  prev = &prev_pts;
+  ids = &ids_;
+  track_cnt = &track_cnt_;
+  plx = plx_;
+  ply = ply_;
+  n = (int)prev_pts.size();
+  fwd.assign(n, P2f{0, 0});
+  back.assign(n, P2f{0, 0});
+  st_fwd.assign(n, 0);
+  st_back.assign(n, 0);
+  arrived.assign(n, 0);
+  alive.assign(n, 0);
+  pending = n;
+  n_alive = 0;
+}
+
+void TailSpec::arrive(int j, P2f f, P2f b, uint8_t sf, uint8_t sb) {
+  if (arrived[j]) return;
+  fwd[j] = f;
+  back[j] = b;
+  st_fwd[j] = sf;
+  st_back[j] = sb;
+  bool ok = sf != 0;
+  if (flow_back) ok = ok && sb && pt_distance((*prev)[j], b) <= 0.5;
+  ok = ok && in_border_wh(P.W, P.H, f);
+  arrived[j] = 1;
+  alive[j] = ok ? 1 : 0;
+  n_alive += ok ? 1 : 0;
+  pending--;
+}
+
+void TailSpec::state_of_alive(PubState& s) const {
+  s = PubState();
+  for (int j = 0; j < n; j++) {
+    if (!alive[j]) continue;
+    s.src_idx.push_back((int)s.cur.size());
+    s.prev.push_back((*prev)[j]);
+    s.cur.push_back(fwd[j]);
+    s.ids.push_back((*ids)[j]);
+    s.track_cnt.push_back((*track_cnt)[j] + 1);
+    if (plx) {
+      s.pre_lx.push_back(plx[j]);
+      s.pre_ly.push_back(ply[j]);
     }
-    host::lift_projective_batch(cam, &c->cur_pts[0].x, (int)n, lx.data(), ly.data());
-    for (size_t i = 0; i < n; i++) {
-      un_cur[2 * i] = (float)(FOCAL * lx[i] / 1.0 + cx);
-      un_cur[2 * i + 1] = (float)(FOCAL * ly[i] / 1.0 + cy);
+  }
+}
+
+int TailSpec::compute(PubState& s, host::BitMask& m, const host::RansacCancel* cancel) {
+  double lift_ms = 0, ms = 0;
+  const int cls = P.f_ransac ? pub_reject_with_f(P, s, cancel, &f_status, &lift_ms, &ms) : 0;
+  if (cls == host::kRansacCancelled) return cls;
+  if (cancel && cancel->fn(cancel->arg)) return host::kRansacCancelled;
+  pub_set_mask(P, s, m);
+  fm_class = cls;
+  fm_lift_ms = lift_ms;
+  fm_ms = ms;
+  return cls;
+}
+
+int TailSpec::run(TailSpecSource& src, int start_bound, uint64_t counters[4]) {
+  struct Watch {
+    TailSpec* ts;
+    TailSpecSource* src;
+    int alive0;
+    bool gave_up;
+  } w{this, &src, 0, false};
+  const host::RansacCancel cancel{[](void* p) {
+                                    Watch& w = *(Watch*)p;
+                                    if (w.src->poll(*w.ts) < 0) w.gave_up = true;
+                                    return w.gave_up || w.ts->n_alive != w.alive0;
+                                  },
+                                  &w};
+  bool started = false, have = false;
+  int have_alive = -1;
+  for (;;) {
+    if (src.poll(*this) < 0) return -1;
+    if (!pending) break;
+    if (pending <= start_bound && !(have && have_alive == n_alive)) {
+      counters[started ? 1 : 0]++;
+      started = true;
+      have = false;
+      w.alive0 = n_alive;
+      state_of_alive(input);
+      result = input;
+      if (compute(result, mask, &cancel) != host::kRansacCancelled) {
+        have = true;
+        have_alive = w.alive0;
+      }
+      if (w.gave_up) return -1;
+      continue;
     }
-    std::vector<uint8_t> status(c->cur_pts.size());
-    const auto t0 = std::chrono::steady_clock::now();
-    host::find_fundamental_mat(un_prev.data(), un_cur.data(), (int)c->cur_pts.size(),
-                               c->cfg.f_threshold, 0.99, status.data(), c->pool);
-    if (c->trace) {
-      const double ms = std::chrono::duration<double, std::milli>(std::chrono::steady_clock::now() - t0).count();
-      c->tr_fm_ms += ms;
-      c->tr_fm_max_ms = std::max(c->tr_fm_max_ms, ms);
-      c->tr_lift_ms += std::chrono::duration<double, std::milli>(t0 - tl).count();
-    }
-    reduce_vector(c->prev_pts, status);
-    reduce_vector(c->cur_pts, status);
-    reduce_vector(c->ids, status);
-    reduce_vector(c->track_cnt, status);
-    reduce_vector(c->src_idx, status);
-  }
+    src.idle();
+  }
+  if (have && have_alive == n_alive) {
+    counters[2]++;
+    return 1;
+  }
+  if (started) counters[3]++;
+  return 0;
 }
 
 void clear_tracker_state(esvio_fe_ctx* c) {
diff --git a/esvio_amd/csrc/fe_track.cpp b/esvio_amd/csrc/fe_track.cpp
--- a/esvio_amd/csrc/fe_track.cpp
+++ b/esvio_amd/csrc/fe_track.cpp
@@ -313,9 +313,16 @@
     HIPCHK(c, hipStreamWaitEvent(c->stream4, c->ev_lane_done[nxt.lane], 0));
     if (!gated) HIPCHK(c, hipStreamWaitEvent(c->stream4, c->ev_lane_done[nxt2->lane], 0));
     const PyrDesc& N2 = c->pyr[nxt2->slotL].d;
+    if (c->chain_block_busy) {
+      c->chain_block_busy = false;
+      HIPCHK(c, sync_event(c->ev_chain_done));
+      *c->hspec[1].expired = 0;
+    }
     LkPair ch = lk_pair(N, N2, nullptr, nullptr, n_max, kLkTemporal, c->zspec[1].out);
     ch.f.chain_in = c->d_chain;
     ch.f.chain_seq = c->chain_seq;
+    ch.f.done = c->zspec[1].done;
+    ch.f.done_seq = c->chain_done_seq = c->chain_seq;
     ch.f.chain_ticks = c->lim.chain;
     ch.f.poll_err = c->zspec[1].expired;
     if (gated) {
@@ -343,6 +350,40 @@
   HIPCHK(c, hipStreamSynchronize(c->stream4));
   return 0;
 }
+
+static bool event_over(hipEvent_t ev);
+
+struct StampSource : TailSpecSource {
+  esvio_fe_ctx* c;
+  std::vector<int> wait;
+  unsigned quiet = 0;
+  bool over = false;
+  explicit StampSource(esvio_fe_ctx* ctx) : c(ctx), wait(ctx->chain_map.size()) {
+    for (size_t j = 0; j < wait.size(); j++) wait[j] = (int)j;
+  }
+  int poll(TailSpec& ts) override {
+    const SpecView& v = c->hspec[1];
+    const uint32_t seq = c->chain_done_seq;
+    size_t k = 0;
+    for (size_t i = 0; i < wait.size(); i++) {
+      const int j = wait[i], pt = c->chain_map[j];
+      if (__atomic_load_n(&v.done[pt], __ATOMIC_ACQUIRE) == seq)
+        ts.arrive(j, v.out.fwd[pt], v.out.back[pt], v.out.st_fwd[pt], v.out.st_back[pt]);
+      else
+        wait[k++] = j;
+    }
+    const bool got = k != wait.size();
+    wait.resize(k);
+    if (wait.empty()) return 0;
+    if (over || __atomic_load_n(v.expired, __ATOMIC_RELAXED)) return -1;
+    if (got)
+      quiet = 0;
+    else if (++quiet % 16 == 0)
+      over = event_over(c->ev_chain_done);
+    return 0;
+  }
+  void idle() override { cpu_relax(); }
+};
 
 void right_tail(esvio_fe_ctx* c, const LkOut& kept, const P2f* left, const int* ids, const int* src,
                 int n, int n_kept, double dt, size_t n_left) {
@@ -464,6 +505,8 @@
   bool will_spec = false, detect = false;
   bool plain = false, arc_side = false, stereo_chained = false;
   bool split_right = false;
+  TailSpec tail;
+  bool tail_read = false, tail_done = false;
   int set_st = 0;
   std::vector<int> surv_src;
   int n_surv = 0, n_kept = 0;
@@ -683,12 +726,26 @@
 
   bool take_expired(int block) { return std::exchange(*c->hspec[block].expired, 0) != 0; }
 
-  int await_early(hipEvent_t done, int block, bool* ok) {
+  int await_early(hipEvent_t done, int block, bool* ok, bool by_point = false) {
     if (!defer_late)
       if (int rc = early_work()) return rc;
     pre_lift();
     lap(PH_ENQ_TEMPORAL);
     if (int rc = exchange_flush(c)) return rc;
+    if (by_point) {
+      tail.begin(pub_params(c), c->cfg.flow_back != 0, c->prev_pts, c->ids, c->track_cnt,
+                 c->pre_lift_valid ? c->pre_lx.data() : nullptr, c->pre_lift_valid ? c->pre_ly.data() : nullptr);
+      StampSource src(c);
+      const int r = tail.run(src, kTailSpecStart, c->tail_spec);
+      if (r >= 0) {
+        lap(PH_WAIT_TEMPORAL);
+        c->chain_block_busy = true;
+        tail_read = true;
+        tail_done = r == 1;
+        *ok = true;
+        return 0;
+      }
+    }
     HIPCHK(c, sync_event(done));
     lap(PH_WAIT_TEMPORAL);
     *ok = !take_expired(block);
@@ -716,11 +773,22 @@
       std::vector<P2f> g_ptsB, g_ptsC;
       std::vector<uint8_t> g_stA, g_stB;
       if (use_chain) {
-        if (int rc = await_early(c->ev_chain_done, 1, &spec_ok)) return rc;
+        const bool by_point = PUB_THIS_FRAME && c->tail_spec_enabled && cfg.f_ransac && n >= 8;
+        if (int rc = await_early(c->ev_chain_done, 1, &spec_ok, by_point)) return rc;
         c->tr_chain_used += spec_ok;
         if (!spec_ok) c->n_chain_expired++;
         if (c->trace && spec_ok) trace_chain_intervals();
-        if (spec_ok) {
+        if (tail_done) {
+          c->prev_pts.swap(tail.input.prev);
+          c->cur_pts.swap(tail.input.cur);
+          c->ids.swap(tail.input.ids);
+          c->track_cnt.swap(tail.input.track_cnt);
+          c->pre_lift_valid = false;
+          return 0;
+        }
+        if (tail_read) {
+          t = LkOut{tail.fwd.data(), tail.back.data(), tail.st_fwd.data(), tail.st_back.data()};
+        } else if (spec_ok) {
           const LkOut& r = c->hspec[1].out;
           g_ptsB.resize(n);
           g_ptsC.resize(n);
@@ -742,6 +810,11 @@
         stereo_chained = plain && c->chain_enabled && c->waits_fit_chain;
         if (stereo_chained) {
           c->n_stereo_chained++;
+          if (c->chain_block_busy) {
+            c->chain_block_busy = false;
+            HIPCHK(c, sync_event(c->ev_chain_done));
+            *c->hspec[1].expired = 0;
+          }
           lk.f.chain_out = c->d_chain;
           lk.f.chain_seq = next_chain_seq(c);
         }
@@ -871,11 +944,16 @@
     const PyrDesc& curL = c->pyr[c->slot_curL].d;
     const PyrDesc& curR = c->pyr[c->slot_curR].d;
     if (PUB_THIS_FRAME) {
-      if (cfg.f_ransac) reject_with_f_event(c);
+      if (tail_done) {
+        pub_trace_fm(c, tail.fm_class, tail.fm_lift_ms, tail.fm_ms);
+        pub_commit(c, tail.result, tail.mask);
+      } else if (cfg.f_ransac) {
+        reject_with_f_event(c);
+      }
       lap(PH_RANSAC);
       PhaseClock parts;
       auto sub = [&](Phase p) { c->lat.cur_phase[p] += parts.lap(); };
-      event_set_mask(c);
+      if (!tail_done) event_set_mask(c);
       sub(PH_PUB_SETMASK);
       if (arc_side) HIPCHK(c, hipStreamWaitEvent(c->stream, c->ev_arc_side, 0));
       n_kept = (int)c->cur_pts.size();
diff --git a/esvio_amd/frontend.py b/esvio_amd/frontend.py
--- a/esvio_amd/frontend.py
+++ b/esvio_amd/frontend.py
@@ -336,7 +336,7 @@
     "esvio_fe_sae_slice_last", "esvio_fe_sae_to_time_surface", "esvio_fe_set_address_filter", "esvio_fe_set_auto_exchange",
     "esvio_fe_set_detector", "esvio_fe_set_pixel_mask",
     "esvio_fe_set_event_images", "esvio_fe_clear_event_images", "esvio_fe_get_event_image", "esvio_fe_get_event_canvas",
-    "esvio_fe_set_host_threads", "esvio_fe_set_launch_thread", "esvio_fe_set_lazy_new_stereo",
+    "esvio_fe_set_host_threads", "esvio_fe_set_launch_thread", "esvio_fe_set_lazy_new_stereo", "esvio_fe_tail_spec_counters",
     "esvio_fe_set_next_batch", "esvio_fe_set_next_batch_mc", "esvio_fe_slice_events", "esvio_fe_slice_flush",
     "esvio_fe_slice_reset", "esvio_fe_track_batch", "esvio_fe_track_event", "esvio_fe_track_event_fields",
     "esvio_fe_track_event_filtered", "esvio_fe_track_event_mc", "esvio_fe_track_raw",
@@ -352,6 +352,7 @@
     "esvio_fe_build_pyramid", "esvio_fe_debug_counters", "esvio_fe_debug_inject", "esvio_fe_device_memory",
     "esvio_fe_export_level",
     "esvio_fe_find_fundamental_mat_held", "esvio_fe_find_fundamental_mat_idle", "esvio_fe_find_fundamental_mat_mt",
+    "esvio_fe_find_fundamental_mat_cancel", "esvio_fe_tail_spec_tap", "esvio_fe_lk_stamp_tap",
     "esvio_fe_get_kernel_stats", "esvio_fe_host_hypot", "esvio_fe_host_nullspace", "esvio_fe_host_stage_copy",
     "esvio_fe_host_stage_pack", "esvio_fe_staging_counters",
     "esvio_fe_kernel_count", "esvio_fe_kernel_name", "esvio_fe_latency_phase_name", "esvio_fe_latency_recent",
@@ -526,6 +527,11 @@
     L.esvio_fe_debug_inject.argtypes = [vp, i]
     L.esvio_fe_debug_counters.argtypes = [vp, vp]
     L.esvio_fe_plain_call_counters.argtypes = [vp, vp]
+    L.esvio_fe_tail_spec_counters.argtypes = [vp, vp]
+    L.esvio_fe_lk_stamp_tap.argtypes = [vp, vp, vp, i, i, vp, i, vp, vp, vp, vp, C.POINTER(C.c_int32)]
+    L.esvio_fe_find_fundamental_mat_cancel.argtypes = [vp, vp, i, d, d, i, vp, C.POINTER(C.c_int32), vp]
+    L.esvio_fe_tail_spec_tap.argtypes = [vp, i, i, i, d, i, i, i, i, vp, vp, vp, vp, vp, vp, vp, vp, i, C.POINTER(C.c_int32),
+                                         vp, vp, vp, vp, C.POINTER(C.c_int32), vp, vp]
     L.esvio_fe_good_features_to_track.argtypes = [vp, vp, i, d, d, vp, vp, vp, vp]
     L.esvio_fe_track_image.argtypes = [vp, d, vp, vp, i, vp]
     L.esvio_fe_pack_track_records.argtypes = [vp, vp, vp]
@@ -1624,6 +1630,24 @@
         self._hd.check(self._hd.L.esvio_fe_debug_counters(self._hd.h, out))
         return dict(spec_redone=out[0], chain_redone=out[1], chain_launched=out[2], chain_used=out[3])
 
+    def lk_stamp_tap(self, prev_img, next_img, prev_pts):
+        prev_img, next_img = np.ascontiguousarray(prev_img, np.uint8), np.ascontiguousarray(next_img, np.uint8)
+        hgt, w = prev_img.shape
+        assert next_img.shape == (hgt, w)
+        p = np.ascontiguousarray(prev_pts, np.float32).reshape(-1, 2)
+        n = len(p)
+        pa, pb = np.zeros((2, n, 2), np.float32), np.zeros((2, n, 2), np.float32)
+        sa, sb = np.zeros((2, n), np.uint8), np.zeros((2, n), np.uint8)
+        run = C.c_int32(0)
+        self._hd.check(self._hd.L.esvio_fe_lk_stamp_tap(self._hd.h, _p(prev_img), _p(next_img), w, hgt, _p(p), n, _p(pa), _p(sa),
+                                                        _p(pb), _p(sb), C.byref(run)))
+        return (pa, sa), (pb, sb), bool(run.value)
+
+    def tail_spec_counters(self):
+        out = (C.c_uint64 * 4)()
+        self._hd.check(self._hd.L.esvio_fe_tail_spec_counters(self._hd.h, out))
+        return dict(started=out[0], restarted=out[1], committed=out[2], redone=out[3])
+
     def plain_call_counters(self):
         out = (C.c_uint64 * 4)()
         self._hd.check(self._hd.L.esvio_fe_plain_call_counters(self._hd.h, out))
@@ -2228,6 +2252,46 @@
     return k.value, status
 
 
+def find_fundamental_mat_cancel(p1, p2, thr=1.0, conf=0.99, cancel_after=0):
+    L = load_library()
+    p1 = np.ascontiguousarray(p1, np.float32).reshape(-1, 2)
+    p2 = np.ascontiguousarray(p2, np.float32).reshape(-1, 2)
+    n = len(p1)
+    status = np.zeros(max(n, 1), np.uint8)
+    k = C.c_int32(0)
+    out = (C.c_uint64 * 2)()
+    rc = L.esvio_fe_find_fundamental_mat_cancel(_p(p1), _p(p2), n, thr, conf, int(cancel_after), _p(status), C.byref(k), out)
+    if rc != 0:
+        raise FrontendError("find_fundamental_mat_cancel rc=%d" % rc)
+    return k.value, status[:n], int(out[0]), int(out[1])
+
+
+def tail_spec_tap(cam, width, height, prev_pts, fwd_pts, back_pts, st_fwd, st_back, ids, track_cnt, arrive_tick,
+                  start_bound=24, focal_length=460, f_threshold=1.0, min_dist=10, f_ransac=1, flow_back=1):
+    L = load_library()
+    f32 = lambda a: np.ascontiguousarray(a, np.float32).reshape(-1, 2)
+    prev_pts, fwd_pts, back_pts = f32(prev_pts), f32(fwd_pts), f32(back_pts)
+    n = len(prev_pts)
+    u8 = lambda a: np.ascontiguousarray(a, np.uint8)
+    i32 = lambda a: np.ascontiguousarray(a, np.int32)
+    st_fwd, st_back, ids, track_cnt, arrive_tick = u8(st_fwd), u8(st_back), i32(ids), i32(track_cnt), i32(arrive_tick)
+    assert len(fwd_pts) == len(back_pts) == len(st_fwd) == len(st_back) == len(ids) == len(track_cnt) == len(arrive_tick) == n
+    m = max(n, 1)
+    kept_ids, kept_cnt, kept_pts = np.zeros(m, np.int32), np.zeros(m, np.int32), np.zeros((m, 2), np.float32)
+    mask = np.zeros((height, (width + 31) // 32), np.uint32)
+    f_status = np.zeros(m, np.uint8)
+    nk, nf = C.c_int32(0), C.c_int32(0)
+    cnt = (C.c_uint64 * 4)()
+    rc = L.esvio_fe_tail_spec_tap(C.byref(cam), width, height, focal_length, f_threshold, min_dist, f_ransac, flow_back, n,
+                                  _p(prev_pts), _p(fwd_pts), _p(back_pts), _p(st_fwd), _p(st_back), _p(ids), _p(track_cnt),
+                                  _p(arrive_tick), int(start_bound), C.byref(nk), _p(kept_ids), _p(kept_pts), _p(kept_cnt),
+                                  _p(mask), C.byref(nf), _p(f_status), cnt)
+    if rc != 0:
+        raise FrontendError("tail_spec_tap rc=%d" % rc)
+    return dict(ids=kept_ids[:nk.value].copy(), pts=kept_pts[:nk.value].copy(), track_cnt=kept_cnt[:nk.value].copy(), mask=mask,
+                f_status=f_status[:nf.value].copy() if nf.value else None, counters=[int(x) for x in cnt])
+
+
 def find_fundamental_mat_idle(p1, p2, thr=1.0, conf=0.99, threads=4, repeats=4, idle_units=64):
     L = load_library()
     p1 = np.ascontiguousarray(p1, np.float32).reshape(-1, 2)
diff --git a/include/esvio_fe.h b/include/esvio_fe.h
--- a/include/esvio_fe.h
+++ b/include/esvio_fe.h
@@ -135,6 +135,7 @@
 int esvio_fe_set_auto_exchange(esvio_fe_handle h, int on);
 
 int esvio_fe_set_lazy_new_stereo(esvio_fe_handle h, int on);
+int esvio_fe_tail_spec_counters(esvio_fe_handle h, uint64_t out4[4]);
 int esvio_fe_set_host_threads(esvio_fe_handle h, int threads);
 int esvio_fe_set_launch_thread(esvio_fe_handle h, int on);
 int esvio_fe_finish(esvio_fe_handle h, esvio_fe_tracks* out);
```

New measurement: 2988 (median of 6 runs). 1.04x the previous value.
